# AdvancedPhotonSource/tike

Measured on AMD Instinct MI355X. Metric: diffraction patterns/sec/GPU (256x256, 8-mode probe), higher is better.
Workload: dtype c64; 1 GPU; c3; positions_per_gpu=10000, modes=8, detector=256, eigen_probes=1, solver=lstsq_grad, num_batch=10, chunk_positions=1000, position_correction=False, object_update=after every minibatch (batch_method wobbly_center), route=no_farplane

## Files before the change

include/tike_amd.h:

```cpp
#ifndef TIKE_AMD_H
#define TIKE_AMD_H

#ifdef __cplusplus
extern "C" {
#endif

#define TIKE_ERR_ARG 1000001
#define TIKE_ERR_UNSUPPORTED 1000002
#define TIKE_ERR_COMM 2000000
#define TIKE_COMM_ID_BYTES 128

#define TIKE_ABI_VERSION 11

const char* tike_build_id(void);

int tike_abi_version(void);

int tike_set_deterministic(int on, void* scratch, long bytes);

int tike_init(void);

int tike_patch_fwd(const void* images, void* patches, const float* positions, int nimage, int H,
                   int W, int nscan, int nrepeat, int patch_width, int padded_width,
                   void* stream);
int tike_patch_adj(void* images, const void* patches, const float* positions, int nimage, int H,
                   int W, int nscan, int nrepeat, int patch_width, int padded_width, int npatch,
                   void* stream);

int tike_conv_fwd(const void* psi, const float* scan, const void* probe, int probe_per_scan,
                  void* nearplane, int nscan, int S, int pw, int det, int H, int W, void* stream);
int tike_conv_adj(const void* nearplane, const float* scan, const void* probe,
                  int probe_per_scan, void* psi, int nscan, int S, int pw, int det, int H, int W,
                  void* stream);
int tike_conv_adj_probe(const void* nearplane, const float* scan, const void* psi,
                        void* probe_adj, int nscan, int S, int pw, int det, int H, int W,
                        void* stream);

int tike_fft2(const void* in, void* out, long ntile, int n, int inverse, float scale,
              void* stream);

int tike_fft2_supported(int n);

int tike_fft2_general(const void* in, void* out, long ntile, int n, int inverse, float scale,
                      int lines_per_group_rows, int lines_per_group_cols, void* stream);

int tike_ptycho_fwd(const void* psi, const float* scan, const void* probe, int probe_per_scan,
                    const void* eigen_probe, const float* eigen_weights, int num_eigen,
                    int eigen_modes, void* farplane, int nscan, int S, int pw, int det, int H,
                    int W, float scale, int sub_batch, void* stream);

int tike_ptycho_adj(const void* farplane, const void* probe, int probe_per_scan,
                    const float* scan, const void* psi, void* psi_adj, void* probe_adj,
                    void* objproj_work, float* acc_work, int nscan, int S, int pw, int det,
                    int H, int W, float scale, int sub_batch, void* stream);

int tike_ptycho_fwd_intensity(const void* psi, const float* scan, const void* probe,
                              int probe_per_scan, const void* unique_probe,
                              const float* eigen_weights, int num_eigen, int eigen_modes,
                              void* farplane, float* intensity, void* patches, int nscan, int S,
                              int pw, int det, int H, int W, float scale, void* stream);

int tike_ptycho_fwd_intensity_only(const void* psi, const float* scan, const void* probe,
                                   int probe_per_scan, const void* unique_probe,
                                   const float* eigen_weights, int num_eigen, int eigen_modes,
                                   void* scratch, float* intensity, int nscan, int S, int pw,
                                   int det, int H, int W, float scale, void* stream);

int tike_ptycho_fwd_gradient_scale(const void* psi, const float* scan, const void* probe,
                                   int probe_per_scan, const void* unique_probe,
                                   const float* eigen_weights, int num_eigen, int eigen_modes,
                                   void* scratch, float* intensity, void* patches,
                                   const float* data, const unsigned char* measured,
                                   float* gscale, float* costs, int nscan, int S, int pw, int det,
                                   int H, int W, float scale, int model, float unmeasured_scaling,
                                   long num_measured, void* stream);

int tike_fwd_pass1(const void* psi, const float* scan, const void* probe, int probe_per_scan,
                   const void* unique_probe, const void* eigen_probe,
                   const float* eigen_weights, int num_eigen, int eigen_modes, void* scratch,
                   void* patches, int nscan, int S, int pw, int det, int H, int W, void* stream);
int tike_fwd_gradient_scale(const void* scratch, const void* data, int data_u16,
                            const unsigned char* measured, float* gscale, float* intensity,
                            float* costs, void* farplane, int nscan, int S, int det, float scale,
                            int model, float unmeasured_scaling, long num_measured,
                            void* stream);

int tike_grad_ifft2_crop(const void* colin, const float* gscale, const float* mode_scale,
                         const unsigned char* measured, int S, void* work, void* chi,
                         long ntile, int det, int pw, float fwd_scale, float inv_scale,
                         void* stream);

int tike_fwd_grad_ifft2_pass1(const void* scratch, const void* data, int data_u16,
                              const unsigned char* measured, float* costs, void* work,
                              int nscan, int S, int det, float fwd_scale, int model,
                              float unmeasured_scaling, long num_measured, void* stream);
int tike_fwd_grad_ifft2_pass1_slices(const void* scratch, const void* data, int data_u16,
                                     const unsigned char* measured, float* costs, void* work,
                                     int nscan, int S, int det, float fwd_scale, int model,
                                     float unmeasured_scaling, long num_measured,
                                     const void* propagator, int nslices, void* stream);
int tike_grad_ifft2_pass1(const void* colin, const float* gscale, const float* mode_scale,
                          const unsigned char* measured, int S, void* work, long ntile, int det,
                          float fwd_scale, void* stream);
int tike_ifft2_pass1_scaled(const void* farplane, const float* gscale, const float* mode_scale,
                            const unsigned char* measured, int S, void* work, long ntile, int det,
                            void* stream);

int tike_ifft2_pass2_gradients(const void* work, const void* patches, const void* probe,
                               const void* eigen_probe, const float* eigen_weights,
                               int num_eigen, int eigen_modes, void* objproj, void* chi0,
                               void* m_probe_update, float mpu_scale, int nscan, int S, int det,
                               float inv_scale, void* stream);
int tike_ifft2_pass2_gradients_scaled(const void* work, const void* patches, const void* probe,
                                      const void* eigen_probe, const float* eigen_weights,
                                      int num_eigen, int eigen_modes, void* objproj, void* chi0,
                                      void* m_probe_update, float mpu_scale, int nscan, int S,
                                      int det, float inv_scale, const float* mode_scale,
                                      void* stream);
int tike_ifft2_pass2_eigen_fits(int det, int num_eigen, int eigen_modes);
int tike_ifft2_pass2_gradients_modes(const void* work, const void* patches, const void* probe,
                                     const void* eigen_probe, const float* eigen_weights,
                                     int num_eigen, int eigen_modes, void* objproj, void* chi0,
                                     void* m_probe_update, float mpu_scale, int nscan, int S,
                                     int det, float inv_scale, int mode0, int nmodes,
                                     int accumulate, void* stream);

int tike_gradient_scale(const float* intensity, const float* data, const unsigned char* measured,
                        float* gscale, float* costs, int nscan, int det, int model,
                        float unmeasured_scaling, long num_measured, void* stream);

int tike_ifft2_crop_scaled(const void* farplane, const float* gscale, int S, void* work,
                           void* chi, long ntile, int det, int pw, float scale, void* stream);

int tike_poisson_steps(const void* farplane, const float* intensity, const float* data,
                       const unsigned char* measured, float* steps, int nscan, int S, int det,
                       float step_start, float weight, int dominant_mode, void* stream);

int tike_poisson_steps_handoff(const void* scratch, const void* data, int data_u16,
                               const unsigned char* measured, float* gscale, float* costs,
                               float* steps, float* sums, int nscan, int S, int det, float scale,
                               float unmeasured_scaling, long num_measured, float step_start,
                               float weight, void* stream);

int tike_poisson_steps_grad_ifft2_pass1(const void* scratch, const void* data, int data_u16,
                                        const unsigned char* measured, float* costs,
                                        float* steps, float* sums, void* work, int nscan, int S,
                                        int det, float scale, float unmeasured_scaling,
                                        long num_measured, float step_start, float weight,
                                        void* stream);

int tike_ifft2_crop_scaled_modes(const void* farplane, const float* gscale,
                                 const float* mode_scale, const unsigned char* measured, int S,
                                 void* work, void* chi, long ntile, int det, int pw, float scale,
                                 void* stream);

int tike_scale_modes(void* farplane, const float* mode_scale, const unsigned char* measured,
                     long ntile, int det, void* stream);

int tike_ifft2_crop(const void* farplane, void* work, void* chi, long ntile, int det, int pw,
                    float scale, void* stream);

int tike_farplane_gradient(void* farplane, const float* data, const unsigned char* measured,
                           float* intensity, float* costs, int nscan, int S, int det, int model,
                           int apply_gradient, float unmeasured_scaling, long num_measured,
                           void* stream);
// ... 37 lines not shown

int tike_varying_probe(const void* probe, const void* eigen_probe, const float* eigen_weights,
                       int num_eigen, int eigen_modes, void* out, int nscan, int S, int pw,
                       void* stream);


int tike_eigen_position_sums(const void* patches, const void* chi0, const void* mpu0,
                             const void* eigen_probe, const void* coefs, int num_eigen,
                             int eigen_modes, int c, float* sums, int nscan, int pw,
                             int chi_modes, void* stream);

int tike_eigen_pixel_update(const void* patches, const void* chi0, const void* mpu0,
                            const void* eigen_probe, const void* coefs, int num_eigen,
                            int eigen_modes, int c, const float* pm, void* update, int nscan,
                            int pw, int chi_modes, void* stream);

int tike_position_sums(const void* patches, const void* chi, int chi_modes, const void* probe,
                       const void* eigen_probe, const float* eigen_weights, int num_eigen,
                       int eigen_modes, const float* taps, int radius, float* numerator,
                       float* denominator, int nscan, int S, int pw, void* stream);

int tike_gen_supported(int S, int pw, int det);

int tike_gen_fwd_rows(const void* psi, const float* scan, const void* probe, int probe_per_scan,
                      const void* unique, const void* eigen_probe, const float* eigen_weights,
                      int num_eigen, int eigen_modes, void* hand1, void* patches, int nscan, int S,
                      int pw, int det, int H, int W, void* stream);

int tike_gen_cols_gradient(const void* hand1, const float* data, const unsigned char* measured,
                           float* costs, void* hand2, int nscan, int S, int pw, int det,
                           float fwd_scale, int model, float unmeasured_scaling,
                           long num_measured, void* stream);

int tike_gen_inv_rows_gradients(const void* hand2, const void* patches, const void* probe,
                                int probe_per_scan, const void* unique, const void* eigen_probe,
                                const float* eigen_weights, int num_eigen, int eigen_modes,
                                void* objproj, void* chi0, void* m_probe_update,
                                float probe_update_scale, int nscan, int S, int pw, int det,
                                float inv_scale, void* stream);

int tike_pfa_supported(int S, int pw, int det);

int tike_pfa_fwd_gather(const void* psi, const float* scan, const void* probe,
                        int probe_per_scan, const void* unique, const void* eigen_probe,
                        const float* eigen_weights, int num_eigen, int eigen_modes,
                        void* subtiles, void* patches, int nscan, int S, int pw, int det, int H,
                        int W, void* stream);

int tike_pfa_fft2(const void* in, void* out, long ntile, int det, int inverse, void* stream);

int tike_pfa_fwd_subtiles_supported(int S, int pw, int det);
int tike_pfa_fwd_subtiles(const void* psi, const float* scan, const void* probe,
                          const void* eigen_probe, const float* eigen_weights, int num_eigen,
                          int eigen_modes, void* probe_scratch, void* subtiles, void* patches,
                          int nscan, int S, int pw, int det, int H, int W, void* stream);

int tike_pfa_combine_gradient(void* subtiles, const float* data, const unsigned char* measured,
                              float* costs, int nscan, int S, int det, float fwd_scale, int model,
                              float unmeasured_scaling, long num_measured, int apply_gradient,
                              void* stream);

int tike_pfa_inv_products(const void* subtiles, const void* patches, const void* probe,
                          int probe_per_scan, const void* unique, const void* eigen_probe,
                          const float* eigen_weights, int num_eigen, int eigen_modes,
                          void* objproj, void* chi0, void* m_probe_update,
                          float probe_update_scale, int nscan, int S, int pw, int det,
                          float inv_scale, void* stream);


int tike_fft2_pass1(const void* in, void* out, long ntile, int det, int inverse, void* stream);

int tike_fft2_pass2_inplace(void* tiles, long ntile, int det, int inverse, float scale,
                            void* stream);

int tike_slice_step(void* wave, const void* psi, const float* scan, void* farplane1, int nscan,
                    int S, int det, int H, int W, float scale, void* stream);

int tike_fft2_pass2_intensity(void* tiles, float* amplitude, long nscan, int S, int det,
                              int inverse, float scale, int keep, void* stream);

int tike_fresnel_colpass(const void* colin, const void* propagator, int adjoint, void* work,
                         long ntile, int det, float scale, void* stream);

int tike_ifft2_pass2_products(void* work, const void* psi, const float* scan, const void* probe,
                              int probe_per_scan, void* objproj, void* probe_numerator,
                              float numerator_scale, void* chi0, int keep_chi, int nscan, int S,
                              int det, int H, int W, float inv_scale, void* stream);

int tike_fresnel_spect_prop(const void* in, void* out, const void* propagator, long ntile, int n,
                            int adjoint, float fwd_scale, float inv_scale, void* stream);


int tike_object_update_precond(const float* acc, const void* precond, const float* pmax,
                               float alpha, void* upd_sum, void* upd_precond, float* combined,
                               long npix, void* stream);

int tike_lstsq_step_sums(const float* stats, const float* costs, int B, float eps, float* sums,
                         void* stream);
int tike_lstsq_step_solve(const float* stats, int B, float eps, const float* sums, double count,
                          int recover_psi, int recover_probe, float* out, void* stream);

int tike_probe_update(void* probe, void* combined, const void* mpu, const float* beta,
                      float inv_num_batch, long n, void* stream);

int tike_eigen_weights0(float* weights, const float* stats, int B, int C, int S, int m,
                        float* norms, void* stream);
int tike_eigen_proj_mean(const float* first, int first_stride, const float* weights_c,
                         long weights_row, const float* norm, long P, int B, float* pm,
                         void* stream);
int tike_eigen_normalise(void* eigen, const void* update, double count, float beta, int npix,
                         float* esum, float* work, void* stream);
int tike_eigen_dsum(const float* sums, int B, long P, float* dsum, void* stream);
int tike_eigen_weights(const float* sums, int B, long P, const float* dsum, double count,
                       float* weights_c, long weights_row, void* coefs_c, int coef_stride,
                       const float* esum, void* stream);

int tike_cgrad_direction(const float* update_planar, const void* update_complex, void* gradient,
                         void* direction, long n, int first, const float* costs, int ncost,
                         double count, double* state, double* sums, void* stream);

int tike_cgrad_line_search(int variable, const void* x, const void* d, void* xs,
                           const void* other, const float* scan, const void* data,
                           int data_u16, void* scratch, float* costs, int nscan, int chunk,
                           int S, int det, int H, int W, float fwd_scale, double count,
                           double* state, int* skip, int nslots, void* stream);

int tike_cgrad_line_search_linear(int variable, const void* x, const void* d, void* xs,
                                  const void* other, const float* scan, const void* data,
                                  int data_u16, void* far_a, int a_valid, void* far_b,
                                  float* costs_k, int nscan, int chunk, int S, int det, int H,
                                  int W, float fwd_scale, double count, double* state,
                                  int stage, double* sums, void* stream);

int tike_eigen_pixel_update1(const void* patches, const void* chi0, const void* mpu0,
                             const void* eigen0, const float* eigen_proj,
                             const float* weights_c, long weights_row, const float* norm,
                             void* update, int nscan, int pw, int chi_modes, const float* stats,
                             const float* costs, float eps, float* sums3, const void* psi,
                             const float* scan, int H, int W, void* stream);
int tike_lstsq_tail_mid(void* eigen0, const void* update, int npix, float* nacc,
                        float beta_eigen, const float* stats, int B, float eps,
                        const float* sums3, double count, int recover_psi, int recover_probe,
                        float* tail3, void* stream);
int tike_eigen_position_sums1(const void* patches, const void* chi0, const void* mpu0,
                              const void* eigen0, float* sums5, float* dsum, int nscan, int pw,
                              int chi_modes, const void* psi, const float* scan, int H, int W,
                              void* stream);
int tike_lstsq_tail_finish(const float* tail3, const float* sums3, double count, float* steps,
                           void* probe, void* combined, const void* mpu, float inv_num_batch,
                           long nprobe, float* weights, long weights_row, int S, int m,
                           const float* stats, const float* sums5, int B, int npix,
                           void* stream);

int tike_lstsq_chunk_gradients(const void* psi, const float* scan, const void* probe,
                               const void* eigen_probe, const float* eigen_weights,
                               int num_eigen, int eigen_modes, const void* data, int data_u16,
                               const unsigned char* measured, int model,
                               float unmeasured_scaling, long num_measured, void* scratch,
                               void* work, float* gscale, void* patches, float* costs,
                               void* objproj, void* chi0, void* m_probe_update,
                               float mpu_scale, float* object_acc, int nscan, int S, int det,
                               int H, int W, float fwd_scale, float inv_scale, void* stream);

int tike_comm_unique_id(void* id);
int tike_comm_create(const void* id, int nranks, int rank, void** comm);
int tike_comm_destroy(void* comm);
int tike_comm_allreduce_sum(void* comm, void* buf, long count, int f64, void* stream);
int tike_comm_broadcast(void* comm, void* buf, long nbytes, int root, void* stream);

int tike_cluster_farthest_fill(const float* points, long n, long* owner, int num_cluster,
                               long turns);
int tike_cluster_swap_sweep(const double* dist, long n, int k, long* label, const long* best,
                            const long* order, double* regret, int* moved);

#ifdef __cplusplus
}
#endif
#endif
```

tike_amd/_lib.py:

```python
import ctypes
import os
import re

import torch

_HERE = os.path.dirname(os.path.abspath(__file__))
LIB_PATH = os.environ.get("TIKE_AMD_LIB") or os.path.join(
    _HERE, "csrc", "libtike_amd.so")
HEADER_PATH = os.path.join(os.path.dirname(_HERE), "include", "tike_amd.h")

ABI_VERSION = 11
ERR_ARG = 1000001
ERR_UNSUPPORTED = 1000002
ERR_COMM = 2000000
COMM_ID_BYTES = 128

if not os.path.isfile(LIB_PATH):
    raise ImportError(
        f"{LIB_PATH} not found: build the HIP library first "
        "(`make -C tike_amd/csrc` or `python -c 'import __graft_entry__ as g; "
        "g.build()'`). tike_amd has no CPU fallback.")

lib = ctypes.CDLL(LIB_PATH)

_p = ctypes.c_void_p
_i = ctypes.c_int
_l = ctypes.c_long
_f = ctypes.c_float
_d = ctypes.c_double

_PROTOTYPES = {
    "tike_abi_version": [],
    "tike_init": [],
    "tike_set_deterministic": [_i, _p, _l],
    "tike_patch_fwd": [_p, _p, _p, _i, _i, _i, _i, _i, _i, _i, _p],
    "tike_patch_adj": [_p, _p, _p, _i, _i, _i, _i, _i, _i, _i, _i, _p],
    "tike_conv_fwd": [_p, _p, _p, _i, _p, _i, _i, _i, _i, _i, _i, _p],
    "tike_conv_adj": [_p, _p, _p, _i, _p, _i, _i, _i, _i, _i, _i, _p],
    "tike_conv_adj_probe": [_p, _p, _p, _p, _i, _i, _i, _i, _i, _i, _p],
    "tike_fft2": [_p, _p, _l, _i, _i, _f, _p],
    "tike_fft2_supported": [_i],
    "tike_fft2_general": [_p, _p, _l, _i, _i, _f, _i, _i, _p],
    "tike_pfa_supported": [_i, _i, _i],
    "tike_pfa_fwd_gather": [_p, _p, _p, _i, _p, _p, _p, _i, _i, _p, _p, _i, _i, _i,
                            _i, _i, _i, _p],
    "tike_pfa_fwd_subtiles_supported": [_i, _i, _i],
    "tike_pfa_fwd_subtiles": [_p, _p, _p, _p, _p, _i, _i, _p, _p, _p, _i, _i,
                              _i, _i, _i, _i, _p],
    "tike_pfa_fft2": [_p, _p, _l, _i, _i, _p],
    "tike_pfa_combine_gradient": [_p, _p, _p, _p, _i, _i, _i, _f, _i, _f, _l, _i,
                                  _p],
    "tike_pfa_inv_products": [_p, _p, _p, _i, _p, _p, _p, _i, _i, _p, _p, _p, _f,
                              _i, _i, _i, _i, _f, _p],
    "tike_gen_supported": [_i, _i, _i],
    "tike_gen_fwd_rows": [_p, _p, _p, _i, _p, _p, _p, _i, _i, _p, _p, _i, _i, _i,
                          _i, _i, _i, _p],
    "tike_gen_cols_gradient": [_p, _p, _p, _p, _p, _i, _i, _i, _i, _f, _i, _f,
                               _l, _p],
    "tike_gen_inv_rows_gradients": [_p, _p, _p, _i, _p, _p, _p, _i, _i, _p, _p,
                                    _p, _f, _i, _i, _i, _i, _f, _p],
    "tike_fresnel_spect_prop": [_p, _p, _p, _l, _i, _i, _f, _f, _p],
    "tike_fft2_pass1": [_p, _p, _l, _i, _i, _p],
    "tike_fft2_pass2_inplace": [_p, _l, _i, _i, _f, _p],
    "tike_slice_step": [_p, _p, _p, _p, _i, _i, _i, _i, _i, _f, _p],
    "tike_fft2_pass2_intensity": [_p, _p, _l, _i, _i, _i, _f, _i, _p],
    "tike_fresnel_colpass": [_p, _p, _i, _p, _l, _i, _f, _p],
    "tike_ifft2_pass2_products": [_p, _p, _p, _p, _i, _p, _p, _f, _p, _i, _i, _i,
                                  _i, _i, _i, _f, _p],
    "tike_ptycho_fwd": [_p, _p, _p, _i, _p, _p, _i, _i, _p, _i, _i, _i, _i,
                        _i, _i, _f, _i, _p],
    "tike_ptycho_adj": [_p, _p, _i, _p, _p, _p, _p, _p, _p, _i, _i, _i, _i, _i,
                        _i, _f, _i, _p],
    "tike_ifft2_crop": [_p, _p, _p, _l, _i, _i, _f, _p],
    "tike_ptycho_fwd_intensity": [_p, _p, _p, _i, _p, _p, _i, _i, _p, _p, _p,
                                  _i, _i, _i, _i, _i, _i, _f, _p],
    "tike_gradient_scale": [_p, _p, _p, _p, _p, _i, _i, _i, _f, _l, _p],
    "tike_ifft2_crop_scaled": [_p, _p, _i, _p, _p, _l, _i, _i, _f, _p],
    "tike_ifft2_crop_scaled_modes": [_p, _p, _p, _p, _i, _p, _p, _l, _i, _i, _f,
                                     _p],
    "tike_poisson_steps": [_p, _p, _p, _p, _p, _i, _i, _i, _f, _f, _i, _p],
    "tike_poisson_steps_handoff": [_p, _p, _i, _p, _p, _p, _p, _p, _i, _i, _i, _f,
                                   _f, _l, _f, _f, _p],
    "tike_scale_modes": [_p, _p, _p, _l, _i, _p],
    "tike_ptycho_fwd_intensity_only": [_p, _p, _p, _i, _p, _p, _i, _i, _p, _p,
                                       _i, _i, _i, _i, _i, _i, _f, _p],
    "tike_ptycho_fwd_gradient_scale": [_p, _p, _p, _i, _p, _p, _i, _i, _p, _p,
                                       _p, _p, _p, _p, _p, _i, _i, _i, _i, _i,
                                       _i, _f, _i, _f, _l, _p],
    "tike_fwd_pass1": [_p, _p, _p, _i, _p, _p, _p, _i, _i, _p, _p, _i, _i, _i,
                       _i, _i, _i, _p],
    "tike_fwd_gradient_scale": [_p, _p, _i, _p, _p, _p, _p, _p, _i, _i, _i, _f,
                                _i, _f, _l, _p],
    "tike_grad_ifft2_pass1": [_p, _p, _p, _p, _i, _p, _l, _i, _f, _p],
    "tike_fwd_grad_ifft2_pass1": [_p, _p, _i, _p, _p, _p, _i, _i, _i, _f, _i, _f,
                                  _l, _p],
    "tike_fwd_grad_ifft2_pass1_slices": [_p, _p, _i, _p, _p, _p, _i, _i, _i, _f, _i, _f,
                                  _l, _p, _i, _p],
    "tike_ifft2_pass1_scaled": [_p, _p, _p, _p, _i, _p, _l, _i, _p],
    "tike_ifft2_pass2_gradients": [_p, _p, _p, _p, _p, _i, _i, _p, _p, _p, _f,
                                   _i, _i, _i, _f, _p],
    "tike_ifft2_pass2_gradients_scaled": [_p, _p, _p, _p, _p, _i, _i, _p, _p,
                                          _p, _f, _i, _i, _i, _f, _p, _p],
    "tike_ifft2_pass2_eigen_fits": [_i, _i, _i],
    "tike_ifft2_pass2_gradients_modes": [_p, _p, _p, _p, _p, _i, _i, _p, _p,
                                         _p, _f, _i, _i, _i, _f, _i, _i, _i, _p],
    "tike_poisson_steps_grad_ifft2_pass1": [_p, _p, _i, _p, _p, _p, _p, _p, _i,
                                            _i, _i, _f, _f, _l, _f, _f, _p],
    "tike_object_update_precond": [_p, _p, _p, _f, _p, _p, _p, _l, _p],
    "tike_lstsq_step_sums": [_p, _p, _i, _f, _p, _p],
    "tike_lstsq_step_solve": [_p, _i, _f, _p, _d, _i, _i, _p, _p],
    "tike_probe_update": [_p, _p, _p, _p, _f, _l, _p],
    "tike_eigen_weights0": [_p, _p, _i, _i, _i, _i, _p, _p],
    "tike_eigen_proj_mean": [_p, _i, _p, _l, _p, _l, _i, _p, _p],
    "tike_eigen_normalise": [_p, _p, _d, _f, _i, _p, _p, _p],
    "tike_eigen_dsum": [_p, _i, _l, _p, _p],
    "tike_eigen_weights": [_p, _i, _l, _p, _d, _p, _l, _p, _i, _p, _p],
    "tike_grad_ifft2_crop": [_p, _p, _p, _p, _i, _p, _p, _l, _i, _i, _f, _f,
                             _p],
    "tike_position_sums": [_p, _p, _i, _p, _p, _p, _i, _i, _p, _i, _p, _p, _i,
                           _i, _i, _p],
    "tike_farplane_gradient": [_p, _p, _p, _p, _p, _i, _i, _i, _i, _i, _f, _l,
                               _p],
    "tike_intensity": [_p, _p, _l, _i, _l, _p],
    "tike_cost_each_pattern": [_p, _p, _p, _l, _l, _i, _p],
    "tike_objective_grad": [_p, _p, _p, _p, _l, _i, _l, _i, _p],
    "tike_lstsq_gradients": [_p, _p, _p, _p, _p, _p, _i, _i, _p, _p, _p, _p, _i,
                             _i, _i, _i, _i, _p],
    "tike_varying_probe": [_p, _p, _p, _i, _i, _p, _i, _i, _i, _p],
    "tike_scatter_patches": [_p, _p, _p, _i, _i, _i, _i, _p],
    "tike_eigen_position_sums": [_p, _p, _p, _p, _p, _i, _i, _i, _p, _i, _i,
                                 _i, _p],
    "tike_eigen_pixel_update": [_p, _p, _p, _p, _p, _i, _i, _i, _p, _p, _i, _i,
                                _i, _p],
    "tike_probe_grad": [_p, _p, _p, _p, _p, _i, _i, _i, _i, _i, _p],
    "tike_probe_preconditioner": [_p, _p, _p, _i, _i, _i, _i, _p],
    "tike_psi_preconditioner": [_p, _p, _p, _i, _i, _i, _i, _p],
    "tike_scatter_amplitudes": [_p, _p, _p, _i, _i, _i, _i, _p],
    "tike_lstsq_step_stats": [_p, _p, _p, _p, _p, _p, _p, _i, _i, _p, _p, _p,
                              _p, _i, _i, _i, _i, _i, _i, _p, _p, _p],
    "tike_eigen_pixel_update1": [_p, _p, _p, _p, _p, _p, _l, _p, _p, _i, _i, _i,
                                 _p, _p, _f, _p, _p, _p, _i, _i, _p],
    "tike_lstsq_tail_mid": [_p, _p, _i, _p, _f, _p, _i, _f, _p, _d, _i, _i, _p,
                            _p],
    "tike_eigen_position_sums1": [_p, _p, _p, _p, _p, _p, _i, _i, _i, _p, _p,
                                  _i, _i, _p],
    "tike_lstsq_tail_finish": [_p, _p, _d, _p, _p, _p, _p, _f, _l, _p, _l, _i,
                               _i, _p, _p, _i, _i, _p],
    "tike_lstsq_chunk_gradients": [_p, _p, _p, _p, _p, _i, _i, _p, _i, _p, _i,
                                   _f, _l, _p, _p, _p, _p, _p, _p, _p, _p, _f,
                                   _p, _i, _i, _i, _i, _i, _f, _f, _p],
    "tike_cgrad_direction": [_p, _p, _p, _p, _l, _i, _p, _i, _d, _p, _p, _p],
    "tike_cgrad_line_search": [_i, _p, _p, _p, _p, _p, _p, _i, _p, _p, _i, _i,
                               _i, _i, _i, _i, _f, _d, _p, _p, _i, _p],
    "tike_cgrad_line_search_linear": [_i, _p, _p, _p, _p, _p, _p, _i, _p, _i, _p,
                                      _p, _i, _i, _i, _i, _i, _i, _f, _d, _p, _i,
                                      _p, _p],
    "tike_comm_unique_id": [_p],
    "tike_comm_create": [_p, _i, _i, ctypes.POINTER(_p)],
    "tike_comm_destroy": [_p],
    "tike_comm_allreduce_sum": [_p, _p, _l, _i, _p],
    "tike_comm_broadcast": [_p, _p, _l, _i, _p],
    "tike_cluster_farthest_fill": [_p, _l, _p, _i, _l],
    "tike_cluster_swap_sweep": [_p, _l, _i, _p, _p, _p, _p, _p],
}


def build_id():
    try:
        fn = lib.tike_build_id
    except AttributeError:
        return ""
    fn.restype = ctypes.c_char_p
    fn.argtypes = []
    return fn().decode()


def declared_symbols():
    with open(HEADER_PATH) as f:
        text = f.read()
    return sorted(set(re.findall(r"^int\s+(tike_\w+)\s*\(", text, flags=re.M)))


for _name, _args in _PROTOTYPES.items():
    try:
        _fn = getattr(lib, _name)
    except AttributeError as e:
        raise ImportError(
            f"{LIB_PATH} does not export {_name}: it was built from another "
            "include/tike_amd.h; rebuild it (`make -C tike_amd/csrc`).") from e
    _fn.argtypes = _args
    _fn.restype = ctypes.c_int


def _check_abi_version():
    got = lib.tike_abi_version()
    m = re.search(r"^#define\s+TIKE_ABI_VERSION\s+(\d+)", open(HEADER_PATH).read(),
                  flags=re.M) if os.path.isfile(HEADER_PATH) else None
    if got != ABI_VERSION or (m and int(m.group(1)) != ABI_VERSION):
        raise ImportError(
            f"{LIB_PATH} reports ABI version {got}, include/tike_amd.h "
            f"{m.group(1) if m else '?'}, this binding expects {ABI_VERSION}: "
            "rebuild the library (`make -C tike_amd/csrc`).")


_check_abi_version()


def check(rc, what=""):
    if rc == 0:
        return
    if rc == ERR_ARG:
        raise ValueError(f"{what}: incompatible shapes / arguments")
    if rc == ERR_UNSUPPORTED:
        raise ValueError(f"{what}: unsupported size for the HIP path")
    if rc >= ERR_COMM:
        raise RuntimeError(f"{what}: RCCL error {rc - ERR_COMM}")
    raise RuntimeError(f"{what}: HIP error {rc}")


DETERMINISTIC = os.environ.get("TIKE_DETERMINISTIC", "0") == "1"
DETERMINISTIC_SCRATCH_MIB = int(os.environ.get("TIKE_DETERMINISTIC_MIB", "256"))
_det_scratch = None


def ensure_deterministic():
    global _det_scratch
    if not DETERMINISTIC:
        return
    current = torch.cuda.current_device()
    if _det_scratch is not None and _det_scratch.device.index == current:
        return
    if _det_scratch is not None:
        torch.cuda.synchronize(_det_scratch.device)
    _det_scratch = torch.empty(DETERMINISTIC_SCRATCH_MIB << 20,
                               dtype=torch.uint8,
                               device=torch.device("cuda", current))
    check(lib.tike_set_deterministic(1, _det_scratch.data_ptr(),
                                     _det_scratch.numel()),
          "tike_set_deterministic")
```

tike_amd/_tuning.py:

```python
import os


def _flag(name, default):
    return os.environ.get(name, "1" if default else "0") == "1"


def _int(name, default=None):
    v = os.environ.get(name)
    return int(v) if v else default


one_launch_512 = _flag("TIKE_ONE_LAUNCH_512", True)
poisson_steps_in_pass2 = _flag("TIKE_POISSON_LINEAR", True)
chunk_positions = _int("TIKE_CHUNK_POSITIONS")
eigen_sums_gather = _flag("TIKE_EIGEN_SUMS_GATHER", True)
stats_gather = _flag("TIKE_STATS_GATHER", False)
precond_chunk = _int("TIKE_PRECOND_CHUNK", 512)
multislice_slice_step = _flag("TIKE_MS_SLICE_STEP", True)
multislice_first_stored = _flag("TIKE_MS_FIRST_STORED", True)
multislice_step_back = _flag("TIKE_MS_STEP_BACK", True)
cgrad_graphs = _flag("TIKE_CGRAD_GRAPHS", False)
fwd_sub_mib = (float(os.environ["TIKE_FWD_SUB_MIB"])
               if os.environ.get("TIKE_FWD_SUB_MIB") else None)
```

tike_amd/csrc/lstsq.hip:

```cpp
#include "fft_engine2.h"
#include <type_traits>

#include "internal.h"
#include "tike_amd.h"

#ifndef TK_STATS_PAIRS
#define TK_STATS_PAIRS 1
#endif
static const bool g_stats_pairs = TK_STATS_PAIRS != 0;

constexpr int TK_STRIP = 32;
#define TK_ATOMIC_ADD(p, v) unsafeAtomicAdd(p, v)

template <bool REAL_ONLY, class ValueFn, class Sink>
__device__ __forceinline__ void scatter_footprint_rows(ValueFn&& value, float fx, float fy,
                                                       int pw, int r0, int r1, Sink&& sink) {
  for (int x0 = 0; x0 < pw; x0 += blockDim.x) {
    const int xp = x0 + threadIdx.x;
    const bool active = xp < pw;
    cf uprev = mk(0.f, 0.f), uprev_last = mk(0.f, 0.f);
    constexpr int RG = 4;
    cf vv[RG], ll[RG], nv[RG], nl[RG];
    auto load_group = [&](int yb, cf (&a)[RG], cf (&b)[RG]) {
      const int xpc = active ? xp : pw - 1;
// ... 423 lines not shown
    if (!WITH_CHI && c.sy >= 0 && c.sx >= 0 && c.sy + pw < H && c.sx + pw < W &&
        total < (1L << 28)) {
      typedef float tk_v4f __attribute__((ext_vector_type(4)));
      const unsigned off = (unsigned)(y * W + x) * (unsigned)sizeof(cf);
      tk_v4f u, l;
      __builtin_memcpy(&u, reinterpret_cast<const char*>(psi) + off, sizeof(u));
      __builtin_memcpy(&l, reinterpret_cast<const char*>(psi) + off + (unsigned)W * 8u, sizeof(l));
      o = mk(u.x * c.w00, u.y * c.w00);
      o.x += u.z * c.w01;
      o.y += u.w * c.w01;
      o.x += l.x * c.w10;
      o.y += l.y * c.w10;
      o.x += l.z * c.w11;
      o.y += l.w * c.w11;
    } else {
      o = tk_gather(psi, (long)yc * W + xc, W, total, c);
      if (!ok) o = mk(0.f, 0.f);
    }
    if (patches) patches[b * P + p] = o;
    if (WITH_CHI) {
      const cf oc = conjf(o);
      cf proj = mk(0.f, 0.f);
#pragma unroll
      for (int s = 0; s < SM; ++s)
        if (SC > 0 || s < S) {
          if (out) acc[s] = acc[s] + oc * xs[s];
          if (objproj) {
            cf ps;
            if (hoist && !(probe.weights != nullptr && probe.eigen != nullptr && s < probe.Sm)) {
              const float w0 =
                  probe.weights ? probe.weights[b * (long)(probe.C + 1) * probe.S + s] : 1.0f;
              ps = pr[s] * w0;
            } else {
              ps = probe.at(b, s, p);
            }
            proj = proj + conjf(ps) * xs[s];
          }
        }
      if (objproj) objproj[b * P + p] = proj;
    } else {
      acc[0].x += norm2(o);
    }
  }
  if (WITH_CHI) {
    if (out) {
#pragma unroll
      for (int s = 0; s < SM; ++s)
        if (SC > 0 || s < S) {
          if (part != nullptr) {
            float* o = part + 2 * (((long)blockIdx.y * S + s) * P + p);
            o[0] = acc[s].x;
            o[1] = acc[s].y;
          } else {
            unsafeAtomicAdd(&out[2 * (s * P + p)], acc[s].x);
            unsafeAtomicAdd(&out[2 * (s * P + p) + 1], acc[s].y);
          }
        }
    }
  } else if (part != nullptr) {
    part[(long)blockIdx.y * P + p] = acc[0].x;
  } else {
    unsafeAtomicAdd(&out[2 * p], acc[0].x);
  }
}

template <bool WITH_CHI>
static void launch_probe_grad(dim3 grid, hipStream_t stream, const cf* chi, const float* scan,
                              const cf* psi, cf* patches, float* out, const TkProbe& probe,
                              cf* objproj, int nscan, int S, int pw, int H, int W, int chunk,
                              float* part = nullptr) {
#define TK_PG(SC)                                                                              \
  hipLaunchKernelGGL((probe_grad_kernel<WITH_CHI, SC>), grid, dim3(256), 0, stream, chi, scan, \
                     psi, patches, out, probe, objproj, nscan, S, pw, H, W, chunk, part)
  switch (WITH_CHI ? S : 1) {
    case 1: TK_PG(1); break;
    case 2: TK_PG(2); break;
    case 3: TK_PG(3); break;
    case 4: TK_PG(4); break;
    case 5: TK_PG(5); break;
    case 6: TK_PG(6); break;
    case 8: TK_PG(8); break;
    default: TK_PG(0); break;
  }
#undef TK_PG
}

static int probe_chunk(int nscan, long len = 0, float** part = nullptr) {
  int chunk = (nscan + 31) / 32;
  chunk = chunk < 8 ? 8 : chunk;
  if (!tk_deterministic()) return chunk;
  const int nchunk = (nscan + chunk - 1) / chunk;
  float* p = len > 0 && part ? tk_det_scratch(sizeof(float) * (size_t)len * nchunk) : nullptr;
  if (p != nullptr) {
    *part = p;
    return chunk;
  }
  return nscan > 8 ? nscan : 8;
}

extern "C" int tike_probe_grad(const void* chi, const float* scan, const void* psi,
                               void* patches, void* m_probe_update, int nscan, int S, int pw,
                               int H, int W, void* stream) {
  TK_ENTER();
  TK_CHECK_ARG(nscan >= 0 && S >= 1 && S <= TK_MAX_MODES && pw >= 1 && H >= 1 && W >= 1);
  if (nscan == 0) return TK_OK;
  TK_CHECK_ARG(chi && scan && psi && m_probe_update);
  const long P = (long)pw * pw;
  float* part = nullptr;
  const int chunk = probe_chunk(nscan, 2 * S * P, &part);
  dim3 grid((unsigned)((P + 255) / 256), (unsigned)((nscan + chunk - 1) / chunk));
  launch_probe_grad<true>(grid, (hipStream_t)stream, (const cf*)chi, scan, (const cf*)psi,
                          (cf*)patches, (float*)m_probe_update,
                          tk_make_probe(psi, 0, nullptr, nullptr, 0, 0, S, pw), (cf*)nullptr,
                          nscan, S, pw, H, W, chunk, part);
  TK_LAUNCH_CHECK();
  if (part != nullptr)
    return tk_ordered_sum((float*)m_probe_update, part, 2 * S * P, (int)grid.y, true,
                          (hipStream_t)stream);
  return TK_OK;
}

extern "C" int tike_lstsq_gradients(const void* chi, const float* scan, const void* psi,
                                    const void* probe, const void* eigen_probe,
                                    const float* eigen_weights, int num_eigen, int eigen_modes,
                                    const void* unique_probe, void* patches,
                                    void* m_probe_update, void* objproj, int nscan, int S,
                                    int pw, int H, int W, void* stream) {
  TK_ENTER();
  TK_CHECK_ARG(nscan >= 0 && S >= 1 && S <= TK_MAX_MODES && pw >= 1 && H >= 1 && W >= 1);
  if (nscan == 0) return TK_OK;
  TK_CHECK_ARG(chi && scan && psi && probe);
  const long P = (long)pw * pw;
  float* part = nullptr;
  const int chunk = probe_chunk(nscan, m_probe_update ? 2 * S * P : 0, &part);
  dim3 grid((unsigned)((P + 255) / 256), (unsigned)((nscan + chunk - 1) / chunk));
  launch_probe_grad<true>(grid, (hipStream_t)stream, (const cf*)chi, scan, (const cf*)psi,
                          (cf*)patches, (float*)m_probe_update,
                          tk_make_probe(probe, 0, eigen_probe, eigen_weights, num_eigen,
                                        eigen_modes, S, pw, unique_probe),
                          (cf*)objproj, nscan, S, pw, H, W, chunk, part);
  TK_LAUNCH_CHECK();
  if (part != nullptr)
    return tk_ordered_sum((float*)m_probe_update, part, 2 * S * P, (int)grid.y, true,
                          (hipStream_t)stream);
  return TK_OK;
}

struct TkModeProbe {
  const cf* base;
  float w0;
  int nE;
};

template <int N, int MW, int MPW, bool HAVE_PROJ, bool EIG = true, bool GRP = false>
__global__ __launch_bounds__(256, 2) void ifft2_pass2_gradients_kernel(
    const cf* __restrict__ mid, const cf* __restrict__ patches, const TkProbe probe,
    cf* __restrict__ objproj, cf* __restrict__ chi0, float* __restrict__ mpu, float mpu_scale,
    int nscan, int S, float inv_scale, int chunk, float* __restrict__ mpu_part,
    const float* __restrict__ mode_scale, int Stot_ = 0, int accumulate_ = 0) {
  const int Stot = GRP ? Stot_ : S;
  const bool accumulate = GRP && accumulate_ != 0;
  constexpr int RB = N / 16;
  constexpr int CW = 4 / MW;
  constexpr int NCB = N / (64 * CW);
  constexpr int NSLICE = 16 * NCB;
  constexpr bool REDUCE = HAVE_PROJ && MW > 1;
  constexpr bool HOIST = RB <= 16;
  static_assert(NCB >= 1 && NSLICE % 8 == 0, "slice layout");
  constexpr int NBUF = RB <= 16 ? 2 : 1;
  __shared__ cf part[REDUCE ? NBUF * 4 * RB * 64 : 1];
  extern __shared__ cf eigl[];
  constexpr long P = (long)N * N;
  const int v = blockIdx.x;
  constexpr int per = NSLICE / 8;
  const int slice = (v & 7) * per + (v >> 3) % per;
  const int nchunk_ = (nscan + chunk - 1) / chunk;
  const int b0 = (nchunk_ - 1 - ((v >> 3) / per)) * chunk;
  const int b1 = min(nscan, b0 + chunk);
  const int ya = slice / NCB, cb = slice % NCB;
  const int w = __builtin_amdgcn_readfirstlane(threadIdx.x >> 6);
  const int lane = threadIdx.x & 63;
  const int mw = w % MW, cw = w / MW;
  constexpr long ROW = 16 * N;
  const long slice0 = (long)ya * N + (cb * CW + cw) * 64;
  const unsigned lb = (unsigned)lane * (unsigned)sizeof(cf);
  if (EIG && HAVE_PROJ && probe.weights != nullptr && probe.eigen != nullptr) {
    const int total = probe.C * probe.Sm * RB * 64 * CW;
    for (int i = threadIdx.x; i < total; i += 256) {
      const int x = i % (64 * CW), yb = (i / (64 * CW)) % RB, cs = i / (64 * CW * RB);
      eigl[i] = conjf(probe.eigen[(long)cs * P + ya * N + yb * ROW + cb * CW * 64 + x]);
    }
  }
  __syncthreads();
  static_assert(MW > 1 || MPW == 1, "a lone mode-wave writes objproj straight from one mode");
  cf acc[MPW][RB];
  cf Pc[HAVE_PROJ && HOIST ? MPW : 1][HAVE_PROJ && HOIST ? RB : 1];
#pragma unroll
  for (int m = 0; m < MPW; ++m) {
    const int s = mw + MW * m;
    const int sc = s < S ? s : S - 1;
#pragma unroll
    for (int yb = 0; yb < RB; ++yb) {
      acc[m][yb] = mk(0.f, 0.f);
      if (HAVE_PROJ && HOIST)
        Pc[m][yb] = conjf(*tk_at(probe.probe + (long)sc * P + slice0 + yb * ROW, lb));
    }
  }
  const bool vary = HAVE_PROJ && probe.weights != nullptr;
  const int nE = (EIG && vary && probe.eigen != nullptr) ? probe.C : 0;
  for (int n = b0; n < b1; ++n) {
    unsigned lo = lb;
    asm volatile("" : "+v"(lo));
    const cf* __restrict__ On = patches + (long)n * P + slice0;
    constexpr bool O_ONCE = HOIST && MPW == 1;
    cf O[HOIST ? RB : 1];
    if (O_ONCE) {
#pragma unroll
      for (int yb = 0; yb < RB; ++yb) O[yb] = *tk_at(On + yb * ROW, lo);
    }
    cf* slot = part + ((((n - b0) & (NBUF - 1)) * 4 + w) * RB) * 64 + lane;
    const cf* slots = part + ((((n - b0) & (NBUF - 1)) * 4 + cw * MW) * RB) * 64 + lane;
    const float* __restrict__ wn =
        vary ? probe.weights + n * (long)(probe.C + 1) * probe.S : nullptr;
#pragma unroll
    for (int m = 0; m < MPW; ++m) {
      const int s = mw + MW * m;
      if (s < S) {
        const cf* __restrict__ src = mid + ((long)n * Stot + s) * P + slice0;
        cf u[RB];
#pragma unroll
        for (int k = 0; k < RB; ++k) u[k] = tk_ld_stream(tk_at(src + k * ROW, lo));
        if (HOIST && !O_ONCE) {
#pragma unroll
          for (int yb = 0; yb < RB; ++yb) O[yb] = *tk_at(On + yb * ROW, lo);
        }
        const float w0 = vary ? wn[s] : 1.0f;
        const float sc = mode_scale ? inv_scale * mode_scale[(long)n * Stot + s] : inv_scale;
        Dft<RB, true>::run(u);
        if (HOIST) {
#pragma unroll
          for (int yb = 0; yb < RB; ++yb) {
            u[yb] = u[yb] * sc;
            acc[m][yb] = acc[m][yb] + conjf(O[yb]) * u[yb];
          }
        } else {
#pragma unroll
          for (int g = 0; g < RB; g += 8) {
            cf o[8];
#pragma unroll
            for (int i = 0; i < 8; ++i) o[i] = *tk_at(On + (g + i) * ROW, lo);
#pragma unroll
            for (int i = 0; i < 8; ++i) {
              u[g + i] = u[g + i] * sc;
              acc[m][g + i] = acc[m][g + i] + conjf(o[i]) * u[g + i];
            }
            __builtin_amdgcn_sched_barrier(0);
          }
        }
        if (s == 0 && chi0 != nullptr) {
#pragma unroll
          for (int yb = 0; yb < RB; ++yb)
            tk_st_stream(tk_at(chi0 + (long)n * P + slice0 + yb * ROW, lo), u[yb]);
        }
        if (HAVE_PROJ) {
          const cf* __restrict__ Ps = probe.probe + (long)s * P + slice0;
          const bool eig = EIG && nE > 0 && s < probe.Sm;
#pragma unroll
          for (int g = 0; g < RB; g += 8) {
            cf pc[8];
#pragma unroll
            for (int i = 0; i < 8; ++i)
              pc[i] = HOIST ? Pc[m][g + i] : conjf(*tk_at(Ps + (g + i) * ROW, lo));
#pragma unroll
            for (int i = 0; i < 8; ++i) {
              cf t = (pc[i] * u[g + i]) * w0;
              if (REDUCE) {
                slot[(g + i) * 64] = m == 0 ? t : slot[(g + i) * 64] + t;
              } else {
                if (eig) {
#pragma unroll 1
                  for (int c = 0; c < nE; ++c)
                    t = t + (eigl[((c * probe.Sm + s) * RB + g + i) * (64 * CW) + cw * 64 + lane] *
                             u[g + i]) * wn[(c + 1) * probe.S + s];
                }
                tk_st_stream(tk_at(objproj + (long)n * P + slice0 + (g + i) * ROW, lo), t);
              }
            }
            if (!HOIST) __builtin_amdgcn_sched_barrier(0);
          }
          if (REDUCE && eig) {
#pragma unroll 1
            for (int c = 0; c < nE; ++c) {
              const float wc = wn[(c + 1) * probe.S + s];
              const cf* __restrict__ el =
                  eigl + ((c * probe.Sm + s) * RB) * (64 * CW) + cw * 64 + lane;
#pragma unroll
              for (int yb = 0; yb < RB; ++yb)
                slot[yb * 64] = slot[yb * 64] + (el[yb * (64 * CW)] * u[yb]) * wc;
            }
          }
        }
      } else if (REDUCE && m == 0) {
#pragma unroll
        for (int yb = 0; yb < RB; ++yb) slot[yb * 64] = mk(0.f, 0.f);
      }
    }
    if (REDUCE) {
      __syncthreads();
#pragma unroll
      for (int q = 0; q < RB / MW; ++q) {
        const int yb = mw + MW * q;
        cf sum = slots[yb * 64];
#pragma unroll
        for (int k = 1; k < MW; ++k) sum = sum + slots[(k * RB + yb) * 64];
        if (accumulate) sum = sum + *tk_at(objproj + (long)n * P + slice0 + yb * ROW, lo);
        tk_st_stream(tk_at(objproj + (long)n * P + slice0 + yb * ROW, lo), sum);
      }
      if (NBUF == 1) __syncthreads();
    }
  }
  if (mpu != nullptr) {
#pragma unroll
    for (int m = 0; m < MPW; ++m) {
      const int s = mw + MW * m;
      if (s < S) {
#pragma unroll
        for (int yb = 0; yb < RB; ++yb) {
          if (mpu_part != nullptr) {
            const long ci = (nchunk_ - 1) - b0 / chunk;
            float* o = tk_at(mpu_part + 2 * ((ci * S + s) * P + slice0 + yb * ROW), lb);
            o[0] = acc[m][yb].x * mpu_scale;
            o[1] = acc[m][yb].y * mpu_scale;
          } else {
            float* o = tk_at(mpu + 2 * ((long)s * P + slice0 + yb * ROW), lb);
            unsafeAtomicAdd(o, acc[m][yb].x * mpu_scale);
            unsafeAtomicAdd(o + 1, acc[m][yb].y * mpu_scale);
          }
        }
      }
    }
  }
}

static int launch_pass2_gradients(const void* work, const void* patches, const void* probe,
                                  const void* eigen_probe, const float* eigen_weights,
                                  int num_eigen, int eigen_modes, void* objproj, void* chi0,
                                  void* m_probe_update, float mpu_scale, int nscan, int S,
                                  int det, float inv_scale, const float* mode_scale,
                                  hipStream_t stream, int Stot = 0, int accumulate = 0) {
  TK_CHECK_ARG(nscan >= 0 && S >= 1 && det >= 1);
  if (nscan == 0) return TK_OK;
  TK_CHECK_ARG(work && patches && (probe || !objproj));
  if (S > 8 || (det != 128 && det != 256 && det != 512)) return TK_ERR_UNSUPPORTED;
  const bool grp = Stot != 0;
  if (grp && objproj && S < 2) return TK_ERR_UNSUPPORTED;
  const TkProbe pr = tk_make_probe(probe, 0, eigen_probe, eigen_weights, num_eigen, eigen_modes,
                                   grp ? Stot : S, det);
  int MW = S >= 3 ? 4 : S;
  if (det == 128 && MW == 1) MW = 2;
  auto eig_bytes = [&](int mw) {
    return sizeof(cf) * (size_t)num_eigen * eigen_modes * (det / 16) * 64 * (4 / mw);
  };
  if (objproj && eigen_weights && eigen_probe)
    while (MW < 4 && eig_bytes(MW) > 32 * 1024) MW *= 2;
  const int MPW = S > 4 ? 2 : 1;
  const int nslice = 16 * (det / (64 * (4 / MW)));
  int nchunk = (1024 + nslice - 1) / nslice;
  {
    int unit = 512, a = nslice;
    while (a % 2 == 0 && unit > 1) { a /= 2; unit /= 2; }
    if (nchunk >= unit) nchunk = nchunk / unit * unit;
  }
  int chunk = (nscan + nchunk - 1) / nchunk;
  if (chunk < 8) chunk = 8;
  nchunk = (nscan + chunk - 1) / chunk;
  const dim3 grid((unsigned)(nslice * nchunk)), block(256);
  float* mpu_part = nullptr;
  const long mpu_len = 2L * S * det * det;
  if (m_probe_update && tk_deterministic()) {
    mpu_part = tk_det_scratch(sizeof(float) * (size_t)mpu_len * nchunk);
    if (mpu_part == nullptr) return TK_ERR_ARG;
  }
  size_t eig_lds = 0;
  if (objproj && eigen_weights && eigen_probe) eig_lds = eig_bytes(MW);
  if (eig_lds > 32 * 1024) return TK_ERR_UNSUPPORTED;
#define TK_P2G(N, MW_, MPW_)                                                                 \
  do {                                                                                       \
    if (grp && !objproj)                                                                     \
      hipLaunchKernelGGL((ifft2_pass2_gradients_kernel<N, MW_, MPW_, false, true, true>),    \
                         grid, block, 0,                                                     \
                         stream, (const cf*)work, (const cf*)patches, pr, (cf*)objproj,      \
                         (cf*)chi0, (float*)m_probe_update, mpu_scale, nscan, S, inv_scale,  \
                         chunk, mpu_part, mode_scale, Stot, accumulate);                     \
    else if (grp && eig_lds > 0)                                                             \
      hipLaunchKernelGGL((ifft2_pass2_gradients_kernel<N, MW_, MPW_, true, true, true>),     \
                         grid, block, eig_lds,                                               \
                         stream, (const cf*)work, (const cf*)patches, pr, (cf*)objproj,      \
                         (cf*)chi0, (float*)m_probe_update, mpu_scale, nscan, S, inv_scale,  \
                         chunk, mpu_part, mode_scale, Stot, accumulate);                     \
    else if (grp)                                                                            \
      hipLaunchKernelGGL((ifft2_pass2_gradients_kernel<N, MW_, MPW_, true, false, true>),    \
                         grid, block, 0,                                                     \
                         stream, (const cf*)work, (const cf*)patches, pr, (cf*)objproj,      \
                         (cf*)chi0, (float*)m_probe_update, mpu_scale, nscan, S, inv_scale,  \
                         chunk, mpu_part, mode_scale, Stot, accumulate);                     \
    else if (objproj && eig_lds > 0)                                                         \
      hipLaunchKernelGGL((ifft2_pass2_gradients_kernel<N, MW_, MPW_, true>), grid, block,    \
                         eig_lds,                                                            \
                         stream, (const cf*)work, (const cf*)patches, pr, (cf*)objproj,      \
                         (cf*)chi0, (float*)m_probe_update, mpu_scale, nscan, S, inv_scale,  \
                         chunk, mpu_part, mode_scale);                                       \
    else if (objproj)                                                                        \
      hipLaunchKernelGGL((ifft2_pass2_gradients_kernel<N, MW_, MPW_, true, false>), grid,    \
                         block, 0,                                                           \
                         stream, (const cf*)work, (const cf*)patches, pr, (cf*)objproj,      \
                         (cf*)chi0, (float*)m_probe_update, mpu_scale, nscan, S, inv_scale,  \
                         chunk, mpu_part, mode_scale);                                       \
    else                                                                                     \
      hipLaunchKernelGGL((ifft2_pass2_gradients_kernel<N, MW_, MPW_, false>), grid, block,   \
                         0, stream, (const cf*)work, (const cf*)patches, pr, (cf*)objproj,   \
                         (cf*)chi0, (float*)m_probe_update, mpu_scale, nscan, S, inv_scale,  \
                         chunk, mpu_part, mode_scale);                                       \
  } while (0)
#define TK_P2G_N(N)                     \
  do {                                  \
    if (MW == 1)                        \
      TK_P2G(N < 256 ? 256 : N, 1, 1);  \
    else if (MW == 2)                   \
      TK_P2G(N, 2, 1);                  \
    else if (MPW == 1)                  \
      TK_P2G(N, 4, 1);                  \
    else                                \
      TK_P2G(N, 4, 2);                  \
  } while (0)
  switch (det) {
    case 128: TK_P2G_N(128); break;
    case 256: TK_P2G_N(256); break;
    default: TK_P2G_N(512); break;
  }
#undef TK_P2G_N
#undef TK_P2G
  TK_LAUNCH_CHECK();
  if (mpu_part != nullptr)
    return tk_ordered_sum((float*)m_probe_update, mpu_part, mpu_len, nchunk, true, stream);
  return TK_OK;
}

extern "C" int tike_ifft2_pass2_gradients(const void* work, const void* patches,
                                          const void* probe, const void* eigen_probe,
                                          const float* eigen_weights, int num_eigen,
                                          int eigen_modes, void* objproj, void* chi0,
                                          void* m_probe_update, float mpu_scale, int nscan,
                                          int S, int det, float inv_scale, void* stream) {
  TK_ENTER();
  return launch_pass2_gradients(work, patches, probe, eigen_probe, eigen_weights, num_eigen,
                                eigen_modes, objproj, chi0, m_probe_update, mpu_scale, nscan, S,
                                det, inv_scale, nullptr, (hipStream_t)stream);
}

extern "C" int tike_ifft2_pass2_gradients_scaled(const void* work, const void* patches,
                                                 const void* probe, const void* eigen_probe,
                                                 const float* eigen_weights, int num_eigen,
                                                 int eigen_modes, void* objproj, void* chi0,
                                                 void* m_probe_update, float mpu_scale,
                                                 int nscan, int S, int det, float inv_scale,
                                                 const float* mode_scale, void* stream) {
  TK_ENTER();
  TK_CHECK_ARG(nscan == 0 || mode_scale != nullptr);
  return launch_pass2_gradients(work, patches, probe, eigen_probe, eigen_weights, num_eigen,
                                eigen_modes, objproj, chi0, m_probe_update, mpu_scale, nscan, S,
                                det, inv_scale, mode_scale, (hipStream_t)stream);
}

extern "C" int tike_ifft2_pass2_eigen_fits(int det, int num_eigen, int eigen_modes) {
  if (det < 16 || num_eigen < 0 || eigen_modes < 0) return 0;
  return sizeof(cf) * (size_t)num_eigen * eigen_modes * (det / 16) * 64 <= 32 * 1024 ? 1 : 0;
}

extern "C" int tike_ifft2_pass2_gradients_modes(const void* work, const void* patches,
                                                const void* probe, const void* eigen_probe,
                                                const float* eigen_weights, int num_eigen,
                                                int eigen_modes, void* objproj, void* chi0,
                                                void* m_probe_update, float mpu_scale,
                                                int nscan, int S, int det, float inv_scale,
                                                int mode0, int nmodes, int accumulate,
                                                void* stream) {
  TK_ENTER();
  TK_CHECK_ARG(S >= 1 && det >= 1 && mode0 >= 0 && nmodes >= 1 && mode0 + nmodes <= S);
  TK_CHECK_ARG(nscan == 0 || (work && (probe || !objproj)));
  const long P = (long)det * det;
  const bool first = mode0 == 0;
  if (first ? eigen_modes > nmodes : false) return TK_ERR_UNSUPPORTED;
  return launch_pass2_gradients(
      (const cf*)work + mode0 * P, patches, probe ? (const cf*)probe + mode0 * P : nullptr,
      first ? eigen_probe : nullptr, eigen_weights ? eigen_weights + mode0 : nullptr,
      first ? num_eigen : (eigen_weights ? num_eigen : 0), first ? eigen_modes : 0, objproj,
      first ? chi0 : nullptr,
      m_probe_update ? (void*)((float*)m_probe_update + 2 * mode0 * P) : nullptr, mpu_scale,
      nscan, nmodes, det, inv_scale, nullptr, (hipStream_t)stream, S, accumulate);
}

template <int RW>
__global__ __launch_bounds__(256) void probe_precond_rows_kernel(
    const float* __restrict__ scan, const cf* __restrict__ psi, float* __restrict__ out,
    int nscan, int pw, int H, int W, int chunk, float* __restrict__ part) {
  typedef float tk_v4f __attribute__((ext_vector_type(4)));
  const long P = (long)pw * pw;
  const long total = (long)H * W;
  const int cols = pw < 256 ? pw : 256, ncb = pw / cols;
  const int x = ((int)blockIdx.x % ncb) * cols + (int)threadIdx.x % cols;
  const int y0 = (((int)blockIdx.x / ncb) * (256 / cols) + (int)threadIdx.x / cols) * RW;
  const int b0 = blockIdx.y * chunk;
  const int b1 = min(nscan, b0 + chunk);
  float acc[RW];
#pragma unroll
  for (int r = 0; r < RW; ++r) acc[r] = 0.f;
  bool inside = true;
  for (int b = b0; b < b1; ++b) {
    const TkCorner c = tk_corner(scan, b);
    inside = inside && c.sy >= 0 && c.sx >= 0 && c.sy + pw < H && c.sx + pw < W;
  }
  if (inside) {
    const unsigned row_bytes = (unsigned)W * (unsigned)sizeof(cf);
    const unsigned lane_off = (unsigned)y0 * row_bytes + (unsigned)x * (unsigned)sizeof(cf);
#pragma unroll 2
    for (int b = b0; b < b1; ++b) {
      const TkCorner c = tk_corner(scan, b);
      const unsigned off = (unsigned)(c.sy * W + c.sx) * (unsigned)sizeof(cf) + lane_off;
      tk_v4f t[RW + 1];
#pragma unroll
      for (int r = 0; r <= RW; ++r)
        __builtin_memcpy(&t[r], reinterpret_cast<const char*>(psi) + off + (unsigned)r * row_bytes,
                         sizeof(tk_v4f));
#pragma unroll
      for (int r = 0; r < RW; ++r) {
        cf o = mk(t[r].x * c.w00, t[r].y * c.w00);
        o.x += t[r].z * c.w01;
        o.y += t[r].w * c.w01;
        o.x += t[r + 1].x * c.w10;
        o.y += t[r + 1].y * c.w10;
        o.x += t[r + 1].z * c.w11;
        o.y += t[r + 1].w * c.w11;
        acc[r] += norm2(o);
      }
    }
  } else {
    for (int b = b0; b < b1; ++b) {
      const TkCorner c = tk_corner(scan, b);
#pragma unroll
      for (int r = 0; r < RW; ++r) {
        const int y = c.sy + y0 + r, xx = c.sx + x;
        const bool ok = y >= 0 && y < H && xx >= 0 && xx < W;
        const int yc = y < 0 ? 0 : (y >= H ? H - 1 : y);
        const int xc = xx < 0 ? 0 : (xx >= W ? W - 1 : xx);
        const cf o = tk_gather(psi, (long)yc * W + xc, W, total, c);
        acc[r] += ok ? norm2(o) : 0.f;
      }
    }
  }
#pragma unroll
  for (int r = 0; r < RW; ++r) {
    const long p = (long)(y0 + r) * pw + x;
    if (part != nullptr)
      part[(long)blockIdx.y * P + p] = acc[r];
    else
      unsafeAtomicAdd(&out[2 * p], acc[r]);
  }
}

extern "C" int tike_probe_preconditioner(const float* scan, const void* psi, void* out,
                                         int nscan, int pw, int H, int W, void* stream) {
  TK_ENTER();
  TK_CHECK_ARG(nscan >= 0 && pw >= 1 && H >= 1 && W >= 1);
  if (nscan == 0) return TK_OK;
  TK_CHECK_ARG(scan && psi && out);
  const long P = (long)pw * pw;
  float* part = nullptr;
  const int chunk = probe_chunk(nscan, P, &part);
  dim3 grid((unsigned)((P + 255) / 256), (unsigned)((nscan + chunk - 1) / chunk));
  constexpr int RW = 4;
  const int cols = pw < 256 ? pw : 256;
  if (g_stats_pairs && (pw % 256 == 0 || 256 % pw == 0) && pw % ((256 / cols) * RW) == 0 &&
      (long)H * W < (1L << 28)) {
    grid.x = (unsigned)(P / (256 * RW));
    hipLaunchKernelGGL(probe_precond_rows_kernel<RW>, grid, dim3(256), 0, (hipStream_t)stream,
                       scan, (const cf*)psi, (float*)out, nscan, pw, H, W, chunk, part);
  } else {
    launch_probe_grad<false>(grid, (hipStream_t)stream, (const cf*)nullptr, scan,
                             (const cf*)psi, (cf*)nullptr, (float*)out,
                             tk_make_probe(psi, 0, nullptr, nullptr, 0, 0, 1, pw),
                             (cf*)nullptr, nscan, 1, pw, H, W, chunk, part);
  }
  TK_LAUNCH_CHECK();
  if (part != nullptr)
    return tk_ordered_sum((float*)out, part, P, (int)grid.y, true, (hipStream_t)stream, 2);
  return TK_OK;
}

template <bool HAVE_PATCHES, bool HAVE_GOBJ>
__device__ __forceinline__ void step_stats_item(
    const cf* __restrict__ chi, const float* __restrict__ scan, const cf* __restrict__ psi,
    const cf* __restrict__ gobj, const TkProbe& probe, const cf* __restrict__ mpu,
    const cf* __restrict__ patches, float* __restrict__ stats, int chi_modes, int pw, int H,
    int W, const cf* __restrict__ eigen0, float* __restrict__ eigen_proj, int nsplit, int n,
    int part, float* red) {
  const long P = (long)pw * pw;
  const long total = (long)H * W;
  const int plen = (int)(P / nsplit);
  {
    const TkCorner c = tk_corner(scan, n);
    const cf* __restrict__ pbase = probe.probe + n * probe.pos_stride;
    float pw0 = 1.0f, pw1 = 0.f;
    int nE = 0;
    const float* __restrict__ wn = nullptr;
    if (probe.weights != nullptr) {
      if (probe.unique != nullptr && 0 < probe.Sm) {
        pbase = probe.unique + (long)n * probe.Sm * P;
      } else {
        wn = probe.weights + n * (long)(probe.C + 1) * probe.S;
        pw0 = wn[0];
        if (probe.eigen != nullptr && 0 < probe.Sm) {
          nE = probe.C;
          pw1 = wn[probe.S];
        }
// ... 313 lines not shown
    }
  }
}

extern "C" int tike_lstsq_step_stats(const void* chi, const float* scan, const void* psi,
                                     const void* object_update_precond, const void* probe,
                                     const void* eigen_probe, const float* eigen_weights,
                                     int num_eigen, int eigen_modes, const void* unique_probe,
                                     const void* m_probe_update, const void* patches,
                                     float* stats, int nscan, int S, int chi_modes, int pw, int H,
                                     int W, const void* eigen0, float* eigen_proj, void* stream) {
  TK_ENTER();
  TK_CHECK_ARG(nscan >= 0 && S >= 1 && chi_modes >= 1 && pw >= 1 && H >= 1 && W >= 1);
  if (nscan == 0) return TK_OK;
  TK_CHECK_ARG(chi && scan && psi && probe && stats);
  TK_CHECK_ARG(!eigen_proj || (eigen0 && m_probe_update));
  const TkProbe pr = tk_make_probe(probe, 0, eigen_probe, eigen_weights, num_eigen, eigen_modes,
                                   S, pw, unique_probe);
  const bool no_eigen = (eigen_probe == nullptr || eigen_modes == 0) && eigen_proj == nullptr;
  const bool one_eigen = eigen_probe != nullptr && eigen_weights != nullptr && eigen_modes > 0 &&
                         num_eigen == 1 && eigen_proj != nullptr && eigen0 == eigen_probe;
  const bool pairs = g_stats_pairs && patches && object_update_precond && m_probe_update &&
                     unique_probe == nullptr && (no_eigen || one_eigen) &&
                     (long)H * W < (1L << 28) && nscan > 1;
  const long nitem = pairs ? (nscan + 1) / 2 : nscan;
  int nsplit = 1;
  while (nsplit < 16 && nitem * nsplit * 2 <= 8192 && ((long)pw * pw) % (2048L * nsplit) == 0)
    nsplit *= 2;
  if (tk_deterministic()) nsplit = 1;
  if (nsplit > 1) {
    hipError_t e = hipMemsetAsync(stats, 0, sizeof(float) * 8 * (size_t)nscan, (hipStream_t)stream);
    if (e == hipSuccess && eigen_proj)
      e = hipMemsetAsync(eigen_proj, 0, sizeof(float) * (size_t)nscan, (hipStream_t)stream);
    if (e != hipSuccess) return (int)e;
  }
#define TK_SS(HP, HG)                                                                         \
  hipLaunchKernelGGL((step_stats_kernel<HP, HG>), dim3(tk_grid((long)nscan * nsplit, 16)),    \
                     dim3(256), 0,                                                            \
                     (hipStream_t)stream, (const cf*)chi, scan, (const cf*)psi,               \
                     (const cf*)object_update_precond, pr, (const cf*)m_probe_update,         \
                     (const cf*)patches, stats, nscan, chi_modes, pw, H, W, (const cf*)eigen0, \
                     eigen_proj, nsplit)
#define TK_SP(EIG)                                                                            \
  hipLaunchKernelGGL((step_stats_pair_kernel<EIG>), dim3(tk_grid(nitem * nsplit, 16)),        \
                     dim3(256), 0,                                                            \
                     (hipStream_t)stream, (const cf*)chi, scan, (const cf*)psi,               \
                     (const cf*)object_update_precond, pr, (const cf*)m_probe_update,         \
                     (const cf*)patches, stats, nscan, chi_modes, pw, H, W, (const cf*)eigen0, \
                     eigen_proj, nsplit)
  if (pairs && one_eigen) TK_SP(true);
  else if (pairs) TK_SP(false);
  else if (patches && object_update_precond) TK_SS(true, true);
  else if (patches) TK_SS(true, false);
  else if (object_update_precond) TK_SS(false, true);
  else TK_SS(false, false);
#undef TK_SS
#undef TK_SP
  TK_LAUNCH_CHECK();
  return TK_OK;
}

struct TkResidual {
  const cf* patches;
  const cf* chi0;
  const cf* mpu0;
  const cf* eigen;
  const cf* coefs;
  int C, Sm, c;
  long P;
  long XS;
  template <bool C0>
  __device__ __forceinline__ cf at(long n, long p) const {
    cf r = conjf(patches[n * P + p]) * chi0[n * XS + p] - mpu0[p];
    if (!C0)
      for (int k = 0; k < c; ++k) r = r - coefs[n * C + k] * eigen[((long)k * Sm) * P + p];
    return r;
  }
};

template <bool C0>
__global__ __launch_bounds__(256) void eigen_position_sums_kernel(const TkResidual R,
                                                                  float* __restrict__ sums,
                                                                  int nscan) {
  __shared__ float red[4];
  const cf* __restrict__ E = R.eigen + ((long)R.c * R.Sm) * R.P;
  for (int n = blockIdx.x; n < nscan; n += gridDim.x) {
    float a[5] = {0.f, 0.f, 0.f, 0.f, 0.f};
    for (long p = threadIdx.x; p < R.P; p += blockDim.x) {
      const cf e = E[p];
      const cf r = R.at<C0>(n, p);
      const cf phi = R.patches[n * R.P + p] * e;
      const cf x = R.chi0[n * R.XS + p];
      a[0] += r.x * e.x + r.y * e.y;
      a[1] += x.x * phi.x + x.y * phi.y;
      a[2] += norm2(phi);
      const cf re = r * conjf(e);
      a[3] += re.x;
      a[4] += re.y;
    }
#pragma unroll
    for (int k = 0; k < 5; ++k) {
      const float v = tk_block_sum256(a[k], red);
      if (threadIdx.x == 0) sums[(long)n * 5 + k] = v;
    }
  }
}

template <bool C0>
__global__ __launch_bounds__(256) void eigen_pixel_update_kernel(const TkResidual R,
                                                                 const float* __restrict__ pm,
                                                                 float* __restrict__ update,
                                                                 int nscan, int chunk,
                                                                 float* __restrict__ part) {
  const long p = (long)blockIdx.x * blockDim.x + threadIdx.x;
  if (p >= R.P) return;
  const int b0 = blockIdx.y * chunk;
  const int b1 = min(nscan, b0 + chunk);
  cf acc = mk(0.f, 0.f);
#pragma unroll 4
  for (int n = b0; n < b1; ++n) {
    const cf r = R.at<C0>(n, p);
    const float w = pm[n];
    acc.x += r.x * w;
    acc.y += r.y * w;
  }
  if (part != nullptr) {
    part[2 * ((long)blockIdx.y * R.P + p)] = acc.x;
    part[2 * ((long)blockIdx.y * R.P + p) + 1] = acc.y;
    return;
  }
  unsafeAtomicAdd(&update[2 * p], acc.x);
  unsafeAtomicAdd(&update[2 * p + 1], acc.y);
}

__device__ __forceinline__ cf tk_patch_pixel(const cf* __restrict__ psi, unsigned off,
                                             unsigned row_bytes, const TkCorner& c) {
  typedef float tk_v4f __attribute__((ext_vector_type(4)));
  tk_v4f u, l;
  __builtin_memcpy(&u, reinterpret_cast<const char*>(psi) + off, sizeof(u));
  __builtin_memcpy(&l, reinterpret_cast<const char*>(psi) + off + row_bytes, sizeof(l));
  cf o = mk(u.x * c.w00, u.y * c.w00);
  o.x += u.z * c.w01;
  o.y += u.w * c.w01;
  o.x += l.x * c.w10;
  o.y += l.y * c.w10;
  o.x += l.z * c.w11;
  o.y += l.w * c.w11;
  return o;
}
__device__ __forceinline__ bool tk_interior(const TkCorner& c, int pw, int H, int W) {
  return c.sy >= 0 && c.sx >= 0 && c.sy + pw < H && c.sx + pw < W && (long)H * W < (1L << 28);
}

__global__ __launch_bounds__(256) void eigen_pixel_update1_kernel(
    const TkResidual R, const float* __restrict__ eproj, const float* __restrict__ weights_c,
    long row, const float* __restrict__ norm, float inv_P, float* __restrict__ update, int nscan,
    int chunk, const float* __restrict__ stats, const float* __restrict__ costs, float eps,
    float* __restrict__ sums3, const cf* __restrict__ psi, const float* __restrict__ scan, int pw,
    int H, int W, float* __restrict__ part) {
  if (blockIdx.x + 1 == gridDim.x) {
    if (blockIdx.y != 0 || sums3 == nullptr) return;
    __shared__ float red[4];
    float a1 = 0.f, a4 = 0.f, c = 0.f;
    for (int n = threadIdx.x; n < nscan; n += 256) {
      a1 += stats[8 * n] + eps;
      a4 += stats[8 * n + 1] + eps;
      c += costs[n];
    }
    a1 = tk_block_sum256(a1, red);
    a4 = tk_block_sum256(a4, red);
    c = tk_block_sum256(c, red);
    if (threadIdx.x == 0) {
      sums3[0] = a1;
      sums3[1] = a4;
      sums3[2] = c;
    }
    return;
  }
  const long p = (long)blockIdx.x * blockDim.x + threadIdx.x;
  if (p >= R.P) return;
  const int b0 = blockIdx.y * chunk;
  const int b1 = min(nscan, b0 + chunk);
  const float inv_norm = 1.0f / norm[0];
  cf acc = mk(0.f, 0.f);
  bool gather = psi != nullptr;
  if (gather) {
    for (int n = b0; n < b1; ++n) gather = gather && tk_interior(tk_corner(scan, n), pw, H, W);
  }
  if (gather) {
    const int py = (int)(p / pw), px = (int)(p % pw);
    const unsigned row_bytes = (unsigned)W * (unsigned)sizeof(cf);
    const unsigned lane_off = (unsigned)py * row_bytes + (unsigned)px * (unsigned)sizeof(cf);
    const cf m0 = R.mpu0[p];
#pragma unroll 4
    for (int n = b0; n < b1; ++n) {
      const TkCorner c = tk_corner(scan, n);
      const cf x = R.chi0[n * R.XS + p];
      const cf o = tk_patch_pixel(
          psi, (unsigned)(c.sy * W + c.sx) * (unsigned)sizeof(cf) + lane_off, row_bytes, c);
      const cf r = conjf(o) * x - m0;
      const float w = (eproj[n] * inv_P + weights_c[n * row]) * inv_norm;
      acc.x += r.x * w;
      acc.y += r.y * w;
    }
  } else {
#pragma unroll 4
    for (int n = b0; n < b1; ++n) {
      const cf r = R.at<true>(n, p);
      const float w = (eproj[n] * inv_P + weights_c[n * row]) * inv_norm;
      acc.x += r.x * w;
      acc.y += r.y * w;
    }
  }
  if (part != nullptr) {
    part[2 * ((long)blockIdx.y * R.P + p)] = acc.x;
    part[2 * ((long)blockIdx.y * R.P + p) + 1] = acc.y;
    return;
  }
  unsafeAtomicAdd(&update[2 * p], acc.x);
  unsafeAtomicAdd(&update[2 * p + 1], acc.y);
}

__global__ __launch_bounds__(256) void column_sum_ordered_kernel(const float* __restrict__ table,
                                                                 int stride, int col, int n,
                                                                 float scale,
                                                                 float* __restrict__ out) {
  __shared__ float red[4];
  float a = 0.f;
  for (int i = threadIdx.x; i < n; i += 256) a += table[(long)i * stride + col] * scale;
  a = tk_block_sum256(a, red);
  if (threadIdx.x == 0) out[0] += a;
}

__global__ __launch_bounds__(256) void eigen_position_sums1_kernel(
    const TkResidual R, float* __restrict__ sums, float* __restrict__ dsum, int nscan,
    const cf* __restrict__ psi, const float* __restrict__ scan, int pw, int H, int W) {
  __shared__ float red[4];
  const cf* __restrict__ E = R.eigen;
  const unsigned row_bytes = (unsigned)W * (unsigned)sizeof(cf);
  const int qstep = (int)blockDim.x / pw, rstep = (int)blockDim.x % pw;
  for (int n = blockIdx.x; n < nscan; n += gridDim.x) {
    float a[5] = {0.f, 0.f, 0.f, 0.f, 0.f};
    TkCorner c = {0, 0, 0.f, 0.f, 0.f, 0.f};
    if (psi != nullptr) c = tk_corner(scan, n);
    const bool gather = psi != nullptr && tk_interior(c, pw, H, W);
    const unsigned off0 = gather ? (unsigned)(c.sy * W + c.sx) * (unsigned)sizeof(cf) : 0u;
    auto body = [&](auto g_tag) {
      constexpr bool G = decltype(g_tag)::value;
      int py = (int)threadIdx.x / pw, px = (int)threadIdx.x % pw;
      for (long p = threadIdx.x; p < R.P; p += blockDim.x) {
        const cf e = E[p];
        const cf x = R.chi0[n * R.XS + p];
        const cf m0 = R.mpu0[p];
        cf o;
        if constexpr (G)
          o = tk_patch_pixel(psi, off0 + (unsigned)py * row_bytes + (unsigned)px * 8u, row_bytes, c);
        else
          o = R.patches[n * R.P + p];
        const cf r = conjf(o) * x - m0;
        const cf phi = o * e;
        py += qstep;
        px += rstep;
        if (px >= pw) {
          px -= pw;
          ++py;
        }
        a[0] += r.x * e.x + r.y * e.y;
        a[1] += x.x * phi.x + x.y * phi.y;
        a[2] += norm2(phi);
        const cf re = r * conjf(e);
        a[3] += re.x;
        a[4] += re.y;
      }
    };
    if (gather)
      body(std::true_type{});
    else
      body(std::false_type{});
#pragma unroll
    for (int k = 0; k < 5; ++k) {
      const float v = tk_block_sum256(a[k], red);
      if (threadIdx.x == 0) {
        sums[(long)n * 5 + k] = v;
        if (k == 2 && dsum != nullptr) unsafeAtomicAdd(dsum, v / (float)R.P);
      }
    }
  }
}

__global__ __launch_bounds__(512) void eigen_position_sums1_pair_kernel(
    const TkResidual R, float* __restrict__ sums, float* __restrict__ dsum, int nscan,
    const cf* __restrict__ psi, const float* __restrict__ scan, int pw, int H, int W) {
  __shared__ float red[8];
  typedef float tk_v4f __attribute__((ext_vector_type(4)));
  const cf* __restrict__ E = R.eigen;
  const unsigned row_bytes = (unsigned)W * (unsigned)sizeof(cf);
  const int cols = pw < 256 ? pw : 256, rows = pw / (512 / cols);
  const int npair = (nscan + 1) / 2;
  auto add = [](float* a, const cf o, const cf x, const cf e, const cf m0) {
    const cf r = conjf(o) * x - m0;
    const cf phi = o * e;
    a[0] += r.x * e.x + r.y * e.y;
    a[1] += x.x * phi.x + x.y * phi.y;
    a[2] += norm2(phi);
    const cf re = r * conjf(e);
    a[3] += re.x;
    a[4] += re.y;
  };
  auto finish = [&](const float* a, const int n) {
#pragma unroll
    for (int k = 0; k < 5; ++k) {
      const float v = tk_block_sum512(a[k], red);
      if (threadIdx.x == 0) {
        sums[(long)n * 5 + k] = v;
        if (k == 2 && dsum != nullptr) unsafeAtomicAdd(dsum, v / (float)R.P);
      }
    }
  };
  auto one = [&](const int n, const TkCorner& c, const bool gather) {
    float a[5] = {0.f, 0.f, 0.f, 0.f, 0.f};
    const unsigned off0 = gather ? (unsigned)(c.sy * W + c.sx) * 8u : 0u;
    for (long p = threadIdx.x; p < R.P; p += blockDim.x) {
      const cf o = gather ? tk_patch_pixel(psi, off0 + (unsigned)(p / pw) * row_bytes +
                                                    (unsigned)(p % pw) * 8u, row_bytes, c)
                          : R.patches[n * R.P + p];
      add(a, o, R.chi0[n * R.XS + p], E[p], R.mpu0[p]);
    }
    finish(a, n);
  };
  auto taps16 = [&](const unsigned off) {
    tk_v4f t;
    __builtin_memcpy(&t, reinterpret_cast<const char*>(psi) + off, sizeof(t));
    return t;
  };
  auto tap = [](const tk_v4f u, const tk_v4f l, const TkCorner& c) {
    cf o = mk(u.x * c.w00, u.y * c.w00);
    o.x += u.z * c.w01;
    o.y += u.w * c.w01;
    o.x += l.x * c.w10;
    o.y += l.y * c.w10;
    o.x += l.z * c.w11;
    o.y += l.w * c.w11;
    return o;
  };
  for (int pair = blockIdx.x; pair < npair; pair += gridDim.x) {
    const int n0 = 2 * pair;
    const bool two = n0 + 1 < nscan;
    const TkCorner c0 = tk_corner(scan, n0);
    const TkCorner c1 = tk_corner(scan, two ? n0 + 1 : n0);
    const bool in0 = tk_interior(c0, pw, H, W), in1 = tk_interior(c1, pw, H, W);
    if (!(two && in0 && in1)) {
      one(n0, c0, in0);
      if (two) one(n0 + 1, c1, in1);
      continue;
    }
    float a[5] = {0.f, 0.f, 0.f, 0.f, 0.f}, b[5] = {0.f, 0.f, 0.f, 0.f, 0.f};
    const unsigned base0 = (unsigned)(c0.sy * W + c0.sx), base1 = (unsigned)(c1.sy * W + c1.sx);
    const cf* __restrict__ chi_a = R.chi0 + (long)n0 * R.XS;
    const cf* __restrict__ chi_b = chi_a + R.XS;
    const int ybeg = ((int)threadIdx.x / cols) * rows;
    for (int x = (int)threadIdx.x % cols; x < pw; x += 256) {
      unsigned rel = (unsigned)(ybeg * W + x);
      tk_v4f u0 = taps16((base0 + rel) * 8u), u1 = taps16((base1 + rel) * 8u);
      int p = ybeg * pw + x;
#pragma unroll 2
      for (int y = 0; y < rows; ++y) {
        rel += (unsigned)W;
        const tk_v4f l0 = taps16((base0 + rel) * 8u), l1 = taps16((base1 + rel) * 8u);
        const cf e = E[p], m0 = R.mpu0[p];
        const cf xa = chi_a[p], xb = chi_b[p];
        add(a, tap(u0, l0, c0), xa, e, m0);
        add(b, tap(u1, l1, c1), xb, e, m0);
        u0 = l0;
        u1 = l1;
        p += pw;
      }
    }
    finish(a, n0);
    finish(b, n0 + 1);
  }
}

static TkResidual make_residual(const void* patches, const void* chi0, const void* mpu0,
                                const void* eigen, const void* coefs, int C, int Sm, int c,
                                int pw, int chi_modes) {
  TkResidual R;
  R.patches = (const cf*)patches;
  R.chi0 = (const cf*)chi0;
  R.mpu0 = (const cf*)mpu0;
  R.eigen = (const cf*)eigen;
  R.coefs = (const cf*)coefs;
  R.C = C;
  R.Sm = Sm;
  R.c = c;
  R.P = (long)pw * pw;
  R.XS = R.P * chi_modes;
  return R;
}

extern "C" int tike_eigen_position_sums(const void* patches, const void* chi0, const void* mpu0,
                                        const void* eigen_probe, const void* coefs,
                                        int num_eigen, int eigen_modes, int c, float* sums,
                                        int nscan, int pw, int chi_modes, void* stream) {
  TK_ENTER();
  TK_CHECK_ARG(nscan >= 0 && pw >= 1 && num_eigen >= 1 && c >= 0 && c < num_eigen &&
               chi_modes >= 1);
  if (nscan == 0) return TK_OK;
  TK_CHECK_ARG(patches && chi0 && mpu0 && eigen_probe && sums && (c == 0 || coefs));
  const TkResidual R = make_residual(patches, chi0, mpu0, eigen_probe, coefs, num_eigen,
                                     eigen_modes, c, pw, chi_modes);
  if (c == 0)
    hipLaunchKernelGGL(eigen_position_sums_kernel<true>, dim3(tk_grid(nscan, 16)), dim3(256), 0,
                       (hipStream_t)stream, R, sums, nscan);
  else
    hipLaunchKernelGGL(eigen_position_sums_kernel<false>, dim3(tk_grid(nscan, 16)), dim3(256),
                       0, (hipStream_t)stream, R, sums, nscan);
  TK_LAUNCH_CHECK();
  return TK_OK;
}

extern "C" int tike_eigen_pixel_update(const void* patches, const void* chi0, const void* mpu0,
                                       const void* eigen_probe, const void* coefs,
                                       int num_eigen, int eigen_modes, int c, const float* pm,
                                       void* update, int nscan, int pw, int chi_modes,
                                       void* stream) {
  TK_ENTER();
  TK_CHECK_ARG(nscan >= 0 && pw >= 1 && num_eigen >= 1 && c >= 0 && c < num_eigen &&
               chi_modes >= 1);
  if (nscan == 0) return TK_OK;
  TK_CHECK_ARG(patches && chi0 && mpu0 && eigen_probe && pm && update && (c == 0 || coefs));
  const long P = (long)pw * pw;
  float* part = nullptr;
  const int chunk = probe_chunk(nscan, 2 * P, &part);
  dim3 grid((unsigned)((P + 255) / 256), (unsigned)((nscan + chunk - 1) / chunk));
  const TkResidual R = make_residual(patches, chi0, mpu0, eigen_probe, coefs, num_eigen,
                                     eigen_modes, c, pw, chi_modes);
  if (c == 0)
    hipLaunchKernelGGL(eigen_pixel_update_kernel<true>, grid, dim3(256), 0, (hipStream_t)stream,
                       R, pm, (float*)update, nscan, chunk, part);
  else
    hipLaunchKernelGGL(eigen_pixel_update_kernel<false>, grid, dim3(256), 0,
                       (hipStream_t)stream, R, pm, (float*)update, nscan, chunk, part);
  TK_LAUNCH_CHECK();
  if (part != nullptr)
    return tk_ordered_sum((float*)update, part, 2 * P, (int)grid.y, true, (hipStream_t)stream);
  return TK_OK;
}

extern "C" int tike_eigen_pixel_update1(const void* patches, const void* chi0,
                                        const void* mpu0, const void* eigen0,
                                        const float* eigen_proj, const float* weights_c,
                                        long weights_row, const float* norm, void* update,
                                        int nscan, int pw, int chi_modes, const float* stats,
                                        const float* costs, float eps, float* sums3,
                                        const void* psi, const float* scan, int H, int W,
                                        void* stream) {
  TK_ENTER();
  TK_CHECK_ARG(nscan >= 0 && pw >= 1 && chi_modes >= 1 && weights_row >= 1);
  if (nscan == 0) {
    if (sums3) return (int)hipMemsetAsync(sums3, 0, 3 * sizeof(float), (hipStream_t)stream);
    return TK_OK;
  }
  TK_CHECK_ARG(!sums3 || (stats && costs));
  TK_CHECK_ARG(!psi || (scan && H >= 1 && W >= 1));
  TK_CHECK_ARG(patches && chi0 && mpu0 && eigen0 && eigen_proj && weights_c && norm && update);
  const long P = (long)pw * pw;
  float* part = nullptr;
  const int chunk = probe_chunk(nscan, 2 * P, &part);
  dim3 grid((unsigned)((P + 255) / 256) + 1, (unsigned)((nscan + chunk - 1) / chunk));
  const TkResidual R = make_residual(patches, chi0, mpu0, eigen0, nullptr, 1, 1, 0, pw, chi_modes);
  hipLaunchKernelGGL(eigen_pixel_update1_kernel, grid, dim3(256), 0, (hipStream_t)stream, R,
                     eigen_proj, weights_c, weights_row, norm, 1.0f / (float)P, (float*)update,
                     nscan, chunk, stats, costs, eps, sums3, (const cf*)psi, scan, pw, H, W,
                     part);
  TK_LAUNCH_CHECK();
  if (part != nullptr)
    return tk_ordered_sum((float*)update, part, 2 * P, (int)grid.y, true, (hipStream_t)stream);
  return TK_OK;
}

extern "C" int tike_eigen_position_sums1(const void* patches, const void* chi0,
                                         const void* mpu0, const void* eigen0, float* sums,
                                         float* dsum, int nscan, int pw, int chi_modes,
                                         const void* psi, const float* scan, int H, int W,
                                         void* stream) {
  TK_ENTER();
  TK_CHECK_ARG(nscan >= 0 && pw >= 1 && chi_modes >= 1);
  if (nscan == 0) return TK_OK;
  TK_CHECK_ARG(!psi || (scan && H >= 1 && W >= 1));
  TK_CHECK_ARG(patches && chi0 && mpu0 && eigen0 && sums && dsum);
  const TkResidual R = make_residual(patches, chi0, mpu0, eigen0, nullptr, 1, 1, 0, pw, chi_modes);
  const bool det = tk_deterministic();
  const int cols = pw < 256 ? pw : 256;
  const bool pairs = g_stats_pairs && psi != nullptr && nscan > 1 &&
                     (pw % 256 == 0 || 256 % pw == 0) && pw % (512 / cols) == 0 &&
                     (long)H * W < (1L << 28);
  if (pairs)
    hipLaunchKernelGGL(eigen_position_sums1_pair_kernel, dim3(tk_grid((nscan + 1) / 2, 16)),
                       dim3(512), 0, (hipStream_t)stream, R, sums, det ? nullptr : dsum, nscan,
                       (const cf*)psi, scan, pw, H, W);
  else
    hipLaunchKernelGGL(eigen_position_sums1_kernel, dim3(tk_grid(nscan, 16)), dim3(256), 0,
                       (hipStream_t)stream, R, sums, det ? nullptr : dsum, nscan, (const cf*)psi,
                       scan, pw, H, W);
  if (det)
    hipLaunchKernelGGL(column_sum_ordered_kernel, dim3(1), dim3(256), 0, (hipStream_t)stream, sums,
                       5, 2, nscan, 1.0f / (float)((long)pw * pw), dsum);
  TK_LAUNCH_CHECK();
  return TK_OK;
}

__global__ __launch_bounds__(256) void varying_probe_kernel(const TkProbe probe,
                                                            cf* __restrict__ out, long total,
                                                            long PP) {
  for (long i = blockIdx.x * (long)blockDim.x + threadIdx.x; i < total;
       i += (long)gridDim.x * blockDim.x) {
    const long pix = i % PP;
    const long ns = i / PP;
    out[i] = probe.at(ns / probe.Sm, (int)(ns % probe.Sm), pix);
  }
}

extern "C" int tike_varying_probe(const void* probe, const void* eigen_probe,
                                  const float* eigen_weights, int num_eigen, int eigen_modes,
                                  void* out, int nscan, int S, int pw, void* stream) {
  TK_ENTER();
  TK_CHECK_ARG(nscan >= 0 && S >= 1 && pw >= 1 && eigen_modes >= 1 && eigen_modes <= S);
  if (nscan == 0) return TK_OK;
  TK_CHECK_ARG(probe && eigen_weights && out && (num_eigen == 0 || eigen_probe));
  const long PP = (long)pw * pw;
  const long total = (long)nscan * eigen_modes * PP;
  hipLaunchKernelGGL(varying_probe_kernel, dim3(tk_grid((total + 255) / 256, 16)), dim3(256), 0,
                     (hipStream_t)stream,
                     tk_make_probe(probe, 0, eigen_probe, eigen_weights, num_eigen, eigen_modes,
                                   S, pw),
                     (cf*)out, total, PP);
  TK_LAUNCH_CHECK();
  return TK_OK;
}

struct TkTaps {
  float t[9];
  int r;
};

template <int RT>
__global__ __launch_bounds__(256) void position_sums_kernel(
    const cf* __restrict__ patches, const cf* __restrict__ chi, int chi_modes,
    const TkProbe probe, const TkTaps taps, float* __restrict__ num, float* __restrict__ den,
    int pw, int nsplit) {
  __shared__ float red[4];
  const long n = blockIdx.x / nsplit;
  const int part = blockIdx.x % nsplit;
  const long P = (long)pw * pw;
  const cf* __restrict__ O = patches + n * P;
  const cf* __restrict__ X = chi + n * chi_modes * P;
  const int crop = pw / 4;
  const int w = pw - 2 * crop;
  float a[4] = {0.f, 0.f, 0.f, 0.f};
  const int ilen = (w * w + nsplit - 1) / nsplit;
  const int iend = min(w * w, (part + 1) * ilen);
  for (int i = part * ilen + threadIdx.x; i < iend; i += blockDim.x) {
    const int y = crop + i / w, x = crop + i % w;
    cf gx = mk(0.f, 0.f), gy = mk(0.f, 0.f);
    const long pix = (long)y * pw + x;
    const cf Pm = probe.at(n, 0, pix);
    const cf c = X[pix];
    auto tap = [&](int d, int r) {
      const float t = taps.t[d + r];
      int yy = y + d, xx = x + d;
      yy = yy < 0 ? 0 : (yy >= pw ? pw - 1 : yy);
      xx = xx < 0 ? 0 : (xx >= pw ? pw - 1 : xx);
      const cf oy = O[yy * pw + x], ox = O[y * pw + xx];
      gx.x += t * oy.x;
      gx.y += t * oy.y;
      gy.x += t * ox.x;
      gy.y += t * ox.y;
    };
    if (RT >= 0) {
#pragma unroll
      for (int d = -RT; d <= RT; ++d) tap(d, RT);
    } else {
      for (int d = -taps.r; d <= taps.r; ++d) tap(d, taps.r);
    }
    const cf px = gx * Pm, py = gy * Pm;
    a[0] += px.x * c.x + px.y * c.y;
    a[1] += py.x * c.x + py.y * c.y;
    a[2] += norm2(px);
    a[3] += norm2(py);
  }
  for (int k = 0; k < 4; ++k) a[k] = tk_block_sum256(a[k], red);
  if (threadIdx.x == 0) {
    if (nsplit > 1) {
      unsafeAtomicAdd(&num[2 * n], a[0]);
      unsafeAtomicAdd(&num[2 * n + 1], a[1]);
      unsafeAtomicAdd(&den[2 * n], a[2]);
      unsafeAtomicAdd(&den[2 * n + 1], a[3]);
    } else {
      num[2 * n] = a[0];
      num[2 * n + 1] = a[1];
      den[2 * n] = a[2];
      den[2 * n + 1] = a[3];
    }
  }
}

__global__ __launch_bounds__(256) void position_sums_pair_kernel(
    const cf* __restrict__ patches, const cf* __restrict__ chi, int chi_modes,
    const TkProbe probe, const TkTaps taps, float* __restrict__ num, float* __restrict__ den,
    int pw, int nscan, int nsplit) {
  __shared__ float red[4];
  typedef float tk_v4f __attribute__((ext_vector_type(4)));
  const long P = (long)pw * pw;
  const int crop = pw / 4;
  const int w = pw - 2 * crop;
  const int cols = w < 256 ? w : 256, groups = 256 / cols, rows = w / (nsplit * groups);
  const int npair = (nscan + 1) / 2;
  const bool shared = probe.weights == nullptr && probe.pos_stride == 0;
  const float t0 = taps.t[0], t1 = taps.t[1], t2 = taps.t[2], t3 = taps.t[3], t4 = taps.t[4];
  auto ld16 = [](const cf* p) {
    tk_v4f v;
    __builtin_memcpy(&v, p, sizeof(v));
    return v;
  };
  auto add = [&](float* a, const cf (&v)[5], const tk_v4f hl, const tk_v4f hr, const cf Pm,
                 const cf c) {
    cf gx = mk(t0 * v[0].x, t0 * v[0].y), gy = mk(t0 * hl.x, t0 * hl.y);
// ... 137 lines not shown
```

tike_amd/csrc/solver.hip:

```cpp
#include "internal.h"
#include "tike_amd.h"

__global__ __launch_bounds__(256) void object_update_precond_kernel(
    const float* __restrict__ acc, const cf* __restrict__ precond,
    const float* __restrict__ pmax, float alpha, cf* __restrict__ upd_sum,
    cf* __restrict__ upd_precond, float* __restrict__ combined, long npix) {
  const float am = alpha * pmax[0];
  for (long i = blockIdx.x * 256L + threadIdx.x; i < npix; i += gridDim.x * 256L) {
    const float re = acc[i], im = acc[npix + i];
    const float p = (1.0f - alpha) * precond[i].x;
    const float inv = 1.0f / sqrtf(p * p + am * am);
    if (upd_sum) upd_sum[i] = mk(re, im);
    if (upd_precond) upd_precond[i] = mk(re * inv, im * inv);
    if (combined) {
      combined[i] += re;
      combined[npix + i] += im;
    }
  }
}

extern "C" int tike_object_update_precond(const float* acc, const void* precond,
                                          const float* pmax, float alpha, void* upd_sum,
                                          void* upd_precond, float* combined, long npix,
                                          void* stream) {
// ... 228 lines not shown
                     (const cf*)update, (float)(1.0 / count), beta, npix, work);
  if (esum) hipLaunchKernelGGL(eigen_normalise_finish_kernel, dim3(1), dim3(1), 0, st, work, esum);
  TK_LAUNCH_CHECK();
  return TK_OK;
}

__global__ __launch_bounds__(256) void eigen_dsum_kernel(const float* __restrict__ sums, int B,
                                                         float inv_P, float* __restrict__ dsum) {
  __shared__ float red[4];
  float a = 0.f;
  for (int n = threadIdx.x; n < B; n += 256) a += sums[5 * n + 2] * inv_P;
  a = tk_block_sum256(a, red);
  if (threadIdx.x == 0) dsum[0] = a;
}

__global__ __launch_bounds__(256) void eigen_weights_kernel(const float* __restrict__ sums, int B,
                                                            float inv_P,
                                                            const float* __restrict__ dsum,
                                                            float inv_count,
                                                            float* __restrict__ weights_c,
                                                            long row, cf* __restrict__ coefs_c,
                                                            int coef_stride,
                                                            const float* __restrict__ esum) {
  const int n = blockIdx.x * 256 + threadIdx.x;
  if (n >= B) return;
  const float* s = sums + 5 * n;
  const float d_mean = dsum[0] * inv_count;
  weights_c[n * row] += (s[1] * inv_P) / (s[2] * inv_P + 0.1f * d_mean);
  if (coefs_c) {
    const float inv = 1.0f / esum[0];
    coefs_c[(long)n * coef_stride] = mk(s[3] * inv, s[4] * inv);
  }
}

extern "C" int tike_eigen_dsum(const float* sums, int B, long P, float* dsum, void* stream) {
  TK_ENTER();
  TK_CHECK_ARG(B >= 0 && P > 0 && dsum && (B == 0 || sums));
  hipLaunchKernelGGL(eigen_dsum_kernel, dim3(1), dim3(256), 0, (hipStream_t)stream, sums, B,
                     1.0f / (float)P, dsum);
  TK_LAUNCH_CHECK();
  return TK_OK;
}

extern "C" int tike_eigen_weights(const float* sums, int B, long P, const float* dsum,
                                  double count, float* weights_c, long weights_row,
                                  void* coefs_c, int coef_stride, const float* esum,
                                  void* stream) {
  TK_ENTER();
  TK_CHECK_ARG(B >= 0 && P > 0 && count > 0);
  if (B == 0) return TK_OK;
  TK_CHECK_ARG(sums && dsum && weights_c && (!coefs_c || esum));
  hipLaunchKernelGGL(eigen_weights_kernel, dim3((B + 255) / 256), dim3(256), 0,
                     (hipStream_t)stream, sums, B, 1.0f / (float)P, dsum, (float)(1.0 / count),
                     weights_c, weights_row, (cf*)coefs_c, coef_stride, esum);
  TK_LAUNCH_CHECK();
  return TK_OK;
}


__global__ __launch_bounds__(256) void lstsq_tail_mid_kernel(
    const cf* __restrict__ E, const cf* __restrict__ update, int npix, float* __restrict__ nacc,
    const float* __restrict__ stats, int B, float eps, const float* __restrict__ sums3,
    float inv_count, int recover_psi, int recover_probe, float* __restrict__ tail3,
    float* __restrict__ part) {
  __shared__ float red[4];
  if (blockIdx.x + 1 < gridDim.x) {
    float uu = 0.f, ee = 0.f, eu = 0.f;
    for (int i = blockIdx.x * 256 + threadIdx.x; i < npix; i += (gridDim.x - 1) * 256) {
      const cf e = E[i], u = update[i];
      uu += norm2(u);
      ee += norm2(e);
      eu += e.x * u.x + e.y * u.y;
    }
    uu = tk_block_sum256(uu, red);
    ee = tk_block_sum256(ee, red);
    eu = tk_block_sum256(eu, red);
    if (threadIdx.x == 0) {
      if (part != nullptr) {
        part[3 * blockIdx.x] = uu;
        part[3 * blockIdx.x + 1] = ee;
        part[3 * blockIdx.x + 2] = eu;
      } else {
        unsafeAtomicAdd(&nacc[0], uu);
        unsafeAtomicAdd(&nacc[1], ee);
        unsafeAtomicAdd(&nacc[2], eu);
      }
    }
    return;
  }
  const float r1 = 0.5f * sums3[0] * inv_count, r4 = 0.5f * sums3[1] * inv_count;
  float so = 0.f, sp = 0.f;
  for (int n = threadIdx.x; n < B; n += 256) {
    const float* s = stats + 8 * n;
    const float A1 = s[0] + eps + r1, A4 = s[1] + eps + r4;
    const float b1 = s[4], b2 = s[5];
    float x1 = 0.f, x2 = 0.f;
    if (recover_psi && recover_probe) {
      const float det = A1 * A4 - (s[2] * s[2] + s[3] * s[3]);
      x1 = -(s[2] * b2 - A4 * b1) / det;
      x2 = (A1 * b2 - s[2] * b1) / det;
    } else if (recover_psi) {
      x1 = b1 / A1;
    } else if (recover_probe) {
      x2 = b2 / A4;
    }
    so += 0.9f * fmaxf(x1, 0.f);
    sp += 0.9f * fmaxf(x2, 0.f);
  }
  so = tk_block_sum256(so, red);
  sp = tk_block_sum256(sp, red);
  if (threadIdx.x == 0) {
    tail3[0] = so;
    tail3[1] = sp;
  }
}

__global__ __launch_bounds__(256) void eigen_apply1_kernel(cf* __restrict__ E,
                                                           const cf* __restrict__ update,
                                                           const float* __restrict__ nacc,
                                                           float inv_count, float beta,
                                                           int npix) {
  const float uu = nacc[0], ee = nacc[1], eu = nacc[2];
  const float mu = sqrtf(uu * inv_count * inv_count / (float)npix);
  const float k = beta / mu * inv_count;
  const float inv = 1.0f / sqrtf((ee + 2.0f * k * eu + k * k * uu) / (float)npix);
  for (int i = blockIdx.x * 256 + threadIdx.x; i < npix; i += gridDim.x * 256)
    E[i] = (E[i] + update[i] * k) * inv;
}

extern "C" int tike_lstsq_tail_mid(void* eigen0, const void* update, int npix, float* nacc,
                                   float beta_eigen, const float* stats, int B, float eps,
                                   const float* sums3, double count, int recover_psi,
                                   int recover_probe, float* tail3, void* stream) {
  TK_ENTER();
  TK_CHECK_ARG(B >= 0 && count > 0 && sums3 && tail3 && (B == 0 || stats));
  TK_CHECK_ARG(!eigen0 || (update && nacc && npix >= 1));
  int grid = !eigen0 ? 0 : (npix >= 256 * 64 ? 64 : (npix + 255) / 256);
  float* part = nullptr;
  if (grid > 0 && tk_deterministic()) {
    part = tk_det_scratch(sizeof(float) * 3 * (size_t)grid);
    if (part == nullptr) grid = 1;
  }
  hipLaunchKernelGGL(lstsq_tail_mid_kernel, dim3(grid + 1), dim3(256), 0, (hipStream_t)stream,
                     (const cf*)eigen0, (const cf*)update, npix, nacc, stats, B, eps, sums3,
                     (float)(1.0 / count), recover_psi, recover_probe, tail3, part);
  if (part != nullptr) {
    int rc = tk_ordered_sum(nacc, part, 3, grid, true, (hipStream_t)stream);
    if (rc) return rc;
  }
  if (eigen0)
    hipLaunchKernelGGL(eigen_apply1_kernel, dim3(grid), dim3(256), 0, (hipStream_t)stream,
                       (cf*)eigen0, (const cf*)update, nacc, (float)(1.0 / count), beta_eigen,
                       npix);
  TK_LAUNCH_CHECK();
  return TK_OK;
}

__global__ __launch_bounds__(256) void lstsq_tail_finish_kernel(
    const float* __restrict__ tail3, const float* __restrict__ sums3, float inv_count,
    float* __restrict__ steps, cf* __restrict__ probe, cf* __restrict__ combined,
    const cf* __restrict__ mpu, float inv_num_batch, long nprobe, float* __restrict__ weights,
    long row, int S, int m, const float* __restrict__ stats, const float* __restrict__ sums5,
    int B, int npix) {
  const float bp = tail3[1] * inv_count;
  const long stride = (long)gridDim.x * 256;
  const long i0 = blockIdx.x * 256L + threadIdx.x;
  if (i0 == 0) {
    steps[0] = tail3[0];
    steps[1] = tail3[1];
    steps[2] = tail3[0] * inv_count;
    steps[3] = bp;
    steps[4] = sums3[2] * inv_count;
  }
  if (probe != nullptr) {
    for (long i = i0; i < nprobe; i += stride) {
      const cf d = mpu[i] * bp;
      probe[i] = probe[i] + d;
      if (combined) combined[i] = combined[i] + d * inv_num_batch;
    }
  }
  if (weights != nullptr) {
    const float inv_P = 1.0f / (float)npix;
    const float d_mean = sums5 ? tail3[2] * inv_count : 0.f;
    for (long n = i0; n < B; n += stride) {
      weights[n * row + m] += 0.1f * stats[8 * n + 6] / stats[8 * n + 7];
      if (sums5) {
        const float* s = sums5 + 5 * n;
        weights[n * row + S + m] += (s[1] * inv_P) / (s[2] * inv_P + 0.1f * d_mean);
      }
    }
  }
}

extern "C" int tike_lstsq_tail_finish(const float* tail3, const float* sums3, double count,
                                      float* steps, void* probe, void* combined, const void* mpu,
                                      float inv_num_batch, long nprobe, float* weights,
                                      long weights_row, int S, int m, const float* stats,
                                      const float* sums5, int B, int npix, void* stream) {
  TK_ENTER();
  TK_CHECK_ARG(tail3 && sums3 && steps && count > 0 && B >= 0 && nprobe >= 0 && npix >= 0);
  TK_CHECK_ARG(!probe || mpu);
  if (B == 0) {
    weights = nullptr;
    sums5 = nullptr;
  }
  TK_CHECK_ARG(!weights || (stats && weights_row >= 1 && S >= 1 && m >= 0 && m < S));
  TK_CHECK_ARG(!sums5 || (weights && weights_row >= 2L * S && npix >= 1));
  long work = 1;
  if (probe && nprobe > work) work = nprobe;
  if (weights && B > work) work = B;
  hipLaunchKernelGGL(lstsq_tail_finish_kernel, dim3(tk_grid((work + 255) / 256, 8)), dim3(256), 0,
                     (hipStream_t)stream, tail3, sums3, (float)(1.0 / count), steps, (cf*)probe,
                     (cf*)combined, (const cf*)mpu, inv_num_batch, nprobe, weights, weights_row,
                     S, m, stats, sums5, B, npix);
  TK_LAUNCH_CHECK();
  return TK_OK;
}

extern "C" int tike_lstsq_chunk_gradients(
    const void* psi, const float* scan, const void* probe, const void* eigen_probe,
    const float* eigen_weights, int num_eigen, int eigen_modes, const void* data, int data_u16,
    const unsigned char* measured, int model, float unmeasured_scaling, long num_measured,
    void* scratch, void* work, float* gscale, void* patches, float* costs, void* objproj,
    void* chi0, void* m_probe_update, float mpu_scale, float* object_acc, int nscan, int S,
    int det, int H, int W, float fwd_scale, float inv_scale, void* stream) {
  TK_ENTER();
  TK_CHECK_ARG(nscan >= 0 && S >= 1 && H >= 1 && W >= 1);
  if (nscan == 0) return TK_OK;
  TK_CHECK_ARG(psi && scan && probe && data && scratch && work && patches);
  TK_CHECK_ARG(scratch != work && (object_acc == nullptr) == (objproj == nullptr));
  if (!((det == 128 && S <= 8) || (det == 256 && S <= 8) || (det == 512 && S <= 4)))
    return TK_ERR_UNSUPPORTED;
  TK_CHECK_ARG(gscale || det == 256);
  if (det == 128) {
    if (data_u16 || (eigen_weights && eigen_modes > 0)) return TK_ERR_UNSUPPORTED;
    float* inten = gscale + (size_t)nscan * det * det;
    int rc = tike_ptycho_fwd_intensity(psi, scan, probe, 0, nullptr, eigen_weights, num_eigen,
                                       eigen_modes, scratch, inten, patches, nscan, S, det, det,
                                       H, W, fwd_scale, stream);
    if (rc) return rc;
    rc = tike_gradient_scale(inten, (const float*)data, measured, gscale, costs, nscan, det,
                             model, unmeasured_scaling, num_measured, stream);
    if (rc) return rc;
    rc = tike_ifft2_pass1_scaled(scratch, gscale, nullptr, nullptr, S, work, (long)nscan * S, det,
                                 stream);
    if (rc) return rc;
    rc = tike_ifft2_pass2_gradients(work, patches, probe, eigen_probe, eigen_weights, num_eigen,
                                    eigen_modes, objproj, chi0, m_probe_update, mpu_scale, nscan,
                                    S, det, inv_scale, stream);
    if (rc) return rc;
    if (object_acc) rc = tike_scatter_patches(objproj, scan, object_acc, nscan, det, H, W, stream);
    return rc;
  }
  int rc = tike_fwd_pass1(psi, scan, probe, 0, nullptr, eigen_probe, eigen_weights, num_eigen,
                          eigen_modes, scratch, patches, nscan, S, det, det, H, W, stream);
  if (rc) return rc;
  if (det == 256) {
    rc = tike_fwd_grad_ifft2_pass1(scratch, data, data_u16, measured, costs, work, nscan, S, det,
                                   fwd_scale, model, unmeasured_scaling, num_measured, stream);
  } else {
    rc = tike_fwd_gradient_scale(scratch, data, data_u16, measured, gscale, nullptr, costs,
                                 nullptr, nscan, S, det, fwd_scale, model, unmeasured_scaling,
                                 num_measured, stream);
    if (rc) return rc;
    rc = tike_grad_ifft2_pass1(scratch, gscale, nullptr, nullptr, S, work, (long)nscan * S, det,
                               fwd_scale, stream);
  }
  if (rc) return rc;
  rc = tike_ifft2_pass2_gradients(work, patches, probe, eigen_probe, eigen_weights, num_eigen,
                                  eigen_modes, objproj, chi0, m_probe_update, mpu_scale, nscan,
                                  S, det, inv_scale, stream);
  if (rc) return rc;
  if (object_acc) rc = tike_scatter_patches(objproj, scan, object_acc, nscan, det, H, W, stream);
  return rc;
}
```

tike_amd/ptycho/solvers/_plan.py:

```python
from dataclasses import dataclass
from types import SimpleNamespace

import torch

from ... import _arrays as A
from ..._lib import check, lib

MODELS = {"gaussian": 0, "poisson": 1}


def algorithmic_bytes(name, n, S, det, pw, C, depth=1):
    T = 8 * S * det * det
    Tw = 8 * S * pw * det
    P = 8 * pw * pw
    D = 4 * det * det
    box = 8 * (pw + 1) * (pw + 1)
    table = {
        "tike_fwd_pass1": n * (T + 2 * P + 8) + (S + C) * P,
        "tike_fwd_gradient_scale": n * (T + 2 * D),
        "tike_fwd_pass1:cost_only": n * (T + P + 8) + (S + C) * P,
        "tike_fwd_gradient_scale:cost_only": n * (T + D + 4),
        "tike_ptycho_fwd_gradient_scale":
        n * (T + P + 2 * D + 8) + (S + C) * P,
        "tike_ptycho_fwd_intensity": n * (T + P + D + 8) + (S + C) * P,
# ... 14 lines not shown
        "tike_farplane_gradient": n * (2 * T + D + 4),
        "tike_ifft2_crop": n * (T + S * P),
        "tike_lstsq_gradients": n * (S * P + 2 * P),
        "tike_scatter_patches": n * (P + box),
        "tike_lstsq_step_stats": n * (3 * P + 32),
        "tike_gen_fwd_rows": n * (Tw + 2 * P + 8) + (S + C) * P,
        "tike_gen_cols_gradient": n * (2 * Tw + D),
        "tike_gen_inv_rows_gradients": n * (Tw + 3 * P) + S * P,
        "tike_pfa_fwd_gather": n * (T + 2 * P + 8) + (S + C) * P,
        "tike_pfa_fft2": n * 2 * T,
        "tike_pfa_combine_gradient": n * (2 * T + D),
        "tike_pfa_inv_products": n * (T + 3 * P) + S * P,
        "tike_fwd_pass1:no_patches": n * (T + P + 8) + (S + C) * P,
        "tike_fwd_pass1:incident": n * (2 * T + P + 8),
        "tike_fresnel_colpass": n * 2 * T + D * 2,
        "tike_fft2_pass2_inplace": n * 2 * T,
        "tike_fft2_pass2_intensity": n * (T + D),
        "tike_fwd_grad_ifft2_pass1_slices": n * (T + D + depth * T),
        "tike_ifft2_pass2_products": n * (T + 3 * P) + S * P,
        "tike_ifft2_pass2_products:incident": n * (2 * T + 2 * P),
    }
    return table.get(name, 0)


@dataclass(frozen=True)
class GradientPlan:
    det: int
    pw: int
    S: int
    model: int
    poisson: bool
    dominant: int
    all_modes: bool
    masked: bool
    route: str
    fused: bool
    general: bool
    pfa: bool
    pos_major: bool
    no_farplane: bool
    split_kept: bool
    one_launch: bool
    steps_in_pass2: bool
    chunk: int
    launches: tuple
    groups: tuple = ()

    def bytes(self, entry, n, C=0):
        return algorithmic_bytes(entry, n, self.S, self.det, self.pw, C)

    @staticmethod
    def for_(op, S, pw, det, exitwave_options, mask_u8, eigen_modes=0,
             num_eigen=0):
        from . import lstsq as L
        eo = exitwave_options
        unmeasured = float(eo.unmeasured_pixels_scaling)
        from ... import _lib
        key = (_lib.DETERMINISTIC, S, pw, det, eo.noise_model,
               eo.step_length_usemodes,
               mask_u8 is not None, unmeasured == 1.0,
               tuple(L.POSITION_MAJOR_SIZES), tuple(L.NO_FARPLANE_SIZES),
               tuple(L.SPLIT_FORWARD_SIZES), tuple(L.ONE_LAUNCH_GRADIENT_SIZES),
               L.POISSON_FROM_HANDOFF, L.POISSON_STEPS_IN_PASS2,
               L.GENERAL_FUSED, L.PFA_ROUTE, L.GENERAL_MIN_DETECTOR,
               L.CHUNK_POSITIONS_OVERRIDE,
               L.mode_groups(S, pw, det, eigen_modes),
               bool(lib.tike_ifft2_pass2_eigen_fits(det, num_eigen,
                                                    eigen_modes)))
        cache = op.__dict__.setdefault("_tike_amd_plans", {})
        if key not in cache:
            cache[key] = GradientPlan._build(S, pw, det, eo, mask_u8, unmeasured,
                                             L, eigen_modes, key[-1])
        return cache[key]

    @staticmethod
    def _build(S, pw, det, eo, mask_u8, unmeasured, L, eigen_modes=0,
               eigen_fits=True):
        poisson = eo.noise_model == "poisson"
        dominant = int(poisson and eo.step_length_usemodes == "dominant_mode")
        all_modes = poisson and not dominant
        pos_major = det in L.POSITION_MAJOR_SIZES
        fused = L.fused_gradients(S, pw, det)
        groups = () if fused or poisson else L.mode_groups(S, pw, det,
                                                           eigen_modes)
        fused = (fused or bool(groups)) and eigen_fits
        groups = groups if fused else ()
        general = (not fused
                   and (not pos_major or L.GENERAL_FUSED == "always")
                   and not poisson and L.general_gradients(S, pw, det))
        pfa = general and L.pfa_gradients(S, pw, det)
        if (pfa and S == 1 and det < 256 and L.GENERAL_FUSED != "always"):
            pfa = general = False
        if (general and not pfa and det < L.GENERAL_MIN_DETECTOR
                and L.GENERAL_FUSED != "always"):
            general = False
        if general:
            pos_major = False
        from ... import _lib
        handoff_steps = L.POISSON_FROM_HANDOFF and not _lib.DETERMINISTIC
        no_farplane = (pos_major
                       and (det in L.NO_FARPLANE_SIZES or (det == 512 and fused))
                       and not (all_modes and not (fused and handoff_steps)))
        split_kept = (pos_major and fused and not no_farplane
                      and det in L.SPLIT_FORWARD_SIZES)
        one_launch = (no_farplane and fused and not poisson
                      and det in L.ONE_LAUNCH_GRADIENT_SIZES)
        steps_in_pass2 = (no_farplane and all_modes and fused and det == 256
                          and (mask_u8 is None or unmeasured == 1.0)
                          and L.POISSON_STEPS_IN_PASS2)
        route = ("pfa" if pfa else "general" if general else
                 "no_farplane" if no_farplane else
                 "split_kept" if split_kept else "pos_major" if pos_major else
                 "unfused")
        launches = {
            "general": ("tike_gen_fwd_rows", "tike_gen_cols_gradient",
                        "tike_gen_inv_rows_gradients"),
            "pfa": ("tike_pfa_fwd_gather", "tike_pfa_fft2",
                    "tike_pfa_combine_gradient", "tike_pfa_fft2",
                    "tike_pfa_inv_products"),
            "no_farplane": ("tike_fwd_pass1",) + (
                ("tike_poisson_steps_grad_ifft2_pass1",) if steps_in_pass2 else
                ("tike_poisson_steps_handoff", "tike_grad_ifft2_pass1")
                if all_modes else ("tike_fwd_grad_ifft2_pass1",) if one_launch
                else ("tike_fwd_gradient_scale",
                      "tike_grad_ifft2_pass1" if fused else
                      "tike_grad_ifft2_crop")) + (
                ("tike_ifft2_pass2_gradients_scaled" if steps_in_pass2 else
                 "tike_ifft2_pass2_gradients",) if fused else
                ("tike_lstsq_gradients",)),
            "split_kept": ("tike_fwd_pass1", "tike_fwd_gradient_scale",
                           "tike_ifft2_pass1_scaled",
                           "tike_ifft2_pass2_gradients"),
            "pos_major": ("tike_ptycho_fwd_intensity", "tike_gradient_scale",
                          "tike_ifft2_pass1_scaled" if fused else
                          "tike_ifft2_crop_scaled",
                          "tike_ifft2_pass2_gradients" if fused else
                          "tike_lstsq_gradients"),
            "unfused": ("tike_ptycho_fwd", "tike_farplane_gradient",
                        "tike_ifft2_crop", "tike_lstsq_gradients"),
        }[route] + ("tike_scatter_patches",)
        return GradientPlan(
            det=det, pw=pw, S=S, model=MODELS[eo.noise_model], poisson=poisson,
            dominant=dominant, all_modes=all_modes, masked=mask_u8 is not None,
            route=route, fused=fused, general=general, pfa=pfa,
            pos_major=pos_major,
            no_farplane=no_farplane, split_kept=split_kept,
            one_launch=one_launch, steps_in_pass2=steps_in_pass2,
            chunk=L.chunk_positions(S, det, pos_major or general),
            launches=tuple("tike_ifft2_pass2_gradients_modes"
                           if groups and e == "tike_ifft2_pass2_gradients" else e
                           for e in launches),
            groups=groups)

    def buffers(self, ws, B, dev, *, varying, want_patches):
        S, pw, det = self.S, self.pw, self.det
        n = min(self.chunk, max(B, 1))
        c64, f32 = torch.complex64, torch.float32
        b = SimpleNamespace(inten=None, gscale=None, steps=None, unique=None,
                            patches=None, sums=None)
        if want_patches or self.fused or self.general:
            b.patches = ws.get("patches", (max(B, 1), pw, pw), c64, dev)
        b.costs = ws.get("costs", (max(B, 1),), f32, dev)
        if self.pos_major or self.poisson:
            b.inten = ws.get("intensity", (n, det, det), f32, dev)
        if self.pos_major:
            b.gscale = ws.get("gscale", (n, det, det), f32, dev)
        if self.poisson:
            b.steps = ws.get("steps", (n, S), f32, dev)
            if self.all_modes and self.no_farplane:
                b.sums = ws.get("poisson_sums", (n, S, 2), f32, dev)
        b.objproj = ws.get("objproj", (n, pw, pw), c64, dev)
        if varying and not self.general:
            b.unique = ws.get("unique", (n, varying, pw, pw), c64, dev)
        b.far = ws.get("far", (n, 1, S, pw if self.general and not self.pfa
                               else det, det), c64, dev)
        b.mid = ws.get("mid", tuple(b.far.shape), c64, dev)
        b.chi = b.mid
        if pw != det and not self.general:
            b.chi = ws.get("chi", (n, 1, S, pw, pw), c64, dev)
        b.single_chunk = B <= self.chunk and not self.fused and not self.general
        b.chi0 = (None if b.single_chunk else
                  ws.get("chi0", (max(B, 1), pw, pw), c64, dev))
        return b

    def forward(self, c, k):
        getattr(self, "_forward_" + self.route)(c, k)

    def _forward_pfa(self, c, k):
        b = c.buf
        from . import lstsq as L
        if L.PFA_SUBTILES_IN_LDS and lib.tike_pfa_fwd_subtiles_supported(
                self.S, self.pw, self.det):
            psub = L._workspace(c.op).get(
                "pfa_probe", (self.S + c.C * c.Sm, self.det, self.det),
                torch.complex64, c.psi.device)
            check(
                lib.tike_pfa_fwd_subtiles(
                    A.ptr(c.psi), A.ptr(k.scan), A.ptr(c.probe), A.ptr(c.ep),
                    A.ptr(k.w), c.C, c.Sm, A.ptr(psub), A.ptr(b.mid),
                    A.ptr(k.patches), k.n, self.S, self.pw, self.det, c.H,
                    c.W, c.st), "prime-factor gather + sub-tile transforms")
        else:
            check(
                lib.tike_pfa_fwd_gather(
                    A.ptr(c.psi), A.ptr(k.scan), A.ptr(c.probe), 0, None,
                    A.ptr(c.ep), A.ptr(k.w), c.C, c.Sm, A.ptr(b.far),
                    A.ptr(k.patches), k.n, self.S, self.pw, self.det, c.H,
                    c.W, c.st), "prime-factor gather")
            check(lib.tike_pfa_fft2(A.ptr(b.far), A.ptr(b.mid), k.n * self.S,
                                    self.det, 0, c.st), "sub-tile transforms")
        check(
            lib.tike_pfa_combine_gradient(
                A.ptr(b.mid), A.ptr(k.data_f32()), A.ptr(c.mask_u8),
                A.ptr(k.costs), k.n, self.S, self.det, c.fwd_scale, self.model,
                c.unmeasured, c.nmeasured, 1, c.st),
            "p x p combine + gradient")
        check(lib.tike_pfa_fft2(A.ptr(b.mid), A.ptr(b.far), k.n * self.S,
                                self.det, 1, c.st),
              "inverse sub-tile transforms")

    def _forward_general(self, c, k):
        b = c.buf
        check(
            lib.tike_gen_fwd_rows(
                A.ptr(c.psi), A.ptr(k.scan), A.ptr(c.probe), 0, None,
                A.ptr(c.ep), A.ptr(k.w), c.C, c.Sm, A.ptr(b.far),
                A.ptr(k.patches), k.n, self.S, self.pw, self.det, c.H, c.W,
                c.st), "general forward rows")
        check(
            lib.tike_gen_cols_gradient(
                A.ptr(b.far), A.ptr(k.data_f32()), A.ptr(c.mask_u8),
                A.ptr(k.costs), A.ptr(b.mid), k.n, self.S, self.pw, self.det,
                c.fwd_scale, self.model, c.unmeasured, c.nmeasured, c.st),
            "general columns + gradient")

    def _forward_no_farplane(self, c, k):
        b, S, det, pw = c.buf, self.S, self.det, self.pw
        n, st = k.n, c.st
        u16 = int(c.data.dtype == torch.uint16)
        check(
            lib.tike_fwd_pass1(
                A.ptr(c.psi), A.ptr(k.scan), A.ptr(c.probe), 0, None,
                A.ptr(c.ep), A.ptr(k.w), c.C, c.Sm, A.ptr(b.far),
                A.ptr(k.patches) if self.fused else None, n, S, pw, det, c.H,
                c.W, st), "forward pass 1")
        if self.steps_in_pass2:
            check(
                lib.tike_poisson_steps_grad_ifft2_pass1(
                    A.ptr(b.far), A.ptr(k.data), u16, A.ptr(c.mask_u8),
                    A.ptr(k.costs), A.ptr(b.steps), A.ptr(b.sums),
                    A.ptr(b.mid), n, S, det, c.fwd_scale, c.unmeasured,
                    c.nmeasured, c.step_start, c.step_weight, st),
                "poisson step lengths + gradient + inverse pass 1")
            return
        if self.all_modes:
            check(
                lib.tike_poisson_steps_handoff(
                    A.ptr(b.far), A.ptr(k.data), u16, A.ptr(c.mask_u8),
                    A.ptr(b.gscale), A.ptr(k.costs), A.ptr(b.steps),
                    A.ptr(b.sums), n, S, det, c.fwd_scale, c.unmeasured,
                    c.nmeasured, c.step_start, c.step_weight, st),
                "forward pass 2 + poisson factor and step lengths")
        elif self.one_launch:
            check(
                lib.tike_fwd_grad_ifft2_pass1(
                    A.ptr(b.far), A.ptr(k.data), u16, A.ptr(c.mask_u8),
                    A.ptr(k.costs), A.ptr(b.mid), n, S, det, c.fwd_scale,
                    self.model, c.unmeasured, c.nmeasured, st),
                "column pass + gradient + inverse pass 1")
            return
        else:
            check(
                lib.tike_fwd_gradient_scale(
                    A.ptr(b.far), A.ptr(k.data), u16, A.ptr(c.mask_u8),
                    A.ptr(b.gscale), A.ptr(b.inten) if self.poisson else None,
                    A.ptr(k.costs), None, n, S, det, c.fwd_scale, self.model,
                    c.unmeasured, c.nmeasured, st),
                "forward pass 2 + gradient scale")
        if self.poisson and self.dominant:
            check(
                lib.tike_poisson_steps(
                    None, A.ptr(b.inten), A.ptr(k.data_f32()),
                    A.ptr(c.mask_u8), A.ptr(b.steps), n, S, det, c.step_start,
                    c.step_weight, 1, st), "poisson step lengths")
        steps = A.ptr(b.steps) if self.poisson else None
        smask = A.ptr(c.mask_u8) if self.poisson else None
        if self.fused:
            check(
                lib.tike_grad_ifft2_pass1(A.ptr(b.far), A.ptr(b.gscale), steps,
                                          smask, S, A.ptr(b.mid), n * S, det,
                                          c.fwd_scale, st),
                "gradient + inverse pass 1")
        else:
            check(
                lib.tike_grad_ifft2_crop(A.ptr(b.far), A.ptr(b.gscale), steps,
                                         smask, S, A.ptr(b.mid), A.ptr(b.chi),
                                         n * S, det, pw, c.fwd_scale,
                                         c.inv_scale, st),
                "gradient + ifft2 + crop")

    def _forward_split_kept(self, c, k):
        b, S, det, pw = c.buf, self.S, self.det, self.pw
        n, st, d = k.n, c.st, k.data_f32()
        check(
            lib.tike_fwd_pass1(
                A.ptr(c.psi), A.ptr(k.scan), A.ptr(c.probe), 0, A.ptr(k.uq),
                None, A.ptr(k.w), c.C, c.Sm, A.ptr(b.far), A.ptr(k.patches), n,
                S, pw, det, c.H, c.W, st), "forward pass 1")
        check(
            lib.tike_fwd_gradient_scale(
                A.ptr(b.far), A.ptr(d), 0, A.ptr(c.mask_u8), A.ptr(b.gscale),
                A.ptr(b.inten) if self.poisson else None, A.ptr(k.costs),
                A.ptr(b.mid), n, S, det, c.fwd_scale, self.model, c.unmeasured,
                c.nmeasured, st), "forward pass 2 + gradient scale")
        if self.poisson:
            check(
                lib.tike_poisson_steps(
                    A.ptr(b.mid), A.ptr(b.inten), A.ptr(d), A.ptr(c.mask_u8),
                    A.ptr(b.steps), n, S, det, c.step_start, c.step_weight,
                    self.dominant, st), "poisson step lengths")
        check(
            lib.tike_ifft2_pass1_scaled(
                A.ptr(b.mid), A.ptr(b.gscale),
                A.ptr(b.steps) if self.poisson else None,
                A.ptr(c.mask_u8) if self.poisson else None, S, A.ptr(b.far),
                n * S, det, st), "scaled inverse pass 1")

    def _forward_pos_major(self, c, k):
        b, S, det, pw = c.buf, self.S, self.det, self.pw
        n, st, d = k.n, c.st, k.data_f32()
        check(
            lib.tike_ptycho_fwd_intensity(
                A.ptr(c.psi), A.ptr(k.scan), A.ptr(c.probe), 0, A.ptr(k.uq),
                A.ptr(k.w), c.C, c.Sm, A.ptr(b.far), A.ptr(b.inten),
                A.ptr(k.patches) if self.fused else None, n, S, pw, det, c.H,
                c.W, c.fwd_scale, st), "forward + intensity")
        check(
            lib.tike_gradient_scale(A.ptr(b.inten), A.ptr(d), A.ptr(c.mask_u8),
                                    A.ptr(b.gscale), A.ptr(k.costs), n, det,
                                    self.model, c.unmeasured, c.nmeasured, st),
            "gradient scale")
        if self.poisson:
            check(
                lib.tike_poisson_steps(
                    A.ptr(b.far), A.ptr(b.inten), A.ptr(d), A.ptr(c.mask_u8),
                    A.ptr(b.steps), n, S, det, c.step_start, c.step_weight,
                    self.dominant, st), "poisson step lengths")
        if self.fused:
            check(
                lib.tike_ifft2_pass1_scaled(
                    A.ptr(b.far), A.ptr(b.gscale),
                    A.ptr(b.steps) if self.poisson else None,
                    A.ptr(c.mask_u8) if self.poisson else None, S,
                    A.ptr(b.mid), n * S, det, st), "scaled inverse pass 1")
        elif self.poisson:
            check(
                lib.tike_ifft2_crop_scaled_modes(
                    A.ptr(b.far), A.ptr(b.gscale), A.ptr(b.steps),
                    A.ptr(c.mask_u8), S, A.ptr(b.mid), A.ptr(b.chi), n * S,
                    det, pw, c.inv_scale, st), "scaled ifft2 + crop (poisson)")
        else:
            check(
                lib.tike_ifft2_crop_scaled(A.ptr(b.far), A.ptr(b.gscale), S,
                                           A.ptr(b.mid), A.ptr(b.chi), n * S,
                                           det, pw, c.inv_scale, st),
                "scaled ifft2 + crop")

    def _forward_unfused(self, c, k):
        b, S, det, pw = c.buf, self.S, self.det, self.pw
        n, st, d = k.n, c.st, k.data_f32()
        c.op.fwd_device(c.probe, k.scan, c.psi, c.eigen_probe, k.w,
                        out=b.far[:n])
        if self.poisson:
            check(lib.tike_intensity(A.ptr(b.far), A.ptr(b.inten), n, S,
                                     det * det, st), "intensity")
            check(
                lib.tike_poisson_steps(
                    A.ptr(b.far), A.ptr(b.inten), A.ptr(d), A.ptr(c.mask_u8),
                    A.ptr(b.steps), n, S, det, c.step_start, c.step_weight,
                    self.dominant, st), "poisson step lengths")
        check(
            lib.tike_farplane_gradient(
                A.ptr(b.far), A.ptr(d), A.ptr(c.mask_u8), None, A.ptr(k.costs),
                n, S, det, self.model, 1, c.unmeasured, c.nmeasured, st),
            "farplane gradient")
        if self.poisson:
            check(
                lib.tike_scale_modes(A.ptr(b.far), A.ptr(b.steps),
                                     A.ptr(c.mask_u8), n * S, det, st),
                "poisson step scaling")
        check(
            lib.tike_ifft2_crop(A.ptr(b.far), A.ptr(b.mid), A.ptr(b.chi), n * S,
                                det, pw, c.inv_scale, st), "ifft2 + crop")

    def gradients(self, c, k):
        b, S, det, pw = c.buf, self.S, self.det, self.pw
        n, st = k.n, c.st
        objproj = A.ptr(b.objproj) if c.recover_psi else None
        chi0 = A.ptr(k.chi0) if c.need_chi0 and k.chi0 is not None else None
        if self.pfa:
            check(
                lib.tike_pfa_inv_products(
                    A.ptr(b.far), A.ptr(k.patches), A.ptr(c.probe), 0, None,
                    A.ptr(c.ep), A.ptr(k.w), c.C, c.Sm, objproj, chi0,
                    A.ptr(c.m_probe_update), 1.0 / c.num_batch, n, S, pw, det,
                    c.inv_scale, st), "prime-factor inverse products")
        elif self.general:
            check(
                lib.tike_gen_inv_rows_gradients(
                    A.ptr(b.mid), A.ptr(k.patches), A.ptr(c.probe), 0, None,
                    A.ptr(c.ep), A.ptr(k.w), c.C, c.Sm, objproj, chi0,
                    A.ptr(c.m_probe_update), 1.0 / c.num_batch, n, S, pw, det,
                    c.inv_scale, st), "general inverse rows + gradients")
        elif self.fused:
            p2 = (A.ptr(b.far if self.split_kept else b.mid), A.ptr(k.patches),
                  A.ptr(c.probe), A.ptr(c.ep), A.ptr(k.w), c.C, c.Sm, objproj,
                  chi0, A.ptr(c.m_probe_update), 1.0 / c.num_batch, n, S, det,
                  c.inv_scale)
            if self.groups:
                for first, count in self.groups:
                    check(lib.tike_ifft2_pass2_gradients_modes(
                        *p2, first, count, int(first > 0), st),
                        "inverse pass 2 + gradients (a group of modes)")
            elif self.steps_in_pass2:
                check(lib.tike_ifft2_pass2_gradients_scaled(
                    *p2, A.ptr(b.steps), st),
                    "inverse pass 2 + gradients (x poisson steps)")
            else:
                check(lib.tike_ifft2_pass2_gradients(*p2, st),
                      "inverse pass 2 + gradients")
        else:
            check(
                lib.tike_lstsq_gradients(
                    A.ptr(b.chi), A.ptr(k.scan), A.ptr(c.psi), A.ptr(c.probe),
                    A.ptr(c.ep), A.ptr(k.w), c.C, c.Sm,
                    None,
                    A.ptr(k.patches), A.ptr(c.m_probe_update), objproj, n, S,
                    pw, c.H, c.W, st), "probe gradient + object projection")
```

tike_amd/ptycho/solvers/lstsq.py:

```python
import logging
from types import SimpleNamespace

import numpy as np
import torch

from ... import _arrays as A
from ... import _tuning
from ... import linalg
from ... import opt
from ... import random as trandom
from ..._lib import check, lib
from ...operators.propagation import fft_scales
from ..position import gaussian_derivative_taps
from ._plan import GradientPlan

logger = logging.getLogger(__name__)

_MODELS = {"gaussian": 0, "poisson": 1}


class _Workspace:

    def __init__(self):
        self.buffers = {}
# ... 49 lines not shown
modes, detector sizes with factors 3 / 5 / 7 ...) run the three general
launches of csrc/general.hip (tike_gen_*; gaussian model) instead of the
unfused round-1 kernels; tests set this to False to compare the two."""


GENERAL_MIN_DETECTOR = 1 << 30
"""Detector sizes below this (and without a prime-factor decomposition) keep
the unfused kernels.  Late in round 6 that is every size: with 384, 768 and
1024 -- the sizes where the LDS line engine's three launches were 10 ... 17 %
ahead -- on the prime-factor kernels, what is left to it loses to the unfused
kernels on the mixed-radix transforms or ties with them (300^2 x 1 ... 8 modes
-43 ... -6 %, 400^2 +-0, 500^2 x 4 +7 %, 600^2 x 2 -12 %, 720^2 x 4 -15 %, 1000^2
x 1 ... 4 -3 ... -25 %; with an eigen probe -14 ... +7 %:
profiles/r06_experiments.md section 17).  The launches stay in the tree and
in the tests (`GENERAL_FUSED = "always"`); 256 restores round 6's first rule."""

PFA_ROUTE = True
"""Detector sizes 3 x 2^k, 5 x 2^k and 7 x 2^k (96 ... 3584), and 1024 / 2048, without position-major
kernels take the prime-factor launches of csrc/pfa.hip (tike_pfa_*): the
power-of-two register engine on p x p sub-tiles; tests set this to False to
compare with the LDS line engine of csrc/general.hip."""


MODE_GROUPS = True
"""More modes than one launch of the inverse's second pass holds in registers
(9 ... 32 at 128^2 / 256^2, 5 ... 16 at 512^2; probe window = detector,
gaussian model) run the far-plane-free kernels with that pass in groups of
modes (tike_ifft2_pass2_gradients_modes); False: the position-major kernels
with a stored far plane, as until round 6."""


def mode_groups(S, pw, det, eigen_modes=0):
    cap = 4 if det == 512 else 8
    if not (MODE_GROUPS and pw == det and det in POSITION_MAJOR_SIZES
            and cap < S <= 4 * cap):
        return ()
    k = -(-S // cap)
    base, extra = divmod(S, k)
    sizes = [base + (i < extra) for i in range(k)]
    if min(sizes) < 2 or eigen_modes > sizes[0]:
        return ()
    firsts = [sum(sizes[:i]) for i in range(k)]
    return tuple(zip(firsts, sizes))


PFA_SUBTILES_IN_LDS = True
"""Prime-factor sizes with 128^2 sub-tiles (384, 640, 896): gather and forward
sub-tile transform in one launch, the sub-tile inside LDS
(tike_pfa_fwd_subtiles); False: tike_pfa_fwd_gather + tike_pfa_fft2."""


def pfa_gradients(S, pw, det):
    return bool(PFA_ROUTE and lib.tike_pfa_supported(S, pw, det))


def general_gradients(S, pw, det):
    return bool(GENERAL_FUSED and lib.tike_gen_supported(S, pw, det))


def fused_gradients(S, pw, det):
    return (pw == det and det in POSITION_MAJOR_SIZES
            and S <= (4 if det == 512 else 8))


def chunk_positions(S, det, position_major=False):
    if CHUNK_POSITIONS_OVERRIDE:
        return max(1, int(CHUNK_POSITIONS_OVERRIDE))
    tiles = max(2048, (1 << 33) // (det * det * 8))
    if position_major:
        return max(1024, tiles // max(S, 1))
    return max(64, tiles // max(S, 1))


def global_count(comm, op, lo, hi):
    cache = op.__dict__.setdefault("_tike_amd_counts", {})
    key = minibatch_key(comm, lo, hi)
    if key not in cache:
        cache[key] = comm.Allreduce_count(hi - lo)
    return cache[key]


def minibatch_key(comm, lo, hi):
    return (getattr(comm, "minibatch", None), lo, hi, comm.size)


def mask_info(exitwave_options, det=None):
    mask = exitwave_options.measured_pixels
    if det is not None and tuple(mask.shape) != (det, det):
        raise ValueError(
            f"measured_pixels shape {tuple(mask.shape)} does not match the "
            f"detector ({det}, {det})")
    key = (id(mask), tuple(mask.shape))
    cached = exitwave_options.__dict__.get("_mask_info")
    if cached is None or cached[0] != key:
        m = mask if A.is_device(mask) else A.to_device(
            np.asarray(mask, dtype=bool))
        n = int(m.sum().item())
        info = (n, None if n == m.numel() else m.to(torch.uint8).contiguous())
        cached = (key, info)
        exitwave_options.__dict__["_mask_info"] = cached
    return cached[1]


def lstsq_grad(parameters, data, batches, comm, *, op, epoch):
    scan = parameters.scan
    psi = parameters.psi
    probe = parameters.probe
    algorithm_options = parameters.algorithm_options
    eigen_weights = parameters.eigen_weights
    eigen_probe = parameters.eigen_probe
    exitwave_options = parameters.exitwave_options
    object_options = parameters.object_options
    probe_options = parameters.probe_options
    position_options = parameters.position_options
    if exitwave_options.noise_model not in _MODELS:
        raise ValueError(
            f"unknown noise model {exitwave_options.noise_model!r}")
    recover_probe = (probe_options is not None
                     and epoch >= probe_options.update_start)
    recover_psi = object_options is not None
    num_batch = algorithm_options.num_batch
    compact = algorithm_options.batch_method == "compact"
    order = (range(num_batch) if compact else
             trandom.randomizer_np.permutation(num_batch))
    if hasattr(data, "hint"):
        data.hint([_lo_hi(batches[b]) for b in order])

    dev = psi.device
    H, W = psi.shape[-2:]
    object_combined = (torch.zeros((2, H, W), dtype=torch.float32, device=dev)
                       if recover_psi and compact else None)
    probe_combined_update = torch.zeros_like(probe)
    steps = torch.zeros((num_batch, 5), dtype=torch.float32, device=dev)
    pmax = None
    if recover_psi:
        pmax = torch.amax(object_options.preconditioner.real).reshape(
            1).contiguous()
    beta_object, beta_probe = [], []
    position_terms = None
    if position_options is not None:
        position_terms = (torch.zeros_like(scan), torch.zeros_like(scan))
    packed = PACKED_TAIL and (eigen_probe is None
                              or eigen_probe.shape[-4] == 1)
    eigen_norms = None
    if (packed and recover_probe and eigen_weights is not None
            and eigen_probe is not None):
        eigen_norms = torch.stack([
            torch.square(eigen_weights[_lo_hi(b)[0]:_lo_hi(b)[1], 1, 0]).sum()
            for b in batches
        ]).to(torch.float32).contiguous()
        if comm.collective:
            comm.Allreduce(eigen_norms)

    for batch_index in order:
        lo, hi = _lo_hi(batches[batch_index])
        comm.minibatch = int(batch_index)
        g = _get_nearplane_gradients(
            data, psi, scan, probe, eigen_probe, eigen_weights, lo, hi, comm,
            num_batch=num_batch, exitwave_options=exitwave_options, op=op,
            recover_psi=recover_psi, recover_probe=recover_probe,
            position_terms=position_terms)

        object_update_precond = None
        if recover_psi:
            object_update_precond = _precondition_object_update(
                g["object_acc"], object_options.preconditioner, pmax=pmax,
                combined=object_combined)
        if packed:
            bbeta_object, bbeta_probe = _packed_tail(
                g, psi, scan, probe, eigen_probe, eigen_weights,
                object_update_precond, lo, hi, comm, op=op,
                num_batch=num_batch, recover_psi=recover_psi,
                recover_probe=recover_probe,
                norm=None if eigen_norms is None else
                eigen_norms[batch_index:batch_index + 1],
                steps_row=steps[batch_index],
                probe_combined_update=probe_combined_update)
        else:
            stats = _step_stats(g, psi, scan, probe, eigen_probe,
                                object_update_precond, lo, hi, op=op)

            if recover_probe and eigen_weights is not None:
                eigen_probe, eigen_weights = _update_nearplane(
                    g, stats, probe, eigen_probe, eigen_weights, lo, hi, comm,
                    num_batch=num_batch)

            bbeta_object, bbeta_probe, _ = _solve_steps(
                stats, g["costs"], g["count"], comm, pw=probe.shape[-1],
                recover_psi=recover_psi, recover_probe=recover_probe,
                out=steps[batch_index])

        if recover_psi:
            if not compact:
                dpsi = bbeta_object * object_update_precond
                if object_options.use_adaptive_moment:
                    dpsi, object_options.v, object_options.m = opt.momentum(
                        g=dpsi, v=object_options.v, m=object_options.m,
                        vdecay=object_options.vdecay,
                        mdecay=object_options.mdecay)
                psi = psi + dpsi
            beta_object.append(bbeta_object)

        if recover_probe:
            if not packed:
                check(
                    lib.tike_probe_update(A.ptr(probe),
                                          A.ptr(probe_combined_update),
                                          A.ptr(g["m_probe_update"]),
                                          A.ptr(bbeta_probe), 1.0 / num_batch,
                                          probe.numel(), A.stream_ptr()),
                    "probe update")
            beta_probe.append(bbeta_probe)

    batch_cost = steps[:, 4]
    if position_options is not None:
        scan = _update_position(scan, position_options, *position_terms, comm,
                                epoch=epoch)

    algorithm_options.costs.append([float(batch_cost.mean().item())])
    if (eigen_weights is not None and eigen_weights.shape[1] > 1
            and not np.isfinite(algorithm_options.costs[-1][0])):
        nonzero = torch.stack([
            (eigen_weights[int(idx[0]):int(idx[0]) + len(idx), 1:, 0]
             != 0).sum(dim=0).to(torch.float32) if len(idx) else torch.zeros(
                 eigen_weights.shape[1] - 1, device=psi.device)
            for idx in batches
        ])
        if comm.collective:
            comm.Allreduce(nonzero)
        if bool((nonzero == 0).any().item()):
            raise ValueError("eigen_probe weights cannot all be zero?")

    if recover_psi and compact:
        object_update_precond = _precondition_object_update(
            object_combined, object_options.preconditioner, pmax=pmax)
        bo = torch.mean(torch.stack(beta_object))
        dpsi = bo * object_update_precond
        psi = psi + dpsi
        if object_options.use_adaptive_moment:
            dpsi, object_options.v, object_options.m = _momentum_checked(
                g=dpsi, v=object_options.v, m=object_options.m,
                mdecay=object_options.mdecay,
                errors=[float(x[0]) for x in algorithm_options.costs[-3:]],
                beta=bo, memory_length=3)
            weight = object_options.preconditioner
            weight = weight / (0.1 * weight.real.max() + weight)
            psi = psi + weight * dpsi

    if recover_probe and probe_options.use_adaptive_moment:
        bp = torch.mean(torch.stack(beta_probe))
        dprobe = probe_combined_update
        if probe_options.v is None:
            probe_options.v = torch.zeros((3, *dprobe.shape),
                                          dtype=dprobe.dtype,
                                          device=dprobe.device)
        if probe_options.m is None:
            probe_options.m = torch.zeros_like(dprobe)
        mode = 0
        (d, probe_options.v[..., mode, :, :],
         probe_options.m[..., mode, :, :]) = _momentum_checked(
             g=dprobe[..., mode, :, :], v=probe_options.v[..., mode, :, :],
             m=probe_options.m[..., mode, :, :], mdecay=probe_options.mdecay,
             errors=[float(x[0]) for x in algorithm_options.costs[-3:]],
             beta=bp, memory_length=3)
        probe[..., mode, :, :] = probe[..., mode, :, :] + d

    parameters.scan = scan
    parameters.psi = psi
    parameters.probe = probe
    parameters.eigen_weights = eigen_weights
    parameters.eigen_probe = eigen_probe
    return parameters


EIGEN_PATCH_RECOMPUTE = True
"""The eigen pixel update of the packed tail gathers the object patches from
psi (L2) instead of streaming the stored ones (HBM): 0.186 -> 0.160 ms per 1000
positions at 256^2.  (With two 16-byte tap loads per pixel the position sums
lost by it, 0.215 -> 0.221 ms; see EIGEN_SUMS_RECOMPUTE.)"""

EIGEN_SUMS_RECOMPUTE = _tuning.eigen_sums_gather
"""The position sums gather too, through the two-positions-per-workgroup row
walk of tike_eigen_position_sums1 (one 16-byte tap load per pixel and
position, E_0 and the probe update loaded once per pair): 0.215 -> 0.176 ms
per 1000 positions at 256^2."""

STATS_PATCH_RECOMPUTE = _tuning.stats_gather
"""The step statistics gather O_n from the object with the two 16-byte tap
loads they already issue for the preconditioned update (same offsets)."""

PACKED_TAIL = True
"""Tests set this to False to run the staged tail (one entry per step of the
reference's _update_nearplane / _precondition_nearplane_gradients)."""


def _lo_hi(batch):
    lo = int(batch[0]) if len(batch) else 0
    return lo, lo + len(batch)


def _eigen_args(eigen_probe, weights):
    if weights is None:
        return None, None, 0, 0
    C = Sm = 0
    if eigen_probe is not None:
        C, Sm = eigen_probe.shape[-4], eigen_probe.shape[-3]
    assert weights.shape[1] == C + 1, (weights.shape, C)
    return eigen_probe, weights, C, Sm


def _once(make):
    box = []

    def get():
        if not box:
            box.append(make())
        return box[0]

    return get


def _get_nearplane_gradients(data, psi, scan, probe, eigen_probe,
                             eigen_weights, lo, hi, comm, *, num_batch,
                             exitwave_options, op, recover_psi, recover_probe,
                             position_terms=None, need_chi0=True):
    dev = psi.device
    B = hi - lo
    S, pw = probe.shape[-3], probe.shape[-1]
    det = op.detector_shape
    H, W = psi.shape[-2:]
    if exitwave_options.noise_model not in _MODELS:
        raise ValueError(
            f"unknown noise model {exitwave_options.noise_model!r}")
    nmeasured, mask_u8 = mask_info(exitwave_options, det)
    fwd_scale, inv_scale = fft_scales(det, op.norm)

    w_old = None if eigen_weights is None else eigen_weights[lo:hi]
    ep, _, C, Sm = _eigen_args(eigen_probe, w_old)
    plan = GradientPlan.for_(op, S, pw, det, exitwave_options, mask_u8,
                             eigen_modes=Sm, num_eigen=C)

    n_obj = 2 * H * W if recover_psi else 0
    n_prb = 2 * probe.numel() if recover_probe else 0
    grads = torch.zeros(n_obj + n_prb, dtype=torch.float32, device=dev)
    obj_acc = grads[:n_obj].view(2, H, W) if recover_psi else None
    m_probe_update = (torch.view_as_complex(
        grads[n_obj:].view(*probe.shape, 2)) if recover_probe else None)
    probe_sum = None
    early = bool(comm.collective and recover_psi and recover_probe)
    buf = plan.buffers(
        _workspace(op), B, dev, varying=Sm if w_old is not None else 0,
        want_patches=bool((recover_probe and eigen_weights is not None)
                          or position_terms))
    if position_terms:
        taps, taps_r = gaussian_derivative_taps(sigma=0.333)
    c = SimpleNamespace(
        op=op, data=data, psi=psi, probe=probe, ep=ep, eigen_probe=eigen_probe,
        C=C, Sm=Sm, H=H, W=W, st=A.stream_ptr(), fwd_scale=fwd_scale,
        inv_scale=inv_scale, nmeasured=nmeasured, mask_u8=mask_u8,
        unmeasured=float(exitwave_options.unmeasured_pixels_scaling),
        step_start=float(exitwave_options.step_length_start),
        step_weight=float(exitwave_options.step_length_weight), buf=buf,
        m_probe_update=m_probe_update, num_batch=num_batch,
        recover_psi=recover_psi, need_chi0=need_chi0)
    chunk = plan.chunk
    for clo in range(lo, hi, chunk):
        chi_hi = min(hi, clo + chunk)
        n, blo = chi_hi - clo, clo - lo
        rows = slice(blo, blo + n)
        k = SimpleNamespace(
            n=n, scan=scan[clo:chi_hi], data=data[clo:chi_hi],
            w=None if w_old is None else w_old[rows], uq=None,
            costs=buf.costs[rows],
            patches=None if buf.patches is None else buf.patches[rows],
            chi0=None if buf.chi0 is None else buf.chi0[rows])
        k.data_f32 = _once(lambda a=clo, b=chi_hi: A.data_f32(data, a, b))
        if k.w is not None and Sm > 0 and buf.unique is not None and (
                not plan.no_farplane):
            k.uq = buf.unique[:n]
            check(
                lib.tike_varying_probe(A.ptr(probe), A.ptr(ep), A.ptr(k.w), C,
                                       Sm, A.ptr(k.uq), n, S, pw, c.st),
                "varying probe")
        plan.forward(c, k)
        plan.gradients(c, k)
        stored_chi0 = plan.fused or plan.general
        if position_terms:
            chi_m, chi_modes = ((k.chi0, 1) if stored_chi0 else (buf.chi, S))
            check(
                lib.tike_position_sums(
                    A.ptr(k.patches), A.ptr(chi_m), chi_modes, A.ptr(probe),
                    A.ptr(ep), A.ptr(k.w), C, Sm, taps.ctypes.data, taps_r,
                    A.ptr(position_terms[0][clo:chi_hi]),
                    A.ptr(position_terms[1][clo:chi_hi]), n, S, pw, c.st),
                "position shift sums")
        if chi_hi == hi and early:
            probe_sum = comm.Allreduce_start(grads[n_obj:])
        if recover_psi:
            check(
                lib.tike_scatter_patches(A.ptr(buf.objproj), A.ptr(k.scan),
                                         A.ptr(obj_acc), n, pw, H, W, c.st),
                "object scatter")
        if not buf.single_chunk and not stored_chi0:
            buf.chi0[rows] = buf.chi[:n, 0, 0]

    if comm.collective and grads.numel():
        if early:
            if probe_sum is None:
                probe_sum = comm.Allreduce_start(grads[n_obj:])
            comm.Allreduce(grads[:n_obj])
            probe_sum.wait()
        else:
            comm.Allreduce(grads)
    count = global_count(comm, op, lo, hi)
    if recover_probe and not (plan.fused or plan.general):
        m_probe_update = m_probe_update / num_batch
    return dict(chi0=buf.chi if buf.single_chunk else buf.chi0[:B],
                chi_modes=S if buf.single_chunk else 1, w_old=w_old,
                patches=None if buf.patches is None else buf.patches[:B],
                object_acc=obj_acc, m_probe_update=m_probe_update,
                costs=buf.costs[:B], count=count, local_count=B)


def object_upd_sum(g):
    acc = g["object_acc"]
    return None if acc is None else torch.complex(acc[0], acc[1])[None]


def _precondition_object_update(object_acc, psi_update_denominator,
                                alpha=0.05, *, pmax=None, combined=None):
    H, W = object_acc.shape[-2:]
    if pmax is None:
        pmax = torch.amax(psi_update_denominator.real).reshape(1).contiguous()
    out = torch.empty((1, H, W), dtype=torch.complex64,
                      device=object_acc.device)
    check(
        lib.tike_object_update_precond(A.ptr(object_acc),
                                       A.ptr(psi_update_denominator),
                                       A.ptr(pmax), alpha, None, A.ptr(out),
                                       A.ptr(combined), H * W, A.stream_ptr()),
        "preconditioned object update")
    return out


def _step_stats(g, psi, scan, probe, eigen_probe, object_update_precond, lo,
                hi, *, op):
    B = hi - lo
    dev = psi.device
    S, pw = probe.shape[-3], probe.shape[-1]
    stats = _workspace(op).get("stats", (max(B, 1), 8), torch.float32, dev)
    ep, w_old, C, Sm = _eigen_args(eigen_probe, g["w_old"])
    eigen0 = eproj = None
    if (ep is not None and C >= 1 and Sm >= 1 and g["patches"] is not None
            and g["m_probe_update"] is not None):
        eigen0 = ep[0, 0, 0]
        eproj = _workspace(op).get("eigen_proj", (max(B, 1),), torch.float32,
                                   dev)
    g["eigen_proj"] = None if eproj is None else eproj[:B]
    check(
        lib.tike_lstsq_step_stats(
            A.ptr(g["chi0"]), A.ptr(scan[lo:hi]), A.ptr(psi),
            A.ptr(object_update_precond), A.ptr(probe), A.ptr(ep),
            A.ptr(w_old), C, Sm, None, A.ptr(g["m_probe_update"]),
            None if (STATS_PATCH_RECOMPUTE and psi.shape[0] == 1
                     and object_update_precond is not None) else
            A.ptr(g["patches"]), A.ptr(stats), B,
            S, g["chi_modes"], pw, psi.shape[-2], psi.shape[-1],
            A.ptr(eigen0), A.ptr(eproj), A.stream_ptr()),
        "step-size statistics")
    return stats[:B]


def _packed_tail(g, psi, scan, probe, eigen_probe, eigen_weights,
                 object_update_precond, lo, hi, comm, *, op, num_batch,
                 recover_psi, recover_probe, norm, steps_row,
                 probe_combined_update):
    B = hi - lo
    dev = psi.device
    st = A.stream_ptr()
    S, pw = probe.shape[-3], probe.shape[-1]
    P = pw * pw
    count = float(g["count"])
    ws = _workspace(op)
    eig = recover_probe and eigen_weights is not None
    C = Sm = 0
    if eig and eigen_probe is not None:
        C, Sm = eigen_probe.shape[-4], eigen_probe.shape[-3]
        assert eigen_weights.shape[-2] == C + 1 and C == 1
    mpu = g["m_probe_update"]
    one = (eig and C == 1 and Sm >= 1 and g["patches"] is not None
           and mpu is not None and norm is not None)
    assert one or C == 0, "packed tail: eigen probe without its operands"
    small = ws.get("tail_small", (4 + 2 * P + 8,), torch.float32, dev)
    small.zero_()
    sums3 = small[:3]
    update = small[4:4 + 2 * P]
    nacc = small[4 + 2 * P:4 + 2 * P + 4]
    tail3 = small[4 + 2 * P + 4:4 + 2 * P + 7]
    stats = _step_stats(g, psi, scan, probe, eigen_probe,
                        object_update_precond, lo, hi, op=op)
    eps_total = float(np.float32(np.float32(1e-9) / P) * P)
    E = w_rows = sums5 = None
    row = 0
    if eig:
        w_rows = eigen_weights[lo:hi]
        row = w_rows.shape[-2] * w_rows.shape[-1]
    gpsi = A.ptr(psi[0]) if EIGEN_PATCH_RECOMPUTE and psi.shape[0] == 1 else None
    if one:
        E = eigen_probe[0, 0, 0]
        check(
            lib.tike_eigen_pixel_update1(
                A.ptr(g["patches"]), A.ptr(g["chi0"]), A.ptr(mpu[0, 0, 0]),
                A.ptr(E), A.ptr(g["eigen_proj"]), w_rows[:, 1, 0].data_ptr(),
                row, A.ptr(norm), A.ptr(update), B, pw, g["chi_modes"],
                A.ptr(stats), A.ptr(g["costs"]), eps_total, A.ptr(sums3),
                gpsi, A.ptr(scan[lo:hi]), psi.shape[-2], psi.shape[-1], st),
            "eigen pixel update")
    else:
        check(
            lib.tike_lstsq_step_sums(A.ptr(stats), A.ptr(g["costs"]), B,
                                     eps_total, A.ptr(sums3), st),
            "step-size sums")
    if comm.collective:
        comm.Allreduce(small[:4 + 2 * P] if one else small[:4])
    beta_eigen = min(0.1, 1.0 / num_batch)
    check(
        lib.tike_lstsq_tail_mid(A.ptr(E), A.ptr(update), P, A.ptr(nacc),
                                beta_eigen, A.ptr(stats), B, eps_total,
                                A.ptr(sums3), count, int(recover_psi),
                                int(recover_probe), A.ptr(tail3), st),
        "step solve")
    if one:
        sums5 = ws.get("eigen_sums5", (max(B, 1), 5), torch.float32, dev)
        check(
            lib.tike_eigen_position_sums1(
                A.ptr(g["patches"]), A.ptr(g["chi0"]), A.ptr(mpu[0, 0, 0]),
                A.ptr(E), A.ptr(sums5), tail3[2:].data_ptr(), B, pw,
                g["chi_modes"], gpsi if EIGEN_SUMS_RECOMPUTE else None,
                A.ptr(scan[lo:hi]), psi.shape[-2], psi.shape[-1], st),
            "eigen position sums")
    if comm.collective:
        comm.Allreduce(tail3)
    check(
        lib.tike_lstsq_tail_finish(
            A.ptr(tail3), A.ptr(sums3), count, A.ptr(steps_row),
            A.ptr(probe) if recover_probe else None,
            A.ptr(probe_combined_update) if recover_probe else None,
            A.ptr(mpu), 1.0 / num_batch, probe.numel(),
            None if w_rows is None else w_rows.data_ptr(), row, S, 0,
            A.ptr(stats), A.ptr(sums5), B, P, st), "minibatch tail")
    return (steps_row[2] if recover_psi else None,
            steps_row[3] if recover_probe else None)


def _solve_steps(stats, costs, count, comm, *, pw, recover_psi, recover_probe,
                 out=None):
    dev = stats.device
    B = stats.shape[0]
    st = A.stream_ptr()
    eps_total = float(np.float32(np.float32(1e-9) / (pw * pw)) * (pw * pw))
    if out is None:
        out = torch.zeros(5, dtype=torch.float32, device=dev)
    sums = torch.empty(3, dtype=torch.float32, device=dev)
    check(
        lib.tike_lstsq_step_sums(A.ptr(stats), A.ptr(costs), B, eps_total,
                                 A.ptr(sums), st), "step-size sums")
    if comm.collective:
        comm.Allreduce(sums)
    check(
        lib.tike_lstsq_step_solve(A.ptr(stats), B, eps_total, A.ptr(sums),
                                  float(count), int(recover_psi),
                                  int(recover_probe), A.ptr(out), st),
        "step-size solve")
    if comm.collective:
        comm.Allreduce(out[:2])
        out[2:4] = out[:2] / count
    return (out[2] if recover_psi else None,
            out[3] if recover_probe else None, out[4])


def _update_nearplane(g, stats, probe, eigen_probe, eigen_weights, lo, hi,
                      comm, *, num_batch):
    m = 0
    dev = probe.device
    count = float(g["count"])
    B = hi - lo
    st = A.stream_ptr()
    Cw, S = eigen_weights.shape[-2] - 1, eigen_weights.shape[-1]
    row = (Cw + 1) * S
    w_rows = eigen_weights[lo:hi]
    norms = torch.empty(max(Cw, 1), dtype=torch.float32, device=dev)
    check(
        lib.tike_eigen_weights0(A.ptr(w_rows), A.ptr(stats), B, Cw, S, m,
                                A.ptr(norms), st), "eigen weights (shared)")
    if Cw < 1 or eigen_probe is None:
        return eigen_probe, eigen_weights
    if m >= eigen_probe.shape[-3]:
        return eigen_probe, eigen_weights
    assert eigen_weights.shape[-2] == eigen_probe.shape[-4] + 1
    if comm.collective:
        comm.Allreduce(norms)
    chi0, patches = g["chi0"], g["patches"]
    mpu0 = g["m_probe_update"][0, 0, m]
    C, Sm, pw = eigen_probe.shape[-4], eigen_probe.shape[-3], probe.shape[-1]
    P = pw * pw
    beta = min(0.1, 1.0 / num_batch)
    sums = torch.empty((max(B, 1), 5), dtype=torch.float32, device=dev)
    coefs = torch.zeros((max(B, 1), C), dtype=torch.complex64, device=dev)
    pm = torch.empty(max(B, 1), dtype=torch.float32, device=dev)
    small = torch.empty(2, dtype=torch.float32, device=dev)
    nwork = torch.empty(4, dtype=torch.float32, device=dev)
    ep = eigen_probe

    def position_sums(c):
        check(
            lib.tike_eigen_position_sums(A.ptr(patches), A.ptr(chi0),
                                         A.ptr(mpu0), A.ptr(ep), A.ptr(coefs),
                                         C, Sm, c, A.ptr(sums), B, pw,
                                         g["chi_modes"], st),
            "eigen position sums")

    for c in range(1, C + 1):
        w_c = w_rows[:, c, m]
        if c == 1 and g.get("eigen_proj") is not None:
            first, stride = g["eigen_proj"], 1
        else:
            position_sums(c - 1)
            first, stride = sums, 5
        check(
            lib.tike_eigen_proj_mean(A.ptr(first), stride, w_c.data_ptr(), row,
                                     norms[c - 1:].data_ptr(), P, B,
                                     A.ptr(pm), st), "eigen projection mean")
        update = torch.zeros((pw, pw), dtype=torch.complex64, device=dev)
        check(
            lib.tike_eigen_pixel_update(A.ptr(patches), A.ptr(chi0),
                                        A.ptr(mpu0), A.ptr(ep), A.ptr(coefs),
                                        C, Sm, c - 1, A.ptr(pm),
                                        A.ptr(update), B, pw, g["chi_modes"],
                                        st),
            "eigen pixel update")
        if comm.collective:
            comm.Allreduce(update)
        E = ep[0, c - 1, m]
        check(
            lib.tike_eigen_normalise(A.ptr(E), A.ptr(update), count, beta, P,
                                     small[1:].data_ptr(), A.ptr(nwork), st),
            "eigen probe normalisation")
        position_sums(c - 1)
        check(lib.tike_eigen_dsum(A.ptr(sums), B, P, A.ptr(small), st),
              "eigen weight denominator")
        if comm.collective:
            comm.Allreduce(small[:1])
        more = c + 1 < eigen_weights.shape[-2]
        check(
            lib.tike_eigen_weights(A.ptr(sums), B, P, A.ptr(small), count,
                                   w_c.data_ptr(), row,
                                   coefs[:, c - 1:].data_ptr() if more else
                                   None, C, small[1:].data_ptr(), st),
            "eigen weights")
    return eigen_probe, eigen_weights


def _trimmed_mean(rows, proportion=0.05):
    count = rows.shape[0]
    cut = int(proportion * count)
    return torch.sort(rows, dim=0).values[cut:count - cut].mean(dim=0)


def _update_position(scan, position_options, numerator, denominator, comm,
                     *, alpha=0.05, epoch=0):
    po = position_options
    if epoch < po.update_start:
        return scan
    damping = alpha * torch.clamp(comm.Allreduce_max(denominator.max()),
                                  min=1e-6)
    shift = numerator / ((1 - alpha) * denominator + damping)
    limit = po.update_magnitude_limit
    if limit > 0:
        shift = shift.clamp(-limit, limit)
    shift -= _trimmed_mean(comm.Allgather_rows(shift))
    if po.use_adaptive_moment:
        moments = dict(vdecay=po.vdecay, mdecay=po.mdecay)
        shift, po.v, po.m = opt.adam(shift, po.v, po.m, **moments)
    return scan - shift


def _cost_is_falling(errors):
    return len(errors) >= 3 and max(errors[-3:-1]) > min(errors[-2:])


def _momentum_checked(g, v, m, mdecay, errors, beta=1.0, memory_length=3):
    memory = (g.new_zeros((memory_length, *g.shape)) if v is None else v)
    memory = torch.cat((memory[1:], (g / linalg.norm(g) * beta)[None]))
    total = torch.zeros_like(g) if m is None else m
    overlap = None
    if _cost_is_falling(errors):
        overlap = (memory[:-1] * memory[-1].conj()).real.sum(
            dim=(-2, -1)).flatten().cpu().numpy()
    if overlap is None or not (overlap > 0).all():
        return torch.zeros_like(g), memory, total / 2
    slope, _ = opt.fit_line_least_squares(
        x=np.arange(overlap.size + 1),
        y=np.concatenate(([0.0], np.log(overlap))))
# ... 3 lines not shown
```

Before: 213,400 patterns/s.

## Fuse eigen projection into pass 2 and merge step stats with eigen sums

Pass 2 of the inverse FFT now computes per-position partials of the eigen-probe projection, using wave DPP reductions into a small table that a finish kernel then reduces. A new fused tail runs the eigen pixel update first, then one kernel that computes both the step statistics and the eigen position sums in a single pass over chi and the patches, followed by a combined eigen and step solve. The aim is to remove separate passes over the patch and residual data and a few kernel launches per minibatch. The cost is added register and reduction work inside pass 2, more specialised code paths, and a reordered tail that is enabled by default for the single-rank, single-eigen-probe case.

```diff
diff --git a/include/tike_amd.h b/include/tike_amd.h
--- a/include/tike_amd.h
+++ b/include/tike_amd.h
@@ -10,7 +10,7 @@
 #define TIKE_ERR_COMM 2000000
 #define TIKE_COMM_ID_BYTES 128
 
-#define TIKE_ABI_VERSION 11
+#define TIKE_ABI_VERSION 12
 
 const char* tike_build_id(void);
 
@@ -354,6 +354,29 @@
                            const float* stats, const float* sums5, int B, int npix,
                            void* stream);
 
+int tike_ifft2_pass2_gradients_eproj(const void* work, const void* patches, const void* probe,
+                                     const void* eigen_probe, const float* eigen_weights,
+                                     int num_eigen, int eigen_modes, void* objproj, void* chi0,
+                                     void* m_probe_update, float mpu_scale, int nscan, int S,
+                                     int det, float inv_scale, float* qtab, float* q,
+                                     void* stream);
+int tike_eigen_pixel_update1q(const void* patches, const void* chi0, const void* mpu0,
+                              const void* eigen0, const float* q, const float* weights_c,
+                              long weights_row, const float* norm, void* update, int nscan,
+                              int pw, int chi_modes, const void* psi, const float* scan, int H,
+                              int W, float* c0part, float* eproj_out, void* stream);
+int tike_lstsq_step_stats_eigen1(const void* chi, const float* scan,
+                                 const void* object_update_precond, const void* probe,
+                                 const void* eigen_probe, const float* eigen_weights,
+                                 int eigen_modes, const void* m_probe_update, const void* patches,
+                                 const void* update, float* nacc, double count, float beta_eigen,
+                                 float* stats, float* sums5, int nscan, int S, int chi_modes,
+                                 int pw, int H, int W, void* stream);
+int tike_lstsq_tail_solve1(void* eigen0, const void* update, int npix, const float* nacc,
+                           float beta_eigen, const float* stats, const float* costs,
+                           const float* sums5, int B, float eps, double count, int recover_psi,
+                           int recover_probe, float* sums3, float* tail3, void* stream);
+
 int tike_lstsq_chunk_gradients(const void* psi, const float* scan, const void* probe,
                                const void* eigen_probe, const float* eigen_weights,
                                int num_eigen, int eigen_modes, const void* data, int data_u16,
diff --git a/tike_amd/_lib.py b/tike_amd/_lib.py
--- a/tike_amd/_lib.py
+++ b/tike_amd/_lib.py
@@ -9,7 +9,7 @@
     _HERE, "csrc", "libtike_amd.so")
 HEADER_PATH = os.path.join(os.path.dirname(_HERE), "include", "tike_amd.h")
 
-ABI_VERSION = 11
+ABI_VERSION = 12
 ERR_ARG = 1000001
 ERR_UNSUPPORTED = 1000002
 ERR_COMM = 2000000
@@ -146,6 +146,15 @@
                                   _i, _i, _p],
     "tike_lstsq_tail_finish": [_p, _p, _d, _p, _p, _p, _p, _f, _l, _p, _l, _i,
                                _i, _p, _p, _i, _i, _p],
+    "tike_ifft2_pass2_gradients_eproj": [_p, _p, _p, _p, _p, _i, _i, _p, _p,
+                                         _p, _f, _i, _i, _i, _f, _p, _p, _p],
+    "tike_eigen_pixel_update1q": [_p, _p, _p, _p, _p, _p, _l, _p, _p, _i, _i,
+                                  _i, _p, _p, _i, _i, _p, _p, _p],
+    "tike_lstsq_step_stats_eigen1": [_p, _p, _p, _p, _p, _p, _i, _p, _p, _p,
+                                     _p, _d, _f, _p, _p, _i, _i, _i, _i, _i,
+                                     _i, _p],
+    "tike_lstsq_tail_solve1": [_p, _p, _i, _p, _f, _p, _p, _p, _i, _f, _d, _i,
+                               _i, _p, _p, _p],
     "tike_lstsq_chunk_gradients": [_p, _p, _p, _p, _p, _i, _i, _p, _i, _p, _i,
                                    _f, _l, _p, _p, _p, _p, _p, _p, _p, _p, _f,
                                    _p, _i, _i, _i, _i, _i, _f, _f, _p],
diff --git a/tike_amd/_tuning.py b/tike_amd/_tuning.py
--- a/tike_amd/_tuning.py
+++ b/tike_amd/_tuning.py
@@ -15,6 +15,7 @@
 chunk_positions = _int("TIKE_CHUNK_POSITIONS")
 eigen_sums_gather = _flag("TIKE_EIGEN_SUMS_GATHER", True)
 stats_gather = _flag("TIKE_STATS_GATHER", False)
+fused_tail = _flag("TIKE_FUSED_TAIL", True)
 precond_chunk = _int("TIKE_PRECOND_CHUNK", 512)
 multislice_slice_step = _flag("TIKE_MS_SLICE_STEP", True)
 multislice_first_stored = _flag("TIKE_MS_FIRST_STORED", True)
diff --git a/tike_amd/csrc/lstsq.hip b/tike_amd/csrc/lstsq.hip
--- a/tike_amd/csrc/lstsq.hip
+++ b/tike_amd/csrc/lstsq.hip
@@ -599,12 +599,14 @@
   int nE;
 };
 
-template <int N, int MW, int MPW, bool HAVE_PROJ, bool EIG = true, bool GRP = false>
+template <int N, int MW, int MPW, bool HAVE_PROJ, bool EIG = true, bool GRP = false,
+          bool QN = false>
 __global__ __launch_bounds__(256, 2) void ifft2_pass2_gradients_kernel(
     const cf* __restrict__ mid, const cf* __restrict__ patches, const TkProbe probe,
     cf* __restrict__ objproj, cf* __restrict__ chi0, float* __restrict__ mpu, float mpu_scale,
     int nscan, int S, float inv_scale, int chunk, float* __restrict__ mpu_part,
-    const float* __restrict__ mode_scale, int Stot_ = 0, int accumulate_ = 0) {
+    const float* __restrict__ mode_scale, int Stot_ = 0, int accumulate_ = 0,
+    float* __restrict__ qtab = nullptr) {
   const int Stot = GRP ? Stot_ : S;
   const bool accumulate = GRP && accumulate_ != 0;
   constexpr int RB = N / 16;
@@ -614,6 +616,8 @@
   constexpr bool REDUCE = HAVE_PROJ && MW > 1;
   constexpr bool HOIST = RB <= 16;
   static_assert(NCB >= 1 && NSLICE % 8 == 0, "slice layout");
+  static_assert(!QN || (HOIST && EIG && HAVE_PROJ && !GRP && NSLICE * CW == N / 4),
+                "q_n partials: eigen slices in LDS, patch values in registers");
   constexpr int NBUF = RB <= 16 ? 2 : 1;
   __shared__ cf part[REDUCE ? NBUF * 4 * RB * 64 : 1];
   extern __shared__ cf eigl[];
@@ -631,6 +635,22 @@
   constexpr long ROW = 16 * N;
   const long slice0 = (long)ya * N + (cb * CW + cw) * 64;
   const unsigned lb = (unsigned)lane * (unsigned)sizeof(cf);
+  auto q_store = [&](float q, int n) {
+    auto dpp = [](float x, auto ctl) {
+      return __int_as_float(__builtin_amdgcn_mov_dpp(__float_as_int(x),
+                                                     decltype(ctl)::value, 0xf, 0xf,
+                                                     false));
+    };
+    q += dpp(q, std::integral_constant<int, 0xb1>{});
+    q += dpp(q, std::integral_constant<int, 0x4e>{});
+    q += dpp(q, std::integral_constant<int, 0x141>{});
+    q += dpp(q, std::integral_constant<int, 0x140>{});
+    auto lane_q = [&](int l) {
+      return __int_as_float(__builtin_amdgcn_readlane(__float_as_int(q), l));
+    };
+    q = (lane_q(0) + lane_q(16)) + (lane_q(32) + lane_q(48));
+    if (lane == 0) qtab[(long)(slice * CW + cw) * nscan + n] = q;
+  };
   if (EIG && HAVE_PROJ && probe.weights != nullptr && probe.eigen != nullptr) {
     const int total = probe.C * probe.Sm * RB * 64 * CW;
     for (int i = threadIdx.x; i < total; i += 256) {
@@ -689,6 +709,17 @@
           for (int yb = 0; yb < RB; ++yb) {
             u[yb] = u[yb] * sc;
             acc[m][yb] = acc[m][yb] + conjf(O[yb]) * u[yb];
+          }
+          if (QN && !REDUCE && s == 0) {
+            const cf* __restrict__ el = eigl + cw * 64 + lane;
+            float q = 0.f;
+#pragma unroll
+            for (int yb = 0; yb < RB; ++yb) {
+              const cf t = conjf(O[yb]) * u[yb];
+              const cf e = el[yb * (64 * CW)];
+              q += t.x * e.x - t.y * e.y;
+            }
+            q_store(q, n);
           }
         } else {
 #pragma unroll
@@ -741,6 +772,18 @@
               const float wc = wn[(c + 1) * probe.S + s];
               const cf* __restrict__ el =
                   eigl + ((c * probe.Sm + s) * RB) * (64 * CW) + cw * 64 + lane;
+              if (QN && c == 0 && s == 0) {
+                float q = 0.f;
+#pragma unroll
+                for (int yb = 0; yb < RB; ++yb) {
+                  const cf e = el[yb * (64 * CW)];
+                  slot[yb * 64] = slot[yb * 64] + (e * u[yb]) * wc;
+                  const cf t = conjf(O[yb]) * u[yb];
+                  q += t.x * e.x - t.y * e.y;
+                }
+                q_store(q, n);
+                continue;
+              }
 #pragma unroll
               for (int yb = 0; yb < RB; ++yb)
                 slot[yb * 64] = slot[yb * 64] + (el[yb * (64 * CW)] * u[yb]) * wc;
@@ -789,16 +832,47 @@
   }
 }
 
+__global__ __launch_bounds__(256) void pass2_q_finish_kernel(const float* __restrict__ qtab,
+                                                             int slots, int nscan,
+                                                             float* __restrict__ q) {
+  const int n = blockIdx.x * 4 + (int)(threadIdx.x >> 6), k = threadIdx.x & 63;
+  if (n >= nscan) return;
+  float a = k < slots ? qtab[(long)k * nscan + n] : 0.f;
+  a = tk_wave_sum(a);
+  if (k == 0) q[n] = a;
+}
+
+template <int N, int MW_, int MPW_>
+static bool launch_pass2_qn(dim3 grid, size_t lds, hipStream_t stream, const cf* work,
+                            const cf* patches, const TkProbe& pr, cf* objproj, cf* chi0,
+                            float* mpu, float mpu_scale, int nscan, int S, float inv_scale,
+                            int chunk, float* mpu_part, const float* mode_scale, float* qtab) {
+  if constexpr (N <= 256) {
+    hipLaunchKernelGGL((ifft2_pass2_gradients_kernel<N, MW_, MPW_, true, true, false, true>),
+                       grid, dim3(256), lds, stream, work, patches, pr, objproj, chi0, mpu,
+                       mpu_scale, nscan, S, inv_scale, chunk, mpu_part, mode_scale, 0, 0, qtab);
+    return true;
+  } else {
+    return false;
+  }
+}
+
 static int launch_pass2_gradients(const void* work, const void* patches, const void* probe,
                                   const void* eigen_probe, const float* eigen_weights,
                                   int num_eigen, int eigen_modes, void* objproj, void* chi0,
                                   void* m_probe_update, float mpu_scale, int nscan, int S,
                                   int det, float inv_scale, const float* mode_scale,
-                                  hipStream_t stream, int Stot = 0, int accumulate = 0) {
+                                  hipStream_t stream, int Stot = 0, int accumulate = 0,
+                                  float* qtab = nullptr, float* q = nullptr) {
   TK_CHECK_ARG(nscan >= 0 && S >= 1 && det >= 1);
   if (nscan == 0) return TK_OK;
   TK_CHECK_ARG(work && patches && (probe || !objproj));
   if (S > 8 || (det != 128 && det != 256 && det != 512)) return TK_ERR_UNSUPPORTED;
+  const bool qn = q != nullptr;
+  TK_CHECK_ARG(!qn || qtab);
+  if (qn && (Stot != 0 || det > 256 || !objproj || !eigen_probe || !eigen_weights ||
+             num_eigen < 1 || eigen_modes < 1))
+    return TK_ERR_UNSUPPORTED;
   const bool grp = Stot != 0;
   if (grp && objproj && S < 2) return TK_ERR_UNSUPPORTED;
   const TkProbe pr = tk_make_probe(probe, 0, eigen_probe, eigen_weights, num_eigen, eigen_modes,
@@ -833,7 +907,13 @@
   if (eig_lds > 32 * 1024) return TK_ERR_UNSUPPORTED;
 #define TK_P2G(N, MW_, MPW_)                                                                 \
   do {                                                                                       \
-    if (grp && !objproj)                                                                     \
+    if (qn) {                                                                                \
+      if (!launch_pass2_qn<N, MW_, MPW_>(grid, eig_lds, stream, (const cf*)work,             \
+                                         (const cf*)patches, pr, (cf*)objproj, (cf*)chi0,    \
+                                         (float*)m_probe_update, mpu_scale, nscan, S,        \
+                                         inv_scale, chunk, mpu_part, mode_scale, qtab))      \
+        return TK_ERR_UNSUPPORTED;                                                           \
+    } else if (grp && !objproj)                                                              \
       hipLaunchKernelGGL((ifft2_pass2_gradients_kernel<N, MW_, MPW_, false, true, true>),    \
                          grid, block, 0,                                                     \
                          stream, (const cf*)work, (const cf*)patches, pr, (cf*)objproj,      \
@@ -888,6 +968,11 @@
 #undef TK_P2G_N
 #undef TK_P2G
   TK_LAUNCH_CHECK();
+  if (qn) {
+    hipLaunchKernelGGL(pass2_q_finish_kernel, dim3((nscan + 3) / 4), dim3(256), 0, stream,
+                       qtab, det / 4, nscan, q);
+    TK_LAUNCH_CHECK();
+  }
   if (mpu_part != nullptr)
     return tk_ordered_sum((float*)m_probe_update, mpu_part, mpu_len, nchunk, true, stream);
   return TK_OK;
@@ -917,6 +1002,20 @@
   return launch_pass2_gradients(work, patches, probe, eigen_probe, eigen_weights, num_eigen,
                                 eigen_modes, objproj, chi0, m_probe_update, mpu_scale, nscan, S,
                                 det, inv_scale, mode_scale, (hipStream_t)stream);
+}
+
+extern "C" int tike_ifft2_pass2_gradients_eproj(const void* work, const void* patches,
+                                                const void* probe, const void* eigen_probe,
+                                                const float* eigen_weights, int num_eigen,
+                                                int eigen_modes, void* objproj, void* chi0,
+                                                void* m_probe_update, float mpu_scale,
+                                                int nscan, int S, int det, float inv_scale,
+                                                float* qtab, float* q, void* stream) {
+  TK_ENTER();
+  TK_CHECK_ARG(nscan == 0 || (qtab && q));
+  return launch_pass2_gradients(work, patches, probe, eigen_probe, eigen_weights, num_eigen,
+                                eigen_modes, objproj, chi0, m_probe_update, mpu_scale, nscan, S,
+                                det, inv_scale, nullptr, (hipStream_t)stream, 0, 0, qtab, q);
 }
 
 extern "C" int tike_ifft2_pass2_eigen_fits(int det, int num_eigen, int eigen_modes) {
@@ -1536,14 +1635,38 @@
   return c.sy >= 0 && c.sx >= 0 && c.sy + pw < H && c.sx + pw < W && (long)H * W < (1L << 28);
 }
 
+constexpr int TK_C0_PARTS = 64;
+__global__ __launch_bounds__(256) void eigen_proj_offset_kernel(const cf* __restrict__ mpu0,
+                                                                const cf* __restrict__ E,
+                                                                long P,
+                                                                float* __restrict__ part) {
+  __shared__ float red[4];
+  float a = 0.f;
+  for (long p = blockIdx.x * 256L + threadIdx.x; p < P; p += 256L * TK_C0_PARTS) {
+    const cf m = mpu0[p], e = E[p];
+    a += m.x * e.x + m.y * e.y;
+  }
+  a = tk_block_sum256(a, red);
+  if (threadIdx.x == 0) part[blockIdx.x] = a;
+}
+
 __global__ __launch_bounds__(256) void eigen_pixel_update1_kernel(
     const TkResidual R, const float* __restrict__ eproj, const float* __restrict__ weights_c,
     long row, const float* __restrict__ norm, float inv_P, float* __restrict__ update, int nscan,
     int chunk, const float* __restrict__ stats, const float* __restrict__ costs, float eps,
     float* __restrict__ sums3, const cf* __restrict__ psi, const float* __restrict__ scan, int pw,
-    int H, int W, float* __restrict__ part) {
+    int H, int W, float* __restrict__ part, const float* __restrict__ c0part,
+    float* __restrict__ eproj_out) {
+  float c0 = 0.f;
+  if (c0part != nullptr) {
+    for (int b = 0; b < TK_C0_PARTS; ++b) c0 += c0part[b];
+  }
   if (blockIdx.x + 1 == gridDim.x) {
-    if (blockIdx.y != 0 || sums3 == nullptr) return;
+    if (blockIdx.y != 0) return;
+    if (eproj_out != nullptr) {
+      for (int n = threadIdx.x; n < nscan; n += 256) eproj_out[n] = eproj[n] - c0;
+    }
+    if (sums3 == nullptr) return;
     __shared__ float red[4];
     float a1 = 0.f, a4 = 0.f, c = 0.f;
     for (int n = threadIdx.x; n < nscan; n += 256) {
@@ -1583,7 +1706,7 @@
       const cf o = tk_patch_pixel(
           psi, (unsigned)(c.sy * W + c.sx) * (unsigned)sizeof(cf) + lane_off, row_bytes, c);
       const cf r = conjf(o) * x - m0;
-      const float w = (eproj[n] * inv_P + weights_c[n * row]) * inv_norm;
+      const float w = ((eproj[n] - c0) * inv_P + weights_c[n * row]) * inv_norm;
       acc.x += r.x * w;
       acc.y += r.y * w;
     }
@@ -1591,7 +1714,7 @@
 #pragma unroll 4
     for (int n = b0; n < b1; ++n) {
       const cf r = R.at<true>(n, p);
-      const float w = (eproj[n] * inv_P + weights_c[n * row]) * inv_norm;
+      const float w = ((eproj[n] - c0) * inv_P + weights_c[n * row]) * inv_norm;
       acc.x += r.x * w;
       acc.y += r.y * w;
     }
@@ -1765,6 +1888,249 @@
   }
 }
 
+__global__ __launch_bounds__(256) __attribute__((amdgpu_waves_per_eu(4)))
+void step_stats_eigen_pair_kernel(
+    const cf* __restrict__ chi, const float* __restrict__ scan, const cf* __restrict__ gobj,
+    const TkProbe probe, const cf* __restrict__ mpu, const cf* __restrict__ patches,
+    const cf* __restrict__ update, const float* __restrict__ nacc, float inv_count, float beta,
+    float* __restrict__ stats, float* __restrict__ sums5, int nscan, int chi_modes, int pw,
+    int H, int W, int nsplit) {
+  __shared__ float red[4];
+  typedef float tk_v4f __attribute__((ext_vector_type(4)));
+  const long P = (long)pw * pw;
+  const int plen = (int)(P / nsplit);
+  const int npair = (nscan + 1) / 2;
+  const float uu = nacc[0], ee = nacc[1], eu = nacc[2];
+  const float mu = sqrtf(uu * inv_count * inv_count / (float)P);
+  const float kk = beta / mu * inv_count;
+  const float inv = 1.0f / sqrtf((ee + 2.0f * kk * eu + kk * kk * uu) / (float)P);
+  auto enew = [&](const cf e, const long p) { return (e + update[p] * kk) * inv; };
+  auto esum = [](float* a, const cf o, const cf x, const cf e, const cf m0) {
+    const cf r = conjf(o) * x - m0;
+    const cf phi = o * e;
+    a[0] += r.x * e.x + r.y * e.y;
+    a[1] += x.x * phi.x + x.y * phi.y;
+    a[2] += norm2(phi);
+    a[3] += r.y * e.x - r.x * e.y;
+  };
+  auto put = [&](float* dst, const float v) {
+    if (nsplit > 1)
+      unsafeAtomicAdd(dst, v);
+    else
+      *dst = v;
+  };
+  auto finish5 = [&](const float* a, const int n) {
+    float t[4];
+#pragma unroll
+    for (int k = 0; k < 4; ++k) t[k] = tk_block_sum256(a[k], red);
+    if (threadIdx.x == 0) {
+      float* o = sums5 + (long)n * 5;
+      put(o, t[0]);
+      put(o + 1, t[1]);
+      put(o + 2, t[2]);
+      put(o + 3, t[0]);
+      put(o + 4, t[3]);
+    }
+  };
+  for (int v = blockIdx.x; v < npair * nsplit; v += gridDim.x) {
+    const int n0 = 2 * (v / nsplit), part = v % nsplit;
+    const TkCorner c0 = tk_corner(scan, n0);
+    const bool two = n0 + 1 < nscan;
+    const TkCorner c1 = tk_corner(scan, two ? n0 + 1 : n0);
+    const bool in0 = c0.sy >= 0 && c0.sx >= 0 && c0.sy + pw < H && c0.sx + pw < W;
+    const bool in1 = c1.sy >= 0 && c1.sx >= 0 && c1.sy + pw < H && c1.sx + pw < W;
+    const int pbeg = part * plen + (int)threadIdx.x;
+    const int pend = part + 1 == nsplit ? (int)P : (part + 1) * plen;
+    if (!(two && in0 && in1)) {
+      for (int i = 0; i < (two ? 2 : 1); ++i) {
+        const int n = n0 + i;
+        step_stats_item<true, true>(chi, scan, nullptr, gobj, probe, mpu, patches, stats,
+                                    chi_modes, pw, H, W, nullptr, nullptr, nsplit, n, part, red);
+        float a[4] = {0.f, 0.f, 0.f, 0.f};
+        for (int p = pbeg; p < pend; p += blockDim.x)
+          esum(a, patches[(long)n * P + p], chi[(long)n * chi_modes * P + p],
+               enew(probe.eigen[p], p), mpu[p]);
+        finish5(a, n);
+      }
+      continue;
+    }
+    float s0 = 1.0f, s1 = 1.0f, t0 = 0.f, t1 = 0.f;
+    if (probe.weights != nullptr) {
+      const float* w = probe.weights + n0 * (long)(probe.C + 1) * probe.S;
+      s0 = w[0];
+      s1 = w[(long)(probe.C + 1) * probe.S];
+      t0 = w[probe.S];
+      t1 = w[(long)(probe.C + 1) * probe.S + probe.S];
+    }
+    float a[8] = {0.f, 0.f, 0.f, 0.f, 0.f, 0.f, 0.f, 0.f};
+    float b[8] = {0.f, 0.f, 0.f, 0.f, 0.f, 0.f, 0.f, 0.f};
+    float ea[4] = {0.f, 0.f, 0.f, 0.f}, eb[4] = {0.f, 0.f, 0.f, 0.f};
+    const unsigned base0 = (unsigned)(c0.sy * W + c0.sx), base1 = (unsigned)(c1.sy * W + c1.sx);
+    const cf* __restrict__ chi_a = chi + ((long)n0 * chi_modes) * P;
+    const cf* __restrict__ chi_b = chi + ((long)(n0 + 1) * chi_modes) * P;
+    const cf* __restrict__ pat_a = patches + (long)n0 * P;
+    const cf* __restrict__ pat_b = pat_a + P;
+    auto tap = [](const tk_v4f u, const tk_v4f l, const TkCorner& c) {
+      cf g = mk(u.x * c.w00, u.y * c.w00);
+      g.x += u.z * c.w01;
+      g.y += u.w * c.w01;
+      g.x += l.x * c.w10;
+      g.y += l.y * c.w10;
+      g.x += l.z * c.w11;
+      g.y += l.w * c.w11;
+      return g;
+    };
+    auto sums = [](float* acc, const cf g, const cf o, const cf x0, const cf p0, const cf pn,
+                   const cf m0) {
+      const cf dOP = g * pn;
+      const cf dPO = m0 * o;
+      const cf OP = o * p0;
+      acc[0] += norm2(dOP);
+      acc[1] += norm2(dPO);
+      const cf a2 = dOP * conjf(dPO);
+      acc[2] += a2.x;
+      acc[3] += a2.y;
+      acc[4] += dOP.x * x0.x + dOP.y * x0.y;
+      acc[5] += dPO.x * x0.x + dPO.y * x0.y;
+      acc[6] += OP.x * x0.x + OP.y * x0.y;
+      acc[7] += norm2(OP);
+    };
+    auto pixel = [&](const int p, const tk_v4f u0, const tk_v4f l0, const tk_v4f u1,
+                     const tk_v4f l1) {
+      const cf oa = pat_a[p], ob = pat_b[p];
+      const cf xa = chi_a[p], xb = chi_b[p];
+      const cf p0 = probe.probe[p];
+      const cf m0 = mpu[p];
+      const cf e1 = probe.eigen[p];
+      const cf en = enew(e1, p);
+      cf pa = p0 * s0, pb = p0 * s1;
+      pa.x += t0 * e1.x;
+      pa.y += t0 * e1.y;
+      pb.x += t1 * e1.x;
+      pb.y += t1 * e1.y;
+      sums(a, tap(u0, l0, c0), oa, xa, p0, pa, m0);
+      sums(b, tap(u1, l1, c1), ob, xb, p0, pb, m0);
+      esum(ea, oa, xa, en, m0);
+      esum(eb, ob, xb, en, m0);
+    };
+    auto taps16 = [&](const unsigned off) {
+      tk_v4f t;
+      __builtin_memcpy(&t, reinterpret_cast<const char*>(gobj) + off, sizeof(t));
+      return t;
+    };
+    const int cols = pw < 256 ? pw : 256, groups = 256 / cols;
+    const int rows = pw / (nsplit * groups);
+    const int ybeg = (part * groups + (int)threadIdx.x / cols) * rows;
+    for (int x = (int)threadIdx.x % cols; x < pw; x += 256) {
+      unsigned rel = (unsigned)(ybeg * W + x);
+      tk_v4f u0 = taps16((base0 + rel) * 8u), u1 = taps16((base1 + rel) * 8u);
+      int p = ybeg * pw + x;
+#pragma unroll 2
+      for (int y = 0; y < rows; ++y) {
+        rel += (unsigned)W;
+        const tk_v4f l0 = taps16((base0 + rel) * 8u), l1 = taps16((base1 + rel) * 8u);
+        pixel(p, u0, l0, u1, l1);
+        u0 = l0;
+        u1 = l1;
+        p += pw;
+      }
+    }
+#pragma unroll
+    for (int k = 0; k < 8; ++k) {
+      const float ta = tk_block_sum256(a[k], red);
+      const float tb = tk_block_sum256(b[k], red);
+      if (threadIdx.x == 0) {
+        put(&stats[(long)n0 * 8 + k], ta);
+        put(&stats[(long)n0 * 8 + 8 + k], tb);
+      }
+    }
+    finish5(ea, n0);
+    finish5(eb, n0 + 1);
+  }
+}
+
+__global__ __launch_bounds__(256) void eigen_norm_sums1_kernel(const cf* __restrict__ E,
+                                                               const cf* __restrict__ update,
+                                                               int npix, float* __restrict__ nacc,
+                                                               float* __restrict__ part) {
+  __shared__ float red[4];
+  float uu = 0.f, ee = 0.f, eu = 0.f;
+  for (int i = blockIdx.x * 256 + threadIdx.x; i < npix; i += gridDim.x * 256) {
+    const cf e = E[i], u = update[i];
+    uu += norm2(u);
+    ee += norm2(e);
+    eu += e.x * u.x + e.y * u.y;
+  }
+  uu = tk_block_sum256(uu, red);
+  ee = tk_block_sum256(ee, red);
+  eu = tk_block_sum256(eu, red);
+  if (threadIdx.x == 0) {
+    if (part != nullptr) {
+      part[3 * blockIdx.x] = uu;
+      part[3 * blockIdx.x + 1] = ee;
+      part[3 * blockIdx.x + 2] = eu;
+    } else {
+      unsafeAtomicAdd(&nacc[0], uu);
+      unsafeAtomicAdd(&nacc[1], ee);
+      unsafeAtomicAdd(&nacc[2], eu);
+    }
+  }
+}
+
+extern "C" int tike_lstsq_step_stats_eigen1(const void* chi, const float* scan,
+                                            const void* object_update_precond, const void* probe,
+                                            const void* eigen_probe, const float* eigen_weights,
+                                            int eigen_modes, const void* m_probe_update,
+                                            const void* patches, const void* update, float* nacc,
+                                            double count, float beta_eigen, float* stats,
+                                            float* sums5, int nscan, int S, int chi_modes,
+                                            int pw, int H, int W, void* stream) {
+  TK_ENTER();
+  TK_CHECK_ARG(nscan >= 0 && S >= 1 && chi_modes >= 1 && pw >= 1 && H >= 1 && W >= 1 &&
+               eigen_modes >= 1 && count > 0);
+  TK_CHECK_ARG(probe && eigen_probe && eigen_weights && m_probe_update && update && nacc);
+  const long P = (long)pw * pw;
+  const long nitem = (nscan + 1) / 2;
+  int nsplit = 1;
+  while (nsplit < 16 && nitem * nsplit * 2 <= 8192 && P % (2048L * nsplit) == 0) nsplit *= 2;
+  if (tk_deterministic()) nsplit = 1;
+  const int groups = 256 / (pw < 256 ? pw : 256);
+  if (!((pw % 256 == 0 || 256 % pw == 0) && pw % (nsplit * groups) == 0 &&
+        (long)H * W < (1L << 28)))
+    return TK_ERR_UNSUPPORTED;
+  int grid = P >= 256 * 64 ? 64 : (int)((P + 255) / 256);
+  float* part = nullptr;
+  if (tk_deterministic()) {
+    part = tk_det_scratch(sizeof(float) * 3 * (size_t)grid);
+    if (part == nullptr) grid = 1;
+  }
+  hipLaunchKernelGGL(eigen_norm_sums1_kernel, dim3(grid), dim3(256), 0, (hipStream_t)stream,
+                     (const cf*)eigen_probe, (const cf*)update, (int)P, nacc, part);
+  TK_LAUNCH_CHECK();
+  if (part != nullptr) {
+    int rc = tk_ordered_sum(nacc, part, 3, grid, true, (hipStream_t)stream);
+    if (rc) return rc;
+  }
+  if (nscan == 0) return TK_OK;
+  TK_CHECK_ARG(chi && scan && object_update_precond && patches && stats && sums5);
+  const TkProbe pr = tk_make_probe(probe, 0, eigen_probe, eigen_weights, 1, eigen_modes, S, pw,
+                                   nullptr);
+  if (nsplit > 1) {
+    hipError_t e = hipMemsetAsync(stats, 0, sizeof(float) * 8 * (size_t)nscan, (hipStream_t)stream);
+    if (e == hipSuccess)
+      e = hipMemsetAsync(sums5, 0, sizeof(float) * 5 * (size_t)nscan, (hipStream_t)stream);
+    if (e != hipSuccess) return (int)e;
+  }
+  hipLaunchKernelGGL(step_stats_eigen_pair_kernel, dim3(tk_grid(nitem * nsplit, 16)), dim3(256),
+                     0, (hipStream_t)stream, (const cf*)chi, scan,
+                     (const cf*)object_update_precond, pr, (const cf*)m_probe_update,
+                     (const cf*)patches, (const cf*)update, (const float*)nacc,
+                     (float)(1.0 / count), beta_eigen, stats, sums5, nscan, chi_modes, pw, H, W,
+                     nsplit);
+  TK_LAUNCH_CHECK();
+  return TK_OK;
+}
+
 static TkResidual make_residual(const void* patches, const void* chi0, const void* mpu0,
                                 const void* eigen, const void* coefs, int C, int Sm, int c,
                                 int pw, int chi_modes) {
@@ -1856,7 +2222,36 @@
   hipLaunchKernelGGL(eigen_pixel_update1_kernel, grid, dim3(256), 0, (hipStream_t)stream, R,
                      eigen_proj, weights_c, weights_row, norm, 1.0f / (float)P, (float*)update,
                      nscan, chunk, stats, costs, eps, sums3, (const cf*)psi, scan, pw, H, W,
-                     part);
+                     part, nullptr, nullptr);
+  TK_LAUNCH_CHECK();
+  if (part != nullptr)
+    return tk_ordered_sum((float*)update, part, 2 * P, (int)grid.y, true, (hipStream_t)stream);
+  return TK_OK;
+}
+
+extern "C" int tike_eigen_pixel_update1q(const void* patches, const void* chi0,
+                                         const void* mpu0, const void* eigen0, const float* q,
+                                         const float* weights_c, long weights_row,
+                                         const float* norm, void* update, int nscan, int pw,
+                                         int chi_modes, const void* psi, const float* scan,
+                                         int H, int W, float* c0part, float* eproj_out,
+                                         void* stream) {
+  TK_ENTER();
+  TK_CHECK_ARG(nscan >= 0 && pw >= 1 && chi_modes >= 1 && weights_row >= 1);
+  if (nscan == 0) return TK_OK;
+  TK_CHECK_ARG(!psi || (scan && H >= 1 && W >= 1));
+  TK_CHECK_ARG(patches && chi0 && mpu0 && eigen0 && q && weights_c && norm && update && c0part);
+  const long P = (long)pw * pw;
+  hipLaunchKernelGGL(eigen_proj_offset_kernel, dim3(TK_C0_PARTS), dim3(256), 0,
+                     (hipStream_t)stream, (const cf*)mpu0, (const cf*)eigen0, P, c0part);
+  float* part = nullptr;
+  const int chunk = probe_chunk(nscan, 2 * P, &part);
+  dim3 grid((unsigned)((P + 255) / 256) + 1, (unsigned)((nscan + chunk - 1) / chunk));
+  const TkResidual R = make_residual(patches, chi0, mpu0, eigen0, nullptr, 1, 1, 0, pw, chi_modes);
+  hipLaunchKernelGGL(eigen_pixel_update1_kernel, grid, dim3(256), 0, (hipStream_t)stream, R, q,
+                     weights_c, weights_row, norm, 1.0f / (float)P, (float*)update, nscan, chunk,
+                     nullptr, nullptr, 0.f, nullptr, (const cf*)psi, scan, pw, H, W, part,
+                     c0part, eproj_out);
   TK_LAUNCH_CHECK();
   if (part != nullptr)
     return tk_ordered_sum((float*)update, part, 2 * P, (int)grid.y, true, (hipStream_t)stream);
diff --git a/tike_amd/csrc/solver.hip b/tike_amd/csrc/solver.hip
--- a/tike_amd/csrc/solver.hip
+++ b/tike_amd/csrc/solver.hip
@@ -404,6 +404,79 @@
     hipLaunchKernelGGL(eigen_apply1_kernel, dim3(grid), dim3(256), 0, (hipStream_t)stream,
                        (cf*)eigen0, (const cf*)update, nacc, (float)(1.0 / count), beta_eigen,
                        npix);
+  TK_LAUNCH_CHECK();
+  return TK_OK;
+}
+
+__global__ __launch_bounds__(256) void lstsq_tail_solve1_kernel(
+    cf* __restrict__ E, const cf* __restrict__ update, const float* __restrict__ nacc,
+    float inv_count, float beta, int npix, const float* __restrict__ stats,
+    const float* __restrict__ costs, const float* __restrict__ sums5, int B, float eps,
+    int recover_psi, int recover_probe, float* __restrict__ sums3, float* __restrict__ tail3) {
+  if (blockIdx.x + 1 < gridDim.x) {
+    const float uu = nacc[0], ee = nacc[1], eu = nacc[2];
+    const float mu = sqrtf(uu * inv_count * inv_count / (float)npix);
+    const float k = beta / mu * inv_count;
+    const float inv = 1.0f / sqrtf((ee + 2.0f * k * eu + k * k * uu) / (float)npix);
+    for (int i = blockIdx.x * 256 + threadIdx.x; i < npix; i += (gridDim.x - 1) * 256)
+      E[i] = (E[i] + update[i] * k) * inv;
+    return;
+  }
+  __shared__ float red[4];
+  float a1 = 0.f, a4 = 0.f, c = 0.f, d = 0.f;
+  for (int n = threadIdx.x; n < B; n += 256) {
+    a1 += stats[8 * n] + eps;
+    a4 += stats[8 * n + 1] + eps;
+    c += costs[n];
+    d += sums5[5 * n + 2] / (float)npix;
+  }
+  a1 = tk_block_sum256(a1, red);
+  a4 = tk_block_sum256(a4, red);
+  c = tk_block_sum256(c, red);
+  d = tk_block_sum256(d, red);
+  const float r1 = 0.5f * a1 * inv_count, r4 = 0.5f * a4 * inv_count;
+  float so = 0.f, sp = 0.f;
+  for (int n = threadIdx.x; n < B; n += 256) {
+    const float* s = stats + 8 * n;
+    const float A1 = s[0] + eps + r1, A4 = s[1] + eps + r4;
+    const float b1 = s[4], b2 = s[5];
+    float x1 = 0.f, x2 = 0.f;
+    if (recover_psi && recover_probe) {
+      const float det = A1 * A4 - (s[2] * s[2] + s[3] * s[3]);
+      x1 = -(s[2] * b2 - A4 * b1) / det;
+      x2 = (A1 * b2 - s[2] * b1) / det;
+    } else if (recover_psi) {
+      x1 = b1 / A1;
+    } else if (recover_probe) {
+      x2 = b2 / A4;
+    }
+    so += 0.9f * fmaxf(x1, 0.f);
+    sp += 0.9f * fmaxf(x2, 0.f);
+  }
+  so = tk_block_sum256(so, red);
+  sp = tk_block_sum256(sp, red);
+  if (threadIdx.x == 0) {
+    sums3[0] = a1;
+    sums3[1] = a4;
+    sums3[2] = c;
+    tail3[0] = so;
+    tail3[1] = sp;
+    tail3[2] = d;
+  }
+}
+
+extern "C" int tike_lstsq_tail_solve1(void* eigen0, const void* update, int npix,
+                                      const float* nacc, float beta_eigen, const float* stats,
+                                      const float* costs, const float* sums5, int B, float eps,
+                                      double count, int recover_psi, int recover_probe,
+                                      float* sums3, float* tail3, void* stream) {
+  TK_ENTER();
+  TK_CHECK_ARG(B >= 0 && count > 0 && npix >= 1 && sums3 && tail3);
+  TK_CHECK_ARG(eigen0 && update && nacc && (B == 0 || (stats && costs && sums5)));
+  const int grid = npix >= 256 * 64 ? 64 : (npix + 255) / 256;
+  hipLaunchKernelGGL(lstsq_tail_solve1_kernel, dim3(grid + 1), dim3(256), 0, (hipStream_t)stream,
+                     (cf*)eigen0, (const cf*)update, nacc, (float)(1.0 / count), beta_eigen,
+                     npix, stats, costs, sums5, B, eps, recover_psi, recover_probe, sums3, tail3);
   TK_LAUNCH_CHECK();
   return TK_OK;
 }
diff --git a/tike_amd/ptycho/solvers/_plan.py b/tike_amd/ptycho/solvers/_plan.py
--- a/tike_amd/ptycho/solvers/_plan.py
+++ b/tike_amd/ptycho/solvers/_plan.py
@@ -190,6 +190,11 @@
                            for e in launches),
             groups=groups)
 
+    def eigen_q(self, C, Sm, H, W):
+        return (self.fused and not self.groups and not self.steps_in_pass2
+                and self.det in (128, 256) and self.pw == self.det
+                and C == 1 and Sm >= 1 and H * W < (1 << 28))
+
     def buffers(self, ws, B, dev, *, varying, want_patches):
         S, pw, det = self.S, self.pw, self.det
         n = min(self.chunk, max(B, 1))
@@ -464,6 +469,10 @@
                 check(lib.tike_ifft2_pass2_gradients_scaled(
                     *p2, A.ptr(b.steps), st),
                     "inverse pass 2 + gradients (x poisson steps)")
+            elif k.q is not None:
+                check(lib.tike_ifft2_pass2_gradients_eproj(
+                    *p2, A.ptr(b.qtab), A.ptr(k.q), st),
+                    "inverse pass 2 + gradients + eigen projection")
             else:
                 check(lib.tike_ifft2_pass2_gradients(*p2, st),
                       "inverse pass 2 + gradients")
diff --git a/tike_amd/ptycho/solvers/lstsq.py b/tike_amd/ptycho/solvers/lstsq.py
--- a/tike_amd/ptycho/solvers/lstsq.py
+++ b/tike_amd/ptycho/solvers/lstsq.py
@@ -225,6 +225,9 @@
         if comm.collective:
             comm.Allreduce(eigen_norms)
 
+    want_q = bool(FUSED_TAIL and eigen_norms is not None and recover_psi
+                  and not comm.collective and not STATS_PATCH_RECOMPUTE)
+
     for batch_index in order:
         lo, hi = _lo_hi(batches[batch_index])
         comm.minibatch = int(batch_index)
@@ -232,7 +235,7 @@
             data, psi, scan, probe, eigen_probe, eigen_weights, lo, hi, comm,
             num_batch=num_batch, exitwave_options=exitwave_options, op=op,
             recover_psi=recover_psi, recover_probe=recover_probe,
-            position_terms=position_terms)
+            position_terms=position_terms, want_q=want_q)
 
         object_update_precond = None
         if recover_psi:
@@ -362,6 +365,12 @@
 """The step statistics gather O_n from the object with the two 16-byte tap
 loads they already issue for the preconditioned update (same offsets)."""
 
+FUSED_TAIL = _tuning.fused_tail
+"""One rank, one eigen probe, the fused pass 2 at 128^2 / 256^2: pass 2 leaves
+the per-position part of the eigen projection, the eigen update runs before
+the step statistics, and the statistics and the eigen position sums are one
+pass over chi_n,0 and the patches (tike_lstsq_step_stats_eigen1)."""
+
 PACKED_TAIL = True
 """Tests set this to False to run the staged tail (one entry per step of the
 reference's _update_nearplane / _precondition_nearplane_gradients)."""
@@ -396,7 +405,8 @@
 def _get_nearplane_gradients(data, psi, scan, probe, eigen_probe,
                              eigen_weights, lo, hi, comm, *, num_batch,
                              exitwave_options, op, recover_psi, recover_probe,
-                             position_terms=None, need_chi0=True):
+                             position_terms=None, need_chi0=True,
+                             want_q=False):
     dev = psi.device
     B = hi - lo
     S, pw = probe.shape[-3], probe.shape[-1]
@@ -427,6 +437,14 @@
                           or position_terms))
     if position_terms:
         taps, taps_r = gaussian_derivative_taps(sigma=0.333)
+    q = None
+    if (want_q and recover_psi and recover_probe and w_old is not None
+            and buf.patches is not None and need_chi0
+            and plan.eigen_q(C, Sm, H, W)):
+        q = _workspace(op).get("eigen_q", (max(B, 1),), torch.float32, dev)
+        buf.qtab = _workspace(op).get("eigen_qtab", (min(plan.chunk, max(B, 1)),
+                                                     det // 4),
+                                      torch.float32, dev)
     c = SimpleNamespace(
         op=op, data=data, psi=psi, probe=probe, ep=ep, eigen_probe=eigen_probe,
         C=C, Sm=Sm, H=H, W=W, st=A.stream_ptr(), fwd_scale=fwd_scale,
@@ -446,7 +464,8 @@
             w=None if w_old is None else w_old[rows], uq=None,
             costs=buf.costs[rows],
             patches=None if buf.patches is None else buf.patches[rows],
-            chi0=None if buf.chi0 is None else buf.chi0[rows])
+            chi0=None if buf.chi0 is None else buf.chi0[rows],
+            q=None if q is None else q[rows])
         k.data_f32 = _once(lambda a=clo, b=chi_hi: A.data_f32(data, a, b))
         if k.w is not None and Sm > 0 and buf.unique is not None and (
                 not plan.no_farplane):
@@ -492,7 +511,8 @@
                 chi_modes=S if buf.single_chunk else 1, w_old=w_old,
                 patches=None if buf.patches is None else buf.patches[:B],
                 object_acc=obj_acc, m_probe_update=m_probe_update,
-                costs=buf.costs[:B], count=count, local_count=B)
+                costs=buf.costs[:B], count=count, local_count=B,
+                q=None if q is None else q[:B])
 
 
 def object_upd_sum(g):
@@ -570,6 +590,15 @@
     update = small[4:4 + 2 * P]
     nacc = small[4 + 2 * P:4 + 2 * P + 4]
     tail3 = small[4 + 2 * P + 4:4 + 2 * P + 7]
+    if (one and g.get("q") is not None and not comm.collective
+            and object_update_precond is not None and psi.shape[0] == 1):
+        return _fused_tail(g, psi, scan, probe, eigen_probe, eigen_weights,
+                           object_update_precond, lo, hi, op=op,
+                           num_batch=num_batch, recover_psi=recover_psi,
+                           recover_probe=recover_probe, norm=norm,
+                           steps_row=steps_row,
+                           probe_combined_update=probe_combined_update,
+                           sums3=sums3, update=update, nacc=nacc, tail3=tail3)
     stats = _step_stats(g, psi, scan, probe, eigen_probe,
                         object_update_precond, lo, hi, op=op)
     eps_total = float(np.float32(np.float32(1e-9) / P) * P)
@@ -622,6 +651,66 @@
             A.ptr(mpu), 1.0 / num_batch, probe.numel(),
             None if w_rows is None else w_rows.data_ptr(), row, S, 0,
             A.ptr(stats), A.ptr(sums5), B, P, st), "minibatch tail")
+    return (steps_row[2] if recover_psi else None,
+            steps_row[3] if recover_probe else None)
+
+
+def _fused_tail(g, psi, scan, probe, eigen_probe, eigen_weights,
+                object_update_precond, lo, hi, *, op, num_batch, recover_psi,
+                recover_probe, norm, steps_row, probe_combined_update, sums3,
+                update, nacc, tail3):
+    B = hi - lo
+    dev = psi.device
+    st = A.stream_ptr()
+    S, pw = probe.shape[-3], probe.shape[-1]
+    P = pw * pw
+    H, W = psi.shape[-2:]
+    count = float(g["count"])
+    ws = _workspace(op)
+    mpu = g["m_probe_update"]
+    Sm = eigen_probe.shape[-3]
+    w_rows = eigen_weights[lo:hi]
+    row = w_rows.shape[-2] * w_rows.shape[-1]
+    E = eigen_probe[0, 0, 0]
+    eps_total = float(np.float32(np.float32(1e-9) / P) * P)
+    stats = ws.get("stats", (max(B, 1), 8), torch.float32, dev)
+    sums5 = ws.get("eigen_sums5", (max(B, 1), 5), torch.float32, dev)
+    eproj = ws.get("eigen_proj", (max(B, 1),), torch.float32, dev)
+    c0part = ws.get("eigen_c0part", (64,), torch.float32, dev)
+    g["eigen_proj"] = eproj[:B]
+    gpsi = A.ptr(psi[0]) if EIGEN_PATCH_RECOMPUTE else None
+    scan_b = A.ptr(scan[lo:hi])
+    check(
+        lib.tike_eigen_pixel_update1q(
+            A.ptr(g["patches"]), A.ptr(g["chi0"]), A.ptr(mpu[0, 0, 0]),
+            A.ptr(E), A.ptr(g["q"]), w_rows[:, 1, 0].data_ptr(), row,
+            A.ptr(norm), A.ptr(update), B, pw, g["chi_modes"], gpsi, scan_b,
+            H, W, A.ptr(c0part), A.ptr(eproj), st),
+        "eigen pixel update")
+    beta_eigen = min(0.1, 1.0 / num_batch)
+    check(
+        lib.tike_lstsq_step_stats_eigen1(
+            A.ptr(g["chi0"]), scan_b, A.ptr(object_update_precond),
+            A.ptr(probe), A.ptr(eigen_probe), A.ptr(g["w_old"]), Sm,
+            A.ptr(mpu), A.ptr(g["patches"]), A.ptr(update), A.ptr(nacc), count,
+            beta_eigen, A.ptr(stats), A.ptr(sums5), B, S, g["chi_modes"], pw,
+            H, W, st),
+        "step-size statistics + eigen position sums")
+    check(
+        lib.tike_lstsq_tail_solve1(
+            A.ptr(E), A.ptr(update), P, A.ptr(nacc), beta_eigen, A.ptr(stats),
+            A.ptr(g["costs"]), A.ptr(sums5), B, eps_total, count,
+            int(recover_psi), int(recover_probe), A.ptr(sums3), A.ptr(tail3),
+            st), "eigen probe + step solve")
+    check(
+        lib.tike_lstsq_tail_finish(
+            A.ptr(tail3), A.ptr(sums3), count, A.ptr(steps_row),
+            A.ptr(probe) if recover_probe else None,
+            A.ptr(probe_combined_update) if recover_probe else None,
+            A.ptr(mpu), 1.0 / num_batch, probe.numel(), w_rows.data_ptr(), row,
+            S, 0, A.ptr(stats), A.ptr(sums5), B, P, st), "minibatch tail")
+    g["stats"] = stats[:B]
+    g["sums5"] = sums5[:B]
     return (steps_row[2] if recover_psi else None,
             steps_row[3] if recover_probe else None)
 
```

New measurement: 217,800 patterns/s (median of 6 runs). 2.1% higher.
